# settylab/Mellon

Measured on AMD Instinct MI355X. Metric: cells/sec fit_predict, higher is better.
Workload: dtype f64

## Files before the change

mellon_amd/csrc/api_fit.hip:

```cpp
#include "api_internal.h"
#include "mln_options.h"
#include <mutex>
#include <unordered_map>

void fit_sample_rows(const mln_fit* f, int64_t s, int64_t* first, int64_t* rows) {
  if (s < 1) s = 1;
  *first = (s - f->row0 % s) % s;
  *rows = (f->n > *first) ? (f->n - *first + s - 1) / s : 0;
}

void fit_free(mln_fit* f) {
  if (!f) return;
  mln_ctx* ctx = f->ctx;
  (void)hipSetDevice(ctx->device);
  (void)hipStreamSynchronize(ctx->stream);
  if (f->L && f->L != f->Lp) (void)mln_dfree(f->L);
  if (f->Lp) (void)mln_dfree(f->Lp);
  triinv_free(&f->tri);
  void* ptrs[] = {f->V, f->Vdr, f->part_grad, f->part_hess, f->part_loss, f->d_z, f->d_out,
                  f->C, f->Cinv, f->d_u, f->d_gu, f->d_tmp, f->P, f->d_w, f->d_w_cached,
                  f->Q1, f->Q2, f->d_zw, f->d_zr, f->eigU, f->L32, f->sv_block, f->f_keep[0], f->f_keep[1], f->Kj, f->d_over,
                  f->dim_ell, f->dim_part, f->dim_z, f->dim_out};
  for (void* p : ptrs) if (p) (void)mln_dfree(p);
  for (double* p : f->saved_precond) if (p) (void)mln_dfree(p);
  if (f->h_state) (void)mln_hfree(f->h_state);
  fit_events_return(ctx, &f->evs);
  if (f->h_z) (void)mln_hfree(f->h_z);
  if (f->h_out) (void)mln_hfree(f->h_out);
  if (f->ev0) (void)hipEventDestroy(f->ev0);
  if (f->ev1) (void)hipEventDestroy(f->ev1);
  delete f;
}

extern "C" void mln_fit_destroy(mln_fit* fit) { fit_free(fit); }

int fit_alloc_workspace(mln_fit* f) {
  mln_ctx* ctx = f->ctx;
  int64_t steps = (f->n + 1) / 2;
  int n_wg = ctx->n_cu > 0 ? ctx->n_cu : 256;
  f->n_wg_cap = n_wg;
  if (steps < n_wg) n_wg = (int)(steps > 0 ? steps : 1);
  f->n_wg = n_wg;
  n_wg = f->n_wg_cap;
  const size_t pm = (size_t)f->ldl;
  f->ld2 = pad16(f->m + 2);
  MLN_HIP(ctx, mln_dmalloc((void**)&f->d_u, sizeof(double) * pm));
  MLN_HIP(ctx, mln_dmalloc((void**)&f->d_gu, sizeof(double) * pm));
  MLN_HIP(ctx, mln_dmalloc((void**)&f->d_tmp, sizeof(double) * (1 + pm)));
  MLN_HIP(ctx, mln_dmalloc((void**)&f->d_w, sizeof(double) * pm));
  MLN_HIP(ctx, mln_dmalloc((void**)&f->d_w_cached, sizeof(double) * pm));
  MLN_HIP(ctx, mln_dmalloc((void**)&f->d_zw, sizeof(double) * 2 * pm));
  MLN_HIP(ctx, mln_dmalloc((void**)&f->d_zr, sizeof(double) * 2 * (size_t)f->ld2));
  MLN_HIP(ctx, hipMemsetAsync(f->d_zr, 0, sizeof(double) * 2 * (size_t)f->ld2, ctx->stream));
  MLN_HIP(ctx, mln_dmalloc((void**)&f->d_over, 64));
  MLN_HIP(ctx, hipMemsetAsync(f->d_over, 0, 64, ctx->stream));
  MLN_HIP(ctx, mln_dmalloc((void**)&f->part_grad, sizeof(double) * pm * n_wg));
  MLN_HIP(ctx, mln_dmalloc((void**)&f->part_hess, sizeof(double) * pm * n_wg));
  MLN_HIP(ctx, mln_dmalloc((void**)&f->part_loss, sizeof(double) * n_wg));
  MLN_HIP(ctx, mln_dmalloc((void**)&f->d_z, sizeof(double) * pm));
  MLN_HIP(ctx, mln_dmalloc((void**)&f->d_out, sizeof(double) * (1 + 2 * pm)));
  MLN_HIP(ctx, mln_hmalloc((void**)&f->h_z, sizeof(double) * pm));
  MLN_HIP(ctx, mln_hmalloc((void**)&f->h_out, sizeof(double) * (1 + 2 * pm)));
  MLN_HIP(ctx, hipEventCreate(&f->ev0));
  MLN_HIP(ctx, hipEventCreate(&f->ev1));
  return MLN_OK;
}

namespace {
struct CopyLane { hipStream_t stream = nullptr; std::vector<hipEvent_t> events; };
std::mutex g_copy_mu;
std::unordered_map<mln_ctx*, CopyLane> g_copy_lanes;
}

static int copy_lane_get(mln_ctx* ctx, int n_events, hipStream_t* stream, std::vector<hipEvent_t>* events) {
  std::lock_guard<std::mutex> lk(g_copy_mu);
  CopyLane& lane = g_copy_lanes[ctx];
  if (!lane.stream) MLN_HIP(ctx, hipStreamCreateWithFlags(&lane.stream, hipStreamNonBlocking));
  while ((int)lane.events.size() < n_events) {
    hipEvent_t e = nullptr;
    MLN_HIP(ctx, hipEventCreateWithFlags(&e, hipEventDisableTiming));
    lane.events.push_back(e);
  }
  *stream = lane.stream;
  events->assign(lane.events.begin(), lane.events.begin() + n_events);
  return MLN_OK;
}

namespace {
std::unordered_map<mln_ctx*, std::vector<hipEvent_t>> g_event_pools;
}
void fit_events_borrow(mln_ctx* ctx, std::vector<hipEvent_t>* evs) {
  std::lock_guard<std::mutex> lk(g_copy_mu);
  auto& pool = g_event_pools[ctx];
  if (evs->empty()) evs->swap(pool);
}
void fit_events_return(mln_ctx* ctx, std::vector<hipEvent_t>* evs) {
  std::lock_guard<std::mutex> lk(g_copy_mu);
  auto& pool = g_event_pools[ctx];
// ... 122 lines not shown
  const double t_enter = now_s();
  const bool trace_all = std::getenv("MELLON_AMD_TRACE") != nullptr;
  MLN_TRY(mln_lower_cov(ctx, cov, d, &f->cov));
  f->d = d; f->n = n; f->full = (xu == nullptr);
  if (f->full) m = n;
  f->m = m;
  if (m < 1 || m > 65535) { mln_set_error(ctx, "number of landmarks out of range"); return MLN_ERR_SHAPE; }
  if (m > objective_max_m()) { mln_set_error(ctx, "m > 8192 landmarks is not supported by this build"); return MLN_ERR_UNSUPPORTED; }
  if (f->full && ctx->n_ranks > 1) { mln_set_error(ctx, "the full (non-sparse) GP cannot be cell-sharded"); return MLN_ERR_UNSUPPORTED; }
  f->ldp = pad16(m);
  f->ldl = pad16(m);
  DevIn dx, du;
  HostUpload up;
  bool pipelined = !f->full && n > 0 && x && !is_device_ptr(x) && (size_t)n * d * sizeof(double) >= ((size_t)32 << 20);
  if (pipelined) {
    dx.ctx = ctx;
    MLN_HIP(ctx, mln_dmalloc((void**)&dx.owned, (size_t)n * d * sizeof(double)));
    dx.dev = dx.owned;
    MLN_TRY(up.start(ctx, x, dx.owned, n, d));
    if (trace_all) fprintf(stderr, "[trace] fit_prepare: upload started at %.4f s (%d chunks)\n", now_s() - t_enter, up.n_chunks);
  } else {
    MLN_TRY(dx.init(ctx, x, (size_t)n * d));
  }
  if (!f->full) MLN_TRY(du.init(ctx, xu, (size_t)m * d));
  const double* centers = f->full ? dx.dev : du.dev;

  double t0 = now_s();
  const size_t lp_bytes = sizeof(double) * (size_t)m * f->ldp;
  MLN_HIP(ctx, mln_dmalloc((void**)&f->Lp, lp_bytes));
  MLN_HIP(ctx, hipMemsetAsync(f->Lp, 0, lp_bytes, ctx->stream));
  if (Lp_in) {
    DevIn dl;
    MLN_TRY(dl.init(ctx, Lp_in, (size_t)m * m));
    MLN_TRY(launch_copy_block(ctx, dl.dev, m, f->Lp, f->ldp, m, m));
    MLN_HIP(ctx, hipStreamSynchronize(ctx->stream));
  } else {
    MLN_TRY(launch_kernel_matrix(ctx, f->cov, centers, m, centers, m, d, f->Lp, f->ldp, jitter));
    const bool implicit = !f->full && (flags & MLN_FIT_IMPLICIT) != 0;
    if (implicit) {
      MLN_HIP(ctx, mln_dmalloc((void**)&f->Kj, lp_bytes));
      MLN_HIP(ctx, hipMemcpyAsync(f->Kj, f->Lp, lp_bytes, hipMemcpyDeviceToDevice, ctx->stream));
    }
    MLN_HIP(ctx, hipStreamSynchronize(ctx->stream));
    f->times[0] += now_s() - t0;
    t0 = now_s();
    if (implicit && (flags & MLN_FIT_DEFER_LP)) f->lp_pending = true;
    else MLN_TRY(dev_cholesky_lower(ctx, f->Lp, m, f->ldp));
  }
  f->jitter = jitter;
  if (!f->lp_pending) {
    MLN_TRY(triinv_build(ctx, f->Lp, m, f->ldp, true, true, &f->tri));
    MLN_HIP(ctx, hipStreamSynchronize(ctx->stream));
    f->times[1] += now_s() - t0;
  }

  if (f->full) {
    f->L = f->Lp;
  } else {
    t0 = now_s();
    const size_t l_bytes = sizeof(double) * (size_t)(n > 0 ? n : 1) * f->ldl;
    const bool trace = std::getenv("MELLON_AMD_TRACE") != nullptr;
    MLN_HIP(ctx, mln_dmalloc((void**)&f->L, l_bytes));
    if (trace) { (void)hipStreamSynchronize(ctx->stream); fprintf(stderr, "[trace] L alloc %.4f s\n", now_s() - t0); }
    int64_t mixed_min = (int64_t)1 << 27;
    bool mixed = false;
    if (const char* ev = std::getenv("MELLON_AMD_MIXED")) mixed = (flags & MLN_FIT_IMPLICIT) != 0 && std::atoi(ev) != 0;
    if (const char* ev = std::getenv("MELLON_AMD_MIXED_MIN_ELEMS")) mixed_min = std::atoll(ev);
    if (mixed && n * m >= mixed_min && n > 0 && m <= 8192)
      MLN_HIP(ctx, mln_dmalloc((void**)&f->L32, sizeof(float) * (size_t)n * f->ldl));
    f->l32_fixed = 0;
    bool bounded = true;
    for (int l = 0; l < f->cov.n_leaves; ++l)
      bounded = bounded && f->cov.leaves[l].kind >= MLN_K_MATERN32 && f->cov.leaves[l].kind <= MLN_K_RATQUAD;
    for (int t = 0; t < f->cov.n_toks; ++t)
      bounded = bounded && (f->cov.tok_op[t] == MLN_OP_LEAF || f->cov.tok_op[t] == MLN_OP_MUL);
    f->cov_bounded01 = bounded;
    if (f->L32) {
      f->l32_fixed = bounded ? 1 : 0;
      if (const char* ev = std::getenv("MELLON_AMD_SURROGATE")) {
        if (std::strcmp(ev, "float") == 0) f->l32_fixed = 0;
        else if (std::strcmp(ev, "fixed") == 0 && bounded) f->l32_fixed = 1;
      }
    }
    if (pipelined) {
      for (int c = 0; c < up.n_chunks; ++c) {
        int64_t r0 = 0, rows = 0;
        MLN_TRY(up.wait_chunk(c, &r0, &rows));
        MLN_TRY(launch_kernel_matrix(ctx, f->cov, dx.dev + r0 * d, rows, du.dev, m, d, f->L + r0 * f->ldl, f->ldl, 0.0,
                                     f->L32 ? f->L32 + r0 * f->ldl : nullptr, f->l32_fixed));
      }
      MLN_TRY(up.finish());
    } else {
      MLN_TRY(launch_kernel_matrix(ctx, f->cov, dx.dev, n, du.dev, m, d, f->L, f->ldl, 0.0, f->L32, f->l32_fixed));
    }
    MLN_TRY(fit_alloc_workspace(f));
    MLN_HIP(ctx, hipStreamSynchronize(ctx->stream));
    if (trace) fprintf(stderr, "[trace] L kernel matrix done at %.4f s\n", now_s() - t0);
    f->times[0] += now_s() - t0;
    if (flags & MLN_FIT_IMPLICIT) {
      f->kspace = true;
    } else {
      t0 = now_s();
      MLN_TRY(triinv_solve_right_T(ctx, f->tri, f->L, n, f->ldl));
      MLN_HIP(ctx, hipStreamSynchronize(ctx->stream));
      f->times[2] += now_s() - t0;
    }
  }
  if (!f->d_u) MLN_TRY(fit_alloc_workspace(f));
  if (trace_all) fprintf(stderr, "[trace] fit_prepare: body done at %.4f s\n", now_s() - t_enter);
  return MLN_OK;
}

extern "C" int mln_fit_prepare(mln_ctx* ctx, const mln_kernel_desc* cov, const double* x, int64_t n_local,
                               int32_t d, const double* xu, int64_t m, double jitter, const double* Lp_in,
                               int32_t flags, mln_fit** out) {
  if (!ctx || !out) return MLN_ERR_ARG;
  *out = nullptr;
  if (n_local < 0 || d < 1 || (n_local > 0 && !x)) { mln_set_error(ctx, "bad shape"); return MLN_ERR_SHAPE; }
  MLN_HIP(ctx, hipSetDevice(ctx->device));
  mln_fit* f = new mln_fit();
  const double t_call = now_s();
  int rc = fit_prepare_impl(ctx, cov, x, n_local, d, xu, m, jitter, Lp_in, flags, f);
  if (std::getenv("MELLON_AMD_TRACE")) fprintf(stderr, "[trace] mln_fit_prepare: %.4f s with the upload's teardown\n", now_s() - t_call);
  if (rc != MLN_OK) { fit_free(f); return rc; }
  *out = f;
  return MLN_OK;
}

extern "C" int mln_fit_from_L(mln_ctx* ctx, const double* L, int64_t n_local, int64_t m, const double* Lp,
                              mln_fit** out) {
  if (!ctx || !out || !L) return MLN_ERR_ARG;
  *out = nullptr;
  if (n_local < 1 || m < 1 || m > 65535) { mln_set_error(ctx, "bad shape"); return MLN_ERR_SHAPE; }
  if (m > objective_max_m()) { mln_set_error(ctx, "m > 8192 columns is not supported by this build"); return MLN_ERR_UNSUPPORTED; }
  MLN_HIP(ctx, hipSetDevice(ctx->device));
  mln_fit* f = new mln_fit();
  f->ctx = ctx; f->n = n_local; f->m = m; f->d = 0; f->full = false;
  f->ldl = pad16(m); f->ldp = pad16(m);
  auto body = [&]() -> int {
    DevIn dl;
    MLN_TRY(dl.init(ctx, L, (size_t)n_local * m));
    const size_t l_bytes = sizeof(double) * (size_t)n_local * f->ldl;
    MLN_HIP(ctx, mln_dmalloc((void**)&f->L, l_bytes));
    MLN_HIP(ctx, hipMemsetAsync(f->L, 0, l_bytes, ctx->stream));
    MLN_TRY(launch_copy_block(ctx, dl.dev, m, f->L, f->ldl, n_local, m));
    if (Lp) {
      DevIn dp;
      MLN_TRY(dp.init(ctx, Lp, (size_t)m * m));
      const size_t lp_bytes = sizeof(double) * (size_t)m * f->ldp;
      MLN_HIP(ctx, mln_dmalloc((void**)&f->Lp, lp_bytes));
      MLN_HIP(ctx, hipMemsetAsync(f->Lp, 0, lp_bytes, ctx->stream));
      MLN_TRY(launch_copy_block(ctx, dp.dev, m, f->Lp, f->ldp, m, m));
      MLN_TRY(triinv_build(ctx, f->Lp, m, f->ldp, true, true, &f->tri));
    }
    MLN_HIP(ctx, hipStreamSynchronize(ctx->stream));
    return fit_alloc_workspace(f);
  };
  int rc = body();
  if (rc != MLN_OK) { fit_free(f); return rc; }
  *out = f;
  return MLN_OK;
}

extern "C" int mln_fit_prepare_from_K(mln_ctx* ctx, const double* Kuu, int64_t n_local, int64_t m, double jitter,
                                      const double* Lp_in, int32_t flags, mln_fit** out) {
  if (!ctx || !out) return MLN_ERR_ARG;
  *out = nullptr;
  const bool full = (flags & MLN_FIT_FULL) != 0;
  if (n_local < 0 || m < 1 || m > 65535 || (full && n_local != m)) { mln_set_error(ctx, "bad shape"); return MLN_ERR_SHAPE; }
  if (!Kuu && !Lp_in) { mln_set_error(ctx, "mln_fit_prepare_from_K needs cov(xu, xu) or its factor"); return MLN_ERR_ARG; }
  if (full && ctx->n_ranks > 1) { mln_set_error(ctx, "the full (non-sparse) GP cannot be cell-sharded"); return MLN_ERR_UNSUPPORTED; }
  MLN_HIP(ctx, hipSetDevice(ctx->device));
  mln_fit* f = new mln_fit();
  f->ctx = ctx; f->n = n_local; f->m = m; f->d = 0; f->full = full;
  f->ldl = pad16(m); f->ldp = pad16(m);
  f->cov.n_leaves = 0; f->cov.n_toks = 0;
// ... 44 lines not shown
  MLN_HIP(ctx, hipStreamSynchronize(ctx->stream));
  f->k_rows_done += n_rows;
  f->times[0] += now_s() - t0;
  return MLN_OK;
}

extern "C" int mln_fit_finish_K(mln_fit* f) {
  if (!f) return MLN_ERR_ARG;
  mln_ctx* ctx = f->ctx;
  if (!f->from_K) { mln_set_error(ctx, "mln_fit_finish_K: not a handle built from kernel values"); return MLN_ERR_ARG; }
  if (f->k_finished || f->full) { f->k_finished = true; return MLN_OK; }
  if (f->k_rows_done < f->n) { mln_set_error(ctx, "mln_fit_finish_K: kernel rows are missing"); return MLN_ERR_SHAPE; }
  MLN_HIP(ctx, hipSetDevice(ctx->device));
  if (!f->kspace) {
    double t0 = now_s();
    MLN_TRY(triinv_solve_right_T(ctx, f->tri, f->L, f->n, f->ldl));
    MLN_HIP(ctx, hipStreamSynchronize(ctx->stream));
    f->times[2] += now_s() - t0;
  }
  f->k_finished = true;
  return fit_alloc_workspace(f);
}


extern "C" int mln_fit_gram_eigh(mln_fit* f, double* w, int32_t* n_sweeps) {
  if (!f || !w) return MLN_ERR_ARG;
  mln_ctx* ctx = f->ctx;
  MLN_HIP(ctx, hipSetDevice(ctx->device));
  const int64_t m = f->m, ld = f->ldl;
  double* G = nullptr;
  MLN_HIP(ctx, mln_dmalloc((void**)&G, sizeof(double) * (size_t)m * ld));
  int rc = f->kspace ? fit_gram(f, G, ld, 1) : gram_of(ctx, f->L, f->ldl, f->n, m, 1.0, G, ld);
  if (rc == MLN_OK && !f->eigU) {
    hipError_t e = mln_dmalloc((void**)&f->eigU, sizeof(double) * (size_t)m * ld);
    if (e != hipSuccess) rc = mln_hip_fail(ctx, e, "alloc eigenvectors", __FILE__, __LINE__);
  }
  std::vector<double> wh((size_t)m);
  int sweeps = 0;
  if (rc == MLN_OK) rc = dev_eigh(ctx, G, m, ld, wh.data(), f->eigU, ld, &sweeps);
  (void)hipStreamSynchronize(ctx->stream);
  (void)mln_dfree(G);
  if (rc != MLN_OK) return rc;
  if (n_sweeps) *n_sweeps = sweeps;
  std::memcpy(w, wh.data(), sizeof(double) * (size_t)m);
  return MLN_OK;
}

extern "C" int mln_fit_gram_rank(mln_fit* f, double tol, int64_t* rank_out, double* sigma_max_out) {
  if (!f || !rank_out || !(tol >= 0.0)) return MLN_ERR_ARG;
  mln_ctx* ctx = f->ctx;
  MLN_HIP(ctx, hipSetDevice(ctx->device));
  const int64_t m = f->m, ld = f->ldl;
  double* G = nullptr;
  MLN_HIP(ctx, mln_dmalloc((void**)&G, sizeof(double) * (size_t)m * ld));
  const int n_ranks = ctx->n_ranks > 1 ? ctx->n_ranks : 1;
  const int64_t n_est = f->n * n_ranks;
  int64_t stride = 1;
  if (f->kspace && n_est >= 24 * m) stride = std::max<int64_t>(1, n_est / (12 * m));
  auto gram = [&]() { return f->kspace ? fit_gram(f, G, ld, stride) : gram_of(ctx, f->L, f->ldl, f->n, m, 1.0, G, ld); };
  int rc = gram();
  double lmax = 0.0;
  const bool ldl_ok = !(mln_experiment("MELLON_AMD_RANK_LDL") && std::atoi(mln_experiment("MELLON_AMD_RANK_LDL")) == 0);
  bool done = false;
  if (rc == MLN_OK && ldl_ok) {
    rc = dev_sym_rank_above_ldl(ctx, G, m, ld, tol * tol, rank_out, &lmax, &done);
    if (rc == MLN_OK && !done) rc = gram();
  }
  if (rc == MLN_OK && !done) rc = dev_sym_rank_above(ctx, G, m, ld, tol * tol, rank_out, &lmax);
  f->rank_path = done ? 1 : 2;
  (void)hipStreamSynchronize(ctx->stream);
  (void)mln_dfree(G);
  if (rc == MLN_OK && sigma_max_out) *sigma_max_out = std::sqrt(std::max(lmax, 0.0));
  return rc;
}

extern "C" int mln_fit_project(mln_fit* f, int64_t p, mln_fit** out) {
  if (!f || !out) return MLN_ERR_ARG;
  *out = nullptr;
  mln_ctx* ctx = f->ctx;
  if (!f->eigU) { mln_set_error(ctx, "project: call mln_fit_gram_eigh first"); return MLN_ERR_ARG; }
  if (f->kspace) { mln_set_error(ctx, "project needs the explicit factor (prepare without MLN_FIT_IMPLICIT)"); return MLN_ERR_UNSUPPORTED; }
  if (p < 1 || p > f->m) { mln_set_error(ctx, "project: rank out of range"); return MLN_ERR_SHAPE; }
  MLN_HIP(ctx, hipSetDevice(ctx->device));
  mln_fit* g = new mln_fit();
  g->ctx = ctx; g->n = f->n; g->m = p; g->d = 0; g->full = false;
  g->ldl = pad16(p); g->ldp = pad16(p);
  auto body = [&]() -> int {
    const size_t l_bytes = sizeof(double) * (size_t)(g->n > 0 ? g->n : 1) * g->ldl;
    MLN_HIP(ctx, mln_dmalloc((void**)&g->L, l_bytes));
    MLN_HIP(ctx, hipMemsetAsync(g->L, 0, l_bytes, ctx->stream));
    if (g->n > 0) {
      GemmArgs a{};
      a.A = f->L; a.lda = f->ldl; a.ta = 0;
      a.B = f->eigU + (f->m - p) * f->ldl; a.ldb = f->ldl; a.tb = 1;
      a.C = g->L; a.ldc = g->ldl;
      a.M = g->n; a.N = p; a.K = f->m; a.alpha = 1.0; a.beta = 0.0; a.split_k = 1;
      MLN_TRY(launch_dgemm(ctx, a));
    }
    MLN_HIP(ctx, hipStreamSynchronize(ctx->stream));
    return fit_alloc_workspace(g);
  };
  int rc = body();
  if (rc != MLN_OK) { fit_free(g); return rc; }
  *out = g;
  return MLN_OK;
}

extern "C" int mln_fit_rank(mln_fit* fit, int64_t* m_out) {
  if (!fit || !m_out) return MLN_ERR_ARG;
  *m_out = fit->m;
  return MLN_OK;
}

extern "C" int mln_fit_get_Lp(mln_fit* f, double* out) {
  if (!f || !out) return MLN_ERR_ARG;
  mln_ctx* ctx = f->ctx;
  if (!f->Lp) { mln_set_error(ctx, "this fit handle holds no Lp"); return MLN_ERR_ARG; }
  MLN_HIP(ctx, hipSetDevice(ctx->device));
  MLN_TRY(fit_ensure_lp(f, false));
  DevOut o;
  MLN_TRY(o.init(ctx, out, (size_t)f->m * f->m));
  MLN_TRY(launch_copy_block(ctx, f->Lp, f->ldp, o.dev, f->m, f->m, f->m));
  return o.commit();
}

extern "C" int mln_fit_get_L(mln_fit* f, int64_t row0, int64_t n_rows, double* out) {
  if (!f || (n_rows > 0 && !out)) return MLN_ERR_ARG;
  mln_ctx* ctx = f->ctx;
  if (row0 < 0 || n_rows < 0 || row0 + n_rows > f->n) { mln_set_error(ctx, "row range out of bounds"); return MLN_ERR_SHAPE; }
  if (n_rows == 0) return MLN_OK;
  MLN_HIP(ctx, hipSetDevice(ctx->device));
  DevOut o;
  MLN_TRY(o.init(ctx, out, (size_t)n_rows * f->m));
  if (f->kspace) {
    MLN_TRY(fit_ensure_lp(f));
    double* tmp = nullptr;
    MLN_HIP(ctx, mln_dmalloc((void**)&tmp, sizeof(double) * (size_t)n_rows * f->ldl));
    int rc = launch_copy_block(ctx, f->L + row0 * f->ldl, f->ldl, tmp, f->ldl, n_rows, f->ldl);
    if (rc == MLN_OK) rc = triinv_solve_right_T(ctx, f->tri, tmp, n_rows, f->ldl);
    if (rc == MLN_OK) rc = launch_copy_block(ctx, tmp, f->ldl, o.dev, f->m, n_rows, f->m);
    if (rc == MLN_OK) rc = o.commit();
    (void)mln_dfree(tmp);
    return rc;
  }
  MLN_TRY(launch_copy_block(ctx, f->L + row0 * f->ldl, f->ldl, o.dev, f->m, n_rows, f->m));
  return o.commit();
}

extern "C" int mln_fit_set_likelihood(mln_fit* f, const double* V, const double* Vdr, double mu) {
  if (!f || (f->n > 0 && (!V || !Vdr))) return MLN_ERR_ARG;
  mln_ctx* ctx = f->ctx;
  MLN_HIP(ctx, hipSetDevice(ctx->device));
  const size_t bytes = sizeof(double) * (size_t)(f->n > 0 ? f->n : 1);
  if (!f->V) MLN_HIP(ctx, mln_dmalloc((void**)&f->V, bytes));
  if (!f->Vdr) MLN_HIP(ctx, mln_dmalloc((void**)&f->Vdr, bytes));
  if (f->n > 0) {
    MLN_HIP(ctx, hipMemcpyAsync(f->V, V, sizeof(double) * f->n, hipMemcpyDefault, ctx->stream));
    MLN_HIP(ctx, hipMemcpyAsync(f->Vdr, Vdr, sizeof(double) * f->n, hipMemcpyDefault, ctx->stream));
    MLN_HIP(ctx, hipStreamSynchronize(ctx->stream));
  }
  f->mu = mu;
  return MLN_OK;
}

ObjArgs obj_args(mln_fit* f) {
  ObjArgs a{};
  a.L = f->L; a.ldl = f->ldl; a.n = f->n; a.m = f->m;
  a.z = f->d_z; a.V = f->V; a.Vdr = f->Vdr; a.mu = f->mu;
  a.part_grad = f->part_grad; a.part_hess = nullptr; a.part_loss = f->part_loss;
  a.weights = nullptr; a.f_out = nullptr;
  a.n_wg = f->n_wg; a.m_pad = f->ldl;
  return a;
}
```

mellon_amd/csrc/api_internal.h:

```cpp
#pragma once
#include <chrono>
#include <cmath>
#include <cstdio>
#include <cstdlib>
#include <algorithm>
#include <atomic>
#include <cstring>
#include <mutex>
#include <string>
#include <thread>
#include <vector>

#include "linalg.h"
#include "mln_internal.h"
#include "objective.h"
#include "precond_rebuild.h"
#include "solver.h"

hipError_t mln_hmalloc(void** out, size_t bytes);
hipError_t mln_hfree(void* p);
void fit_events_borrow(mln_ctx* ctx, std::vector<hipEvent_t>* evs);
void fit_events_return(mln_ctx* ctx, std::vector<hipEvent_t>* evs);

void mln_dfree_defer(std::vector<void*>* sink);
bool is_device_ptr(const void* p);
double now_s();

struct DevIn {
  mln_ctx* ctx;
  const double* dev = nullptr;
  double* owned = nullptr;
  int init(mln_ctx* c, const double* p, size_t count) {
    ctx = c;
    if (count == 0 || !p) { dev = p; return MLN_OK; }
    if (is_device_ptr(p)) { dev = p; return MLN_OK; }
    MLN_HIP(ctx, mln_dmalloc((void**)&owned, count * sizeof(double)));
    MLN_HIP(ctx, hipMemcpyAsync(owned, p, count * sizeof(double), hipMemcpyHostToDevice, ctx->stream));
    dev = owned;
    return MLN_OK;
  }
  ~DevIn() {
    if (owned) { (void)hipStreamSynchronize(ctx->stream); (void)mln_dfree(owned); }
  }
};

struct DevOut {
  mln_ctx* ctx;
  double* dev = nullptr;
  double* owned = nullptr;
  double* host = nullptr;
  size_t count = 0;
  int init(mln_ctx* c, double* p, size_t n, bool copy_in = false) {
    ctx = c; count = n;
    if (n == 0) { dev = p; return MLN_OK; }
    if (is_device_ptr(p)) { dev = p; return MLN_OK; }
    host = p;
    MLN_HIP(ctx, mln_dmalloc((void**)&owned, n * sizeof(double)));
    if (copy_in) MLN_HIP(ctx, hipMemcpyAsync(owned, p, n * sizeof(double), hipMemcpyHostToDevice, ctx->stream));
    dev = owned;
    return MLN_OK;
  }
  int commit() {
    if (owned && count) {
      MLN_HIP(ctx, hipMemcpyAsync(host, owned, count * sizeof(double), hipMemcpyDeviceToHost, ctx->stream));
    }
    MLN_HIP(ctx, hipStreamSynchronize(ctx->stream));
    return MLN_OK;
  }
  ~DevOut() {
    if (owned) { (void)hipStreamSynchronize(ctx->stream); (void)mln_dfree(owned); }
  }
};

struct mln_fit {
  mln_ctx* ctx = nullptr;
  DevCov cov;
  int d = 0;
  int64_t n = 0, m = 0, ldl = 0, ldp = 0;
  bool full = false;
  double* L = nullptr;
  double* Lp = nullptr;
  TriInv tri;
  double *V = nullptr, *Vdr = nullptr;
  double mu = 0.0;
  int n_wg = 0;
  double *part_grad = nullptr, *part_hess = nullptr, *part_loss = nullptr;
  double *d_z = nullptr, *d_out = nullptr;
  double *h_z = nullptr, *h_out = nullptr;
  hipEvent_t ev0 = nullptr, ev1 = nullptr;
  double times[MLN_N_STAGE_TIMES] = {0};
  double *C = nullptr, *Cinv = nullptr;
  double *d_u = nullptr, *d_gu = nullptr, *d_tmp = nullptr;
  int n_wg_cap = 0;
  bool kspace = false;
  double* P = nullptr;
  double* Kj = nullptr;
  bool lp_pending = false, lp_failed = false, tri_pending = false;
  double jitter = 0.0;
  double* d_w = nullptr;
  std::vector<double> z_cached;
  double* d_w_cached = nullptr;
  double *Q1 = nullptr, *Q2 = nullptr, *d_zw = nullptr, *d_zr = nullptr;
  double* eigU = nullptr;
  float* L32 = nullptr;
  double emu_excluded = 0.0;
  bool cov_bounded01 = false;
  int l32_fixed = 0;
  int evals32 = 0;
  double times32 = 0.0;
  int64_t ld2 = 0;
  int* d_over = nullptr;
  int64_t row0 = 0;
  SolverBuffers sv{};
  void* sv_block = nullptr;
  SolverState* h_state = nullptr;
  int sv_maxcor = 0;
  std::vector<hipEvent_t> evs;
  double* f_keep[2] = {nullptr, nullptr};
  int f_final = -1;
  int64_t precond_stride = 0;
  bool from_K = false, k_finished = false;
  int64_t k_rows_done = 0;
  double* saved_precond[5] = {nullptr, nullptr, nullptr, nullptr, nullptr};
  int n_revert = 0, n_rebuild_skipped = 0, n_start_halvings = 0, rank_path = 0;
  double build_seconds = 0.0;
  double times_sub = 0.0, times_rebuild = 0.0, sub_pass_equiv = 0.0;
  int evals_sub = 0, n_rebuild = 0;
  double* dim_ell = nullptr;
  int dim_k = 0;
  double mu_dim = 0.0, mu_dens = 0.0;
  double *dim_part = nullptr, *dim_z = nullptr, *dim_out = nullptr;
};

struct DevScratch {
  mln_ctx* ctx;
  double* p = nullptr;
  explicit DevScratch(mln_ctx* c) : ctx(c) {}
  hipError_t alloc(size_t bytes) { return mln_dmalloc((void**)&p, bytes); }
  ~DevScratch() {
    if (p) { (void)hipStreamSynchronize(ctx->stream); (void)mln_dfree(p); }
  }
  DevScratch(const DevScratch&) = delete;
  DevScratch& operator=(const DevScratch&) = delete;
};


int dev_allreduce(mln_ctx* ctx, double* dev, int64_t count);
int dev_bcast0(mln_ctx* ctx, double* dev, int64_t count);
int reject_distance_leaf(mln_ctx* ctx, const DevCov& dc);
int64_t pad16(int64_t m);
void fit_sample_rows(const mln_fit* f, int64_t s, int64_t* first, int64_t* rows);
void fit_free(mln_fit* f);
int fit_alloc_workspace(mln_fit* f);
int fit_prepare_impl(mln_ctx* ctx, const mln_kernel_desc* cov, const double* x, int64_t n, int32_t d,
                            const double* xu, int64_t m, double jitter, const double* Lp_in, int32_t flags,
                            mln_fit* f);
ObjArgs obj_args(mln_fit* f);
void obj_account(mln_fit* f, bool f32 = false);
int fit_w_from_z(mln_fit* f, const double* z_dev, double* w_dev, const double* z_host = nullptr);
int fit_cache_pair_from_u(mln_fit* f, const double* u_dev);
int fit_enqueue_eval(mln_fit* f, const double* u_dev, double* gn_dev, bool use32, const int* gate,
                            hipEvent_t* ev, const std::vector<int64_t>* sub_strides = nullptr);
int fit_objective_u(mln_fit* f, const double* u, double* loss, double* grad_u, double* z_out,
                           bool use32 = false);
int fit_solver_alloc(mln_fit* f, int maxcor);
int gram_of(mln_ctx* ctx, const double* A, int64_t lda, int64_t rows, int64_t m, double alpha, double* G,
                   int64_t ldg, bool quantised = false);
int emulated_ranks(const mln_ctx* ctx);
int fit_ensure_kj(mln_fit* f);
int fit_ensure_lp(mln_fit* f, bool need_tri = true);
int fit_lp_finish(mln_fit* f, int rc_chol, double t0);
int fit_gram(mln_fit* f, double* G, int64_t ldg, int64_t row_stride, bool whiten = true);
int fit_gemvT(mln_fit* f, const double* t_dev, double* rhs_dev);
void fit_drop_precond_operators(mln_fit* f);
int fit_factor_precond(mln_fit* f);
int fit_build_precond(mln_fit* f, int64_t row_stride);
int fit_rebuild_precond(mln_fit* f, const double* f_dev, double rows_per_m, int* outcome, double cap = 1e300);
void fit_precond_saved_free(mln_fit* f);
int fit_precond_revert(mln_fit* f);
int fit_small_gemv(mln_fit* f, const double* M, int trans, const double* w, double* y);
int launch_scale_rows_cols(mln_ctx* ctx, double* A, int64_t ld, int64_t rows, int64_t cols, const double* row,
                                  const double* col);
int sparse_solve_impl(mln_ctx* ctx, const mln_kernel_desc* cov, const double* x, int64_t n_local,
                             int32_t d, const double* xu, int64_t m, const double* y, int64_t p, double mu,
                             const double* sigmas, int32_t kind, double jitter, double* W, double* Lp_out,
                             double* Cs_out);
unsigned grid_1d(int64_t count);
```

mellon_amd/csrc/api_precond.hip:

```cpp
#include "api_internal.h"
#include "mln_options.h"

namespace {
__global__ void k_pack_lower(const double* __restrict__ G, int64_t m, int64_t ld, double* __restrict__ out) {
  const int64_t i = blockIdx.y;
  const int64_t j = (int64_t)blockIdx.x * blockDim.x + threadIdx.x;
  if (j <= i) out[i * (i + 1) / 2 + j] = G[i * ld + j];
}
__global__ void k_unpack_symmetric(const double* __restrict__ in, int64_t m, int64_t ld, double* __restrict__ G) {
  const int64_t i = blockIdx.y;
  const int64_t j = (int64_t)blockIdx.x * blockDim.x + threadIdx.x;
  if (j < m) G[i * ld + j] = (j <= i) ? in[i * (i + 1) / 2 + j] : in[j * (j + 1) / 2 + i];
}
}

int allreduce_symmetric_lower(mln_ctx* ctx, double* G, int64_t m, int64_t ldg) {
  const int64_t cnt = m * (m + 1) / 2;
  double* packed = nullptr;
  MLN_HIP(ctx, mln_dmalloc((void**)&packed, sizeof(double) * (size_t)cnt));
  const dim3 grid((unsigned)((m + 255) / 256), (unsigned)m), block(256);
  hipLaunchKernelGGL(k_pack_lower, grid, block, 0, ctx->stream, G, m, ldg, packed);
  int rc = dev_allreduce(ctx, packed, cnt);
  if (rc == MLN_OK) {
    hipLaunchKernelGGL(k_unpack_symmetric, grid, block, 0, ctx->stream, packed, m, ldg, G);
// ... 13 lines not shown
  double* parts = nullptr;
  if (split > 1) MLN_HIP(ctx, mln_dmalloc((void**)&parts, sizeof(double) * stride * split));
  GemmArgs g{};
  g.A = A; g.lda = lda; g.B = A; g.ldb = lda;
  g.C = (split > 1) ? parts : G; g.ldc = ldg;
  g.M = m; g.N = m; g.K = rows; g.alpha = alpha; g.beta = 0.0; g.ta = 1; g.tb = 0; g.lower_only = 1;
  g.split_k = split; g.c_split_stride = (int64_t)stride;
  int rc = MLN_OK;
  if (split > 1) rc = (hipMemsetAsync(parts, 0, sizeof(double) * stride * split, ctx->stream) == hipSuccess) ? MLN_OK : MLN_ERR_HIP;
  else rc = (hipMemsetAsync(G, 0, sizeof(double) * stride, ctx->stream) == hipSuccess) ? MLN_OK : MLN_ERR_HIP;
  if (rc == MLN_OK && rows > 0)
    rc = quantised ? launch_gram_i8(ctx, A, lda, rows, m, alpha, g.C, ldg, (int64_t)stride, split) : launch_dgemm(ctx, g);
  if (rc == MLN_OK && split > 1) rc = launch_sum_partials(ctx, parts, split, (int64_t)stride, G, (int64_t)stride, 0.0);
  if (rc == MLN_OK && ctx->n_ranks > 1) rc = allreduce_symmetric_lower(ctx, G, m, ldg);
  else if (rc == MLN_OK) rc = launch_symmetrize_from_lower(ctx, G, m, ldg);
  (void)hipStreamSynchronize(ctx->stream);
  if (parts) (void)mln_dfree(parts);
  return rc;
}

extern "C" int mln_diag_gram_i8(mln_ctx* ctx, const double* A, int64_t rows, int64_t m, double* out, int32_t reps,
                                double* ms_out) {
  if (!ctx || !A || !out || rows < 1 || m < 1) return MLN_ERR_ARG;
  MLN_HIP(ctx, hipSetDevice(ctx->device));
  DevIn a;
  DevOut o;
  MLN_TRY(a.init(ctx, A, (size_t)rows * m));
  MLN_TRY(o.init(ctx, out, (size_t)m * m));
  const int split = gram_i8_splits(rows, m);
  const size_t stride = (size_t)m * m;
  double *parts = nullptr, *G = nullptr;
  MLN_HIP(ctx, mln_dmalloc((void**)&parts, sizeof(double) * stride * split));
  MLN_HIP(ctx, mln_dmalloc((void**)&G, sizeof(double) * stride));
  hipEvent_t e0, e1;
  MLN_HIP(ctx, hipEventCreate(&e0));
  MLN_HIP(ctx, hipEventCreate(&e1));
  int rc = MLN_OK;
  if (reps < 1) reps = 1;
  for (int r = 0; r <= reps && rc == MLN_OK; ++r) {
    if (r == 1) (void)hipEventRecord(e0, ctx->stream);
    rc = (hipMemsetAsync(parts, 0, sizeof(double) * stride * split, ctx->stream) == hipSuccess) ? MLN_OK : MLN_ERR_HIP;
    if (rc == MLN_OK) rc = launch_gram_i8(ctx, a.dev, m, rows, m, 1.0, parts, m, (int64_t)stride, split);
    if (rc == MLN_OK) rc = launch_sum_partials(ctx, parts, split, (int64_t)stride, G, (int64_t)stride, 0.0);
  }
  (void)hipEventRecord(e1, ctx->stream);
  (void)hipStreamSynchronize(ctx->stream);
  float ms = 0.f;
  (void)hipEventElapsedTime(&ms, e0, e1);
  if (ms_out) *ms_out = ms / reps;
  if (rc == MLN_OK) rc = launch_symmetrize_from_lower(ctx, G, m, m);
  if (rc == MLN_OK) rc = launch_copy_block(ctx, G, m, o.dev, m, m, m);
  if (rc == MLN_OK) rc = o.commit();
  (void)hipStreamSynchronize(ctx->stream);
  (void)mln_dfree(parts); (void)mln_dfree(G);
  (void)hipEventDestroy(e0); (void)hipEventDestroy(e1);
  return rc;
}

int emulated_ranks(const mln_ctx* ctx) {
  if (ctx->n_ranks > 1) return 0;
  if (const char* ev = std::getenv("MELLON_AMD_EMULATE_RANKS")) { const int n = std::atoi(ev); return n > 1 ? n : 0; }
  return 0;
}

int fit_ensure_kj(mln_fit* f) {
  if (f->Kj) return MLN_OK;
  mln_ctx* ctx = f->ctx;
  if (!f->Lp) { mln_set_error(ctx, "this fit handle holds no Lp"); return MLN_ERR_ARG; }
  const size_t bytes = sizeof(double) * (size_t)f->m * f->ldp;
  MLN_HIP(ctx, mln_dmalloc((void**)&f->Kj, bytes));
  MLN_HIP(ctx, hipMemsetAsync(f->Kj, 0, bytes, ctx->stream));
  GemmArgs g{};
  g.A = f->Lp; g.lda = f->ldp; g.B = f->Lp; g.ldb = f->ldp; g.C = f->Kj; g.ldc = f->ldp;
  g.M = f->m; g.N = f->m; g.K = f->m; g.alpha = 1.0; g.beta = 0.0; g.ta = 0; g.tb = 1; g.lower_only = 1;
  MLN_TRY(launch_dgemm(ctx, g));
  return launch_symmetrize_from_lower(ctx, f->Kj, f->m, f->ldp);
}

int fit_gram(mln_fit* f, double* G, int64_t ldg, int64_t row_stride, bool whiten) {
  mln_ctx* ctx = f->ctx;
  if (row_stride < 1) row_stride = 1;
  const int64_t first = (row_stride - f->row0 % row_stride) % row_stride;
  const int64_t rows = (f->n > first) ? (f->n - first + row_stride - 1) / row_stride : 0;
  const double* Ls = f->L + first * f->ldl;
  if (!f->kspace) return gram_of(ctx, Ls, f->ldl * row_stride, rows, f->m, (double)row_stride, G, ldg);
  bool quant = f->cov_bounded01 && f->m >= 256 && row_stride > 1;
  if (const char* ev = mln_experiment("MELLON_AMD_GRAM_I8")) quant = quant && std::atoi(ev) != 0;
  int rc = gram_of(ctx, Ls, f->ldl * row_stride, rows, f->m, (double)row_stride, G, ldg, quant);
  if (rc != MLN_OK || !whiten) return rc;
  MLN_TRY(fit_ensure_lp(f));
  double* T = nullptr;
  {
    hipError_t e = mln_dmalloc((void**)&T, sizeof(double) * (size_t)f->m * ldg);
    if (e == hipSuccess) e = hipMemsetAsync(T, 0, sizeof(double) * (size_t)f->m * ldg, ctx->stream);
    if (e != hipSuccess) rc = mln_hip_fail(ctx, e, "alloc Gram temp", __FILE__, __LINE__);
  }
  if (rc == MLN_OK) rc = triinv_solve_left(ctx, f->tri, G, f->m, ldg);
  if (rc == MLN_OK) rc = launch_transpose(ctx, G, ldg, T, ldg, f->m);
  if (rc == MLN_OK) rc = triinv_solve_left(ctx, f->tri, T, f->m, ldg);
  if (rc == MLN_OK) rc = (hipMemcpyAsync(G, T, sizeof(double) * (size_t)f->m * ldg, hipMemcpyDeviceToDevice,
                                         ctx->stream) == hipSuccess) ? MLN_OK : MLN_ERR_HIP;
  (void)hipStreamSynchronize(ctx->stream);
  if (T) (void)mln_dfree(T);
  return rc;
}

int fit_gemvT(mln_fit* f, const double* t_dev, double* rhs_dev) {
  mln_ctx* ctx = f->ctx;
  ObjArgs a = obj_args(f);
  a.weights = t_dev;
  a.part_loss = nullptr;
  MLN_TRY(launch_objective(ctx, a));
  MLN_TRY(launch_reduce_obj(ctx, a, f->d_out));
  MLN_TRY(dev_allreduce(ctx, f->d_out, 1 + f->m));
  if (f->kspace) { MLN_TRY(fit_ensure_lp(f)); MLN_TRY(triinv_solve_left(ctx, f->tri, f->d_out + 1, 1, 1)); }
  MLN_HIP(ctx, hipMemcpyAsync(rhs_dev, f->d_out + 1, sizeof(double) * f->m, hipMemcpyDeviceToDevice, ctx->stream));
  return MLN_OK;
}

void fit_drop_precond_operators(mln_fit* f) {
  (void)hipStreamSynchronize(f->ctx->stream);
  void* ptrs[] = {f->Cinv, f->P, f->Q1, f->Q2};
  for (void* p : ptrs) if (p) (void)mln_dfree(p);
  f->Cinv = nullptr; f->P = nullptr; f->Q1 = nullptr; f->Q2 = nullptr;
}

int fit_factor_precond(mln_fit* f) {
  mln_ctx* ctx = f->ctx;
  const int64_t m = f->m, ldg = f->ldl;
  const size_t bytes = sizeof(double) * (size_t)m * ldg;
  int rc = f->kspace ? MLN_OK : launch_add_diag(ctx, f->C, m, ldg, 1.0);
  if (rc == MLN_OK && f->kspace && f->lp_pending && !f->lp_failed && f->ldp == ldg) {
    const double t0 = now_s();
    int bad = 0;
    rc = dev_cholesky_lower2(ctx, f->C, f->Lp, m, ldg, &bad);
    const int rc_lp = (rc == MLN_ERR_NOT_PD && !(bad & 2)) ? MLN_OK : rc;
    if (rc == MLN_OK || rc == MLN_ERR_NOT_PD) {
      const std::string msg = ctx->err;
      const int rl = fit_lp_finish(f, rc_lp, t0);
      if (rl != MLN_OK) return rl;
      if (rc != MLN_OK) mln_set_error(ctx, msg);
    }
  } else if (rc == MLN_OK) {
    rc = dev_cholesky_lower(ctx, f->C, m, ldg);
  }
  TriInv t;
  if (rc == MLN_OK) rc = triinv_build(ctx, f->C, m, ldg, true, false, &t);
  double* inv = nullptr;
  auto zeroed = [&](double** p, const char* what) {
    hipError_t e = mln_dmalloc((void**)p, bytes);
    if (e == hipSuccess) e = hipMemsetAsync(*p, 0, bytes, ctx->stream);
    if (e != hipSuccess) rc = mln_hip_fail(ctx, e, what, __FILE__, __LINE__);
  };
  if (rc == MLN_OK) zeroed(&inv, "alloc factor inverse");
  if (rc == MLN_OK) rc = launch_add_diag(ctx, inv, m, ldg, 1.0);
  if (rc == MLN_OK) rc = triinv_solve_left(ctx, t, inv, m, ldg, true);
  if (rc == MLN_OK && f->kspace) {
    zeroed(&f->P, "alloc P");
    if (rc == MLN_OK) rc = launch_transpose(ctx, inv, ldg, f->P, ldg, m);
  } else if (rc == MLN_OK) {
    const int64_t ld = ldg;
    const size_t blk = (size_t)m * ld;
    hipError_t e = mln_dmalloc((void**)&f->Q1, sizeof(double) * blk);
    if (e == hipSuccess) e = mln_dmalloc((void**)&f->Q2, sizeof(double) * blk * 2);
    if (e == hipSuccess) e = hipMemsetAsync(f->Q1, 0, sizeof(double) * blk, ctx->stream);
    if (e == hipSuccess) e = hipMemsetAsync(f->Q2, 0, sizeof(double) * blk * 2, ctx->stream);
    if (e != hipSuccess) rc = mln_hip_fail(ctx, e, "alloc stacked operators", __FILE__, __LINE__);
    if (rc == MLN_OK) rc = launch_transpose(ctx, inv, ld, f->Q1, ld, m);
    if (rc == MLN_OK) rc = launch_copy_block(ctx, inv, ld, f->Q2, ld * 2, m, ld);
    if (rc == MLN_OK) rc = launch_copy_block(ctx, inv, ld, f->Q2 + ld, ld * 2, m, ld);
  }
  (void)hipStreamSynchronize(ctx->stream);
  triinv_free(&t);
  if (rc == MLN_OK) f->Cinv = inv; else if (inv) (void)mln_dfree(inv);
  return rc;
}

int fit_build_precond(mln_fit* f, int64_t row_stride) {
  if (f->Cinv) return MLN_OK;
  mln_ctx* ctx = f->ctx;
  const int64_t m = f->m, ldg = f->ldl;
  const size_t bytes = sizeof(double) * (size_t)m * ldg;
  double t0 = now_s();
  MLN_HIP(ctx, mln_dmalloc((void**)&f->C, bytes));
  int rc = fit_gram(f, f->C, ldg, row_stride, false);
  if (rc == MLN_OK && f->kspace) rc = fit_ensure_kj(f);
  if (rc == MLN_OK && f->kspace) rc = launch_axpby(ctx, m * ldg, 1.0, f->Kj, 1.0, f->C);
  MLN_HIP(ctx, hipStreamSynchronize(ctx->stream));
  f->times[3] += now_s() - t0;
  double t1 = now_s();
  if (rc == MLN_OK) rc = fit_factor_precond(f);
  f->times[4] += now_s() - t1;
  if (rc == MLN_OK) { f->precond_stride = row_stride < 1 ? 1 : row_stride; f->build_seconds = now_s() - t0; }
  return rc;
}

void fit_precond_saved_free(mln_fit* f) {
  bool any = false;
  for (double* p : f->saved_precond) any = any || p;
  if (!any) return;
  (void)hipStreamSynchronize(f->ctx->stream);
  for (double*& p : f->saved_precond) { if (p) (void)mln_dfree(p); p = nullptr; }
}

int fit_precond_revert(mln_fit* f) {
  if (!f->saved_precond[0] || !f->saved_precond[1]) return MLN_ERR_ARG;
  fit_drop_precond_operators(f);
  if (f->C) { (void)mln_dfree(f->C); f->C = nullptr; }
  f->C = f->saved_precond[0]; f->Cinv = f->saved_precond[1]; f->P = f->saved_precond[2];
  f->Q1 = f->saved_precond[3]; f->Q2 = f->saved_precond[4];
  for (double*& p : f->saved_precond) p = nullptr;
  return MLN_OK;
}

int fit_rebuild_precond(mln_fit* f, const double* f_dev, double rows_per_m, int* outcome, double cap) {
  mln_ctx* ctx = f->ctx;
  const int64_t m = f->m, ldg = f->ldl;
  *outcome = 0;
  RebuildSelection sel{};
  double target = rows_per_m * (double)m;
  if (const int n_emu = emulated_ranks(ctx)) target /= (double)n_emu;
  const bool tr_on = std::getenv("MELLON_AMD_TRACE") != nullptr;
  double tt[6] = {0, 0, 0, 0, 0, 0};
  auto lap = [&](int i, double& t0) { if (tr_on) { (void)hipStreamSynchronize(ctx->stream); const double t1 = now_s(); tt[i] += t1 - t0; t0 = t1; } };
  double tl = now_s();
  MLN_TRY(rebuild_select_rows(ctx, f_dev, f->V, f->n, f->row0, target, 0x6d656c6c6f6eull, &sel, cap));
  lap(0, tl);
  if (tr_on)
    fprintf(stderr, "[trace] rebuild: %lld of %lld local rows kept (target %.0f global), c = %.4g, 1/c = %.4g, w_max = %.4g, sum a = %.6g\n",
            (long long)sel.rows, (long long)f->n, target, sel.c, 1.0 / sel.c, sel.w_max, sel.sum_a);
  double range_cap = 1e7;
  if (const char* ev = mln_experiment("MELLON_AMD_REBUILD_RANGE")) range_cap = std::atof(ev);
  if (!(sel.w_max * sel.c <= range_cap) || !std::isfinite(sel.sum_a)) {
    rebuild_selection_free(ctx, &sel);
    *outcome = 1;
    return MLN_OK;
  }
  double* R = nullptr;
  int rc = MLN_OK;
  const int64_t rr = sel.rows > 0 ? sel.rows : 1;
  if (mln_dmalloc((void**)&R, sizeof(double) * (size_t)rr * f->ldl) != hipSuccess) rc = MLN_ERR_HIP;
  if (rc == MLN_OK) rc = launch_gather_scale_rows(ctx, f->L, f->ldl, sel.idx, sel.scale, sel.rows, R);
  double* old_set[5] = {f->C, f->Cinv, f->P, f->Q1, f->Q2};
  f->C = nullptr; f->Cinv = nullptr; f->P = nullptr; f->Q1 = nullptr; f->Q2 = nullptr;
  if (rc == MLN_OK && mln_dmalloc((void**)&f->C, sizeof(double) * (size_t)m * ldg) != hipSuccess) rc = MLN_ERR_HIP;
  lap(1, tl);
  if (rc == MLN_OK) {
    bool quant = f->kspace && f->cov_bounded01 && m >= 256;
    if (const char* ev = mln_experiment("MELLON_AMD_GRAM_I8")) quant = quant && std::atoi(ev) != 0;
    rc = gram_of(ctx, R, f->ldl, sel.rows, m, sel.w_max, f->C, ldg, quant);
  }
  (void)hipStreamSynchronize(ctx->stream);
  if (R) (void)mln_dfree(R);
  rebuild_selection_free(ctx, &sel);
  lap(2, tl);
  if (rc == MLN_OK && f->kspace) rc = fit_ensure_kj(f);
  if (rc == MLN_OK && f->kspace) rc = launch_axpby(ctx, m * ldg, 1.0, f->Kj, 1.0, f->C);
  lap(3, tl);
  if (rc == MLN_OK) rc = fit_factor_precond(f);
  lap(4, tl);
  if (tr_on) fprintf(stderr, "[trace] rebuild ms: select %.2f, gather %.2f, gram %.2f, + Kj %.2f, factor+inverses+stacks %.2f (rc %d)\n",
                     1e3 * tt[0], 1e3 * tt[1], 1e3 * tt[2], 1e3 * tt[3], 1e3 * tt[4], rc);
  if (rc == MLN_ERR_NOT_PD) {
    fit_drop_precond_operators(f);
    if (f->C) { (void)hipStreamSynchronize(ctx->stream); (void)mln_dfree(f->C); }
    f->C = old_set[0]; f->Cinv = old_set[1]; f->P = old_set[2]; f->Q1 = old_set[3]; f->Q2 = old_set[4];
    *outcome = 2;
    return MLN_OK;
  }
  if (rc != MLN_OK) {
    fit_drop_precond_operators(f);
    if (f->C) { (void)hipStreamSynchronize(ctx->stream); (void)mln_dfree(f->C); }
    f->C = old_set[0]; f->Cinv = old_set[1]; f->P = old_set[2]; f->Q1 = old_set[3]; f->Q2 = old_set[4];
    return rc;
  }
  fit_precond_saved_free(f);
  for (int i = 0; i < 5; ++i) f->saved_precond[i] = old_set[i];
  return MLN_OK;
}

int fit_small_gemv(mln_fit* f, const double* M, int trans, const double* w, double* y) {
  mln_ctx* ctx = f->ctx;
  ObjArgs a{};
  a.L = M; a.ldl = f->ldl; a.n = f->m; a.m = f->m; a.mu = 0.0;
  a.part_grad = f->part_grad; a.part_hess = nullptr; a.part_loss = nullptr;
  a.m_pad = f->ldl;
  int64_t steps = (f->m + 1) / 2;
  a.n_wg = (int)((steps < f->n_wg_cap) ? (steps > 0 ? steps : 1) : f->n_wg_cap);
  if (trans) {
    a.weights = w;
    MLN_TRY(launch_objective(ctx, a));
    MLN_TRY(launch_reduce_obj(ctx, a, f->d_tmp));
    MLN_HIP(ctx, hipMemcpyAsync(y, f->d_tmp + 1, sizeof(double) * f->m, hipMemcpyDeviceToDevice, ctx->stream));
  } else {
    a.z = w;
    a.f_out = y;
    MLN_TRY(launch_objective(ctx, a));
  }
  return MLN_OK;
}

extern "C" int mln_fit_set_row_offset(mln_fit* f, int64_t global_row0) {
  if (!f || global_row0 < 0) return MLN_ERR_ARG;
  f->row0 = global_row0;
  return MLN_OK;
}

extern "C" int mln_precond_build(mln_fit* f, int64_t row_stride) {
  if (!f) return MLN_ERR_ARG;
  MLN_HIP(f->ctx, hipSetDevice(f->ctx->device));
  if (row_stride < 1) row_stride = 1;
  if (f->Cinv && f->precond_stride != row_stride) {
    fit_drop_precond_operators(f);
    if (f->C) { (void)mln_dfree(f->C); f->C = nullptr; }
    f->precond_stride = 0;
  }
  return fit_build_precond(f, row_stride);
}

extern "C" int mln_ridge_init(mln_fit* f, const double* target, double* z0) {
  if (!f || !z0 || (f->n > 0 && !target)) return MLN_ERR_ARG;
  mln_ctx* ctx = f->ctx;
  MLN_HIP(ctx, hipSetDevice(ctx->device));
  MLN_TRY(fit_build_precond(f, 1));
  double t0 = now_s();
  DevIn dt;
  MLN_TRY(dt.init(ctx, target, (size_t)f->n));
  int64_t rs = (f->precond_stride >= 11 && f->m <= objective_max_m_one_pass()) ? f->precond_stride : 1;
  if (const char* ev = mln_experiment("MELLON_AMD_SUBSAMPLE")) { if (std::atoi(ev) == 0) rs = 1; }
  ObjArgs a = obj_args(f);
  a.weights = dt.dev;
  a.part_loss = nullptr;
  if (rs > 1) {
    int64_t first = 0, rows = 0;
    fit_sample_rows(f, rs, &first, &rows);
    a.n = rows; a.row_first = first; a.row_stride = rs; a.out_scale = (double)rs;
  }
  if (f->kspace) {
    a.L32 = f->L32;
    a.l32_fixed = f->l32_fixed;
    MLN_TRY(launch_objective(ctx, a));
    MLN_TRY(launch_reduce_obj(ctx, a, f->d_out));
    MLN_TRY(dev_allreduce(ctx, f->d_out, 1 + f->m));
    MLN_TRY(fit_small_gemv(f, f->Cinv, 0, f->d_out + 1, f->d_gu));
    MLN_TRY(fit_small_gemv(f, f->P, 0, f->d_gu, f->d_w));
    MLN_TRY(fit_ensure_lp(f, false));
    MLN_TRY(fit_small_gemv(f, f->Lp, 1, f->d_w, f->d_z));
  } else {
    MLN_TRY(launch_objective(ctx, a));
    MLN_TRY(launch_reduce_obj(ctx, a, f->d_out));
    MLN_TRY(dev_allreduce(ctx, f->d_out, 1 + f->m));
    MLN_TRY(fit_small_gemv(f, f->Cinv, 0, f->d_out + 1, f->d_gu));
  }
  if (!f->kspace) MLN_TRY(fit_small_gemv(f, f->Cinv, 1, f->d_gu, f->d_z));
  MLN_TRY(fit_cache_pair_from_u(f, f->d_gu));
  MLN_HIP(ctx, hipMemcpyAsync(z0, f->d_z, sizeof(double) * f->m, hipMemcpyDefault, ctx->stream));
  MLN_HIP(ctx, hipStreamSynchronize(ctx->stream));
  f->times[4] += now_s() - t0;
  return MLN_OK;
}

extern "C" int mln_precond_apply(mln_fit* f, int32_t mode, const double* in, double* out) {
  if (!f || !in || !out) return MLN_ERR_ARG;
  mln_ctx* ctx = f->ctx;
  MLN_HIP(ctx, hipSetDevice(ctx->device));
  MLN_TRY(fit_build_precond(f, 1));
  MLN_HIP(ctx, hipMemcpyAsync(f->d_u, in, sizeof(double) * f->m, hipMemcpyDefault, ctx->stream));
  if (f->kspace && mode >= 0 && mode <= 2) {
    MLN_TRY(fit_ensure_lp(f));
    if (mode == 0) {
      MLN_TRY(fit_w_from_z(f, f->d_u, f->d_w, is_device_ptr(in) ? nullptr : in));
      MLN_TRY(fit_small_gemv(f, f->C, 1, f->d_w, f->d_gu));
    } else if (mode == 1) {
      MLN_TRY(fit_small_gemv(f, f->P, 0, f->d_u, f->d_w));
      MLN_TRY(fit_small_gemv(f, f->Lp, 1, f->d_w, f->d_gu));
    } else {
      MLN_TRY(fit_small_gemv(f, f->Lp, 0, f->d_u, f->d_w));
      MLN_TRY(fit_small_gemv(f, f->Cinv, 0, f->d_w, f->d_gu));
    }
  }
  else if (mode == 0) MLN_TRY(fit_small_gemv(f, f->C, 1, f->d_u, f->d_gu));
  else if (mode == 1) MLN_TRY(fit_small_gemv(f, f->Cinv, 1, f->d_u, f->d_gu));
  else if (mode == 2) MLN_TRY(fit_small_gemv(f, f->Cinv, 0, f->d_u, f->d_gu));
  else { mln_set_error(ctx, "mln_precond_apply: unknown mode"); return MLN_ERR_ARG; }
  MLN_HIP(ctx, hipMemcpyAsync(out, f->d_gu, sizeof(double) * f->m, hipMemcpyDefault, ctx->stream));
  MLN_HIP(ctx, hipStreamSynchronize(ctx->stream));
  return MLN_OK;
}
```

mellon_amd/csrc/api_solve.hip:

```cpp
#include "api_internal.h"
#include "mln_options.h"


void obj_account(mln_fit* f, bool f32) {
  float ms = 0.f;
  const bool ok = hipEventElapsedTime(&ms, f->ev0, f->ev1) == hipSuccess;
  if (f32) {
    if (ok) f->times32 += 1e-3 * ms;
    f->evals32 += 1;
    return;
  }
  if (ok) f->times[5] += 1e-3 * ms;
  f->times[6] += 1.0;
  f->times[7] = (double)f->n * (double)f->ldl * 8.0;
}

int fit_w_from_z(mln_fit* f, const double* z_dev, double* w_dev, const double* z_host) {
  mln_ctx* ctx = f->ctx;
  if (z_host && f->z_cached.size() == (size_t)f->m &&
      std::memcmp(z_host, f->z_cached.data(), sizeof(double) * f->m) == 0) {
    MLN_HIP(ctx, hipMemcpyAsync(w_dev, f->d_w_cached, sizeof(double) * f->m, hipMemcpyDeviceToDevice, ctx->stream));
    return MLN_OK;
  }
  MLN_TRY(fit_ensure_lp(f));
  MLN_HIP(ctx, hipMemcpyAsync(w_dev, z_dev, sizeof(double) * f->m, hipMemcpyDeviceToDevice, ctx->stream));
  return triinv_solve_left_T(ctx, f->tri, w_dev, 1, 1);
}

int fit_cache_pair_from_u(mln_fit* f, const double* u_dev) {
  mln_ctx* ctx = f->ctx;
  f->z_cached.assign((size_t)f->m, 0.0);
  MLN_HIP(ctx, hipMemcpyAsync(f->z_cached.data(), f->d_z, sizeof(double) * f->m, hipMemcpyDeviceToHost, ctx->stream));
  if (f->kspace) MLN_TRY(fit_small_gemv(f, f->P, 0, u_dev, f->d_w_cached));
  MLN_HIP(ctx, hipStreamSynchronize(ctx->stream));
  return MLN_OK;
}

extern "C" int mln_objective(mln_fit* f, const double* z, double* loss, double* grad, double* hess_diag) {
  if (!f || !z || !loss || !grad) return MLN_ERR_ARG;
  mln_ctx* ctx = f->ctx;
  if (!f->V) { mln_set_error(ctx, "mln_fit_set_likelihood has not been called"); return MLN_ERR_ARG; }
  if (hess_diag && f->kspace) {
    mln_set_error(ctx, "the Hessian diagonal needs the explicit factor L: prepare the fit without MLN_FIT_IMPLICIT");
    return MLN_ERR_UNSUPPORTED;
  }
  MLN_HIP(ctx, hipSetDevice(ctx->device));
  MLN_TRY(fit_ensure_lp(f));
  const int64_t m = f->m;
  MLN_HIP(ctx, hipMemcpyAsync(f->d_z, z, sizeof(double) * m, hipMemcpyDefault, ctx->stream));
  MLN_HIP(ctx, hipMemcpyAsync(f->h_z, f->d_z, sizeof(double) * m, hipMemcpyDeviceToHost, ctx->stream));
  ObjArgs a = obj_args(f);
  if (f->kspace) {
    MLN_TRY(fit_w_from_z(f, f->d_z, f->d_w));
    a.z = f->d_w;
  }
  if (hess_diag) a.part_hess = f->part_hess;
  const int64_t nout = 1 + m + (hess_diag ? m : 0);
  MLN_HIP(ctx, hipEventRecord(f->ev0, ctx->stream));
  MLN_TRY(launch_objective(ctx, a));
  MLN_HIP(ctx, hipEventRecord(f->ev1, ctx->stream));
  MLN_TRY(launch_reduce_obj(ctx, a, f->d_out));
  MLN_TRY(dev_allreduce(ctx, f->d_out, nout));
  if (f->kspace) MLN_TRY(triinv_solve_left(ctx, f->tri, f->d_out + 1, 1, 1));
  MLN_HIP(ctx, hipMemcpyAsync(f->h_out, f->d_out, sizeof(double) * nout, hipMemcpyDeviceToHost, ctx->stream));
  MLN_HIP(ctx, hipStreamSynchronize(ctx->stream));
  obj_account(f);
  double zz = 0.0;
  for (int64_t j = 0; j < m; ++j) zz += f->h_z[j] * f->h_z[j];
  *loss = f->h_out[0] + 0.5 * zz + 0.5 * (double)m * std::log(2.0 * M_PI);
  std::vector<double> tmp;
  double* gh = grad;
  if (is_device_ptr(grad)) { tmp.resize(m); gh = tmp.data(); }
  for (int64_t j = 0; j < m; ++j) gh[j] = f->h_out[1 + j] + f->h_z[j];
  if (gh != grad) MLN_HIP(ctx, hipMemcpy(grad, gh, sizeof(double) * m, hipMemcpyHostToDevice));
  if (hess_diag) {
    std::vector<double> th;
    double* hh = hess_diag;
    if (is_device_ptr(hess_diag)) { th.resize(m); hh = th.data(); }
    for (int64_t j = 0; j < m; ++j) hh[j] = f->h_out[1 + m + j] + 1.0;
    if (hh != hess_diag) MLN_HIP(ctx, hipMemcpy(hess_diag, hh, sizeof(double) * m, hipMemcpyHostToDevice));
  }
  return MLN_OK;
}

extern "C" int mln_transform(mln_fit* f, const double* z, double mu, double* f_out) {
  if (!f || !z || (f->n > 0 && !f_out)) return MLN_ERR_ARG;
  mln_ctx* ctx = f->ctx;
  MLN_HIP(ctx, hipSetDevice(ctx->device));
  if (f->n == 0) return MLN_OK;
  MLN_HIP(ctx, hipMemcpyAsync(f->d_z, z, sizeof(double) * f->m, hipMemcpyDefault, ctx->stream));
  if (f->f_final >= 0 && mu == f->mu && !is_device_ptr(z) && f->z_cached.size() == (size_t)f->m &&
      std::memcmp(z, f->z_cached.data(), sizeof(double) * f->m) == 0) {
    MLN_HIP(ctx, hipMemcpyAsync(f_out, f->f_keep[f->f_final], sizeof(double) * (size_t)f->n, hipMemcpyDefault, ctx->stream));
    MLN_HIP(ctx, hipStreamSynchronize(ctx->stream));
    return MLN_OK;
  }
  DevOut o;
  MLN_TRY(o.init(ctx, f_out, (size_t)f->n));
  ObjArgs a = obj_args(f);
  if (f->kspace) {
    MLN_TRY(fit_w_from_z(f, f->d_z, f->d_w, is_device_ptr(z) ? nullptr : z));
    a.z = f->d_w;
  }
  a.f_out = o.dev;
  a.mu = mu;
  MLN_TRY(launch_objective(ctx, a));
  return o.commit();
}

int fit_enqueue_eval(mln_fit* f, const double* u_dev, double* gn_dev, bool use32, const int* gate,
                            hipEvent_t* ev, const std::vector<int64_t>* sub_strides) {
  mln_ctx* ctx = f->ctx;
  const int64_t m = f->m, ld = f->ldl, ld2 = f->ld2;
  if (f->kspace) {
    GemvTri g1{f->P, ld, m, u_dev, f->d_w, nullptr, 1, m, m, 0, 0, gate};
    MLN_TRY(launch_gemv_tri(ctx, g1));
    GemvTri gk{f->Kj, f->ldp, m, f->d_w, f->d_zr, nullptr, 2, m, m, 0, 0, gate};
    MLN_TRY(launch_gemv_tri(ctx, gk));
  } else {
    GemvTri g1{f->Q1, ld, m, u_dev, f->d_zr, nullptr, 1, m, m, 0, 0, gate};
    MLN_TRY(launch_gemv_tri(ctx, g1));
  }
  ObjArgs a = obj_args(f);
  a.z = f->kspace ? f->d_w : f->d_zr;
  a.gate = gate;
  if (gate && f->f_keep[0] && objective_can_keep_f(f->n, f->n_wg)) { a.f_keep[0] = f->f_keep[0]; a.f_keep[1] = f->f_keep[1]; a.f_slot = &f->sv.st->f_slot; }
  if (gate) { a.cap = &f->sv.st->cap; a.over_flag = f->d_over; }
  if (ev) MLN_HIP(ctx, hipEventRecord(ev[0], ctx->stream));
  if (f->L32 && (gate || use32)) {
    ObjArgs a32 = a;
    a32.L32 = f->L32;
    a32.l32_fixed = f->l32_fixed;
    a32.gate_want = MLN_GATE_F32;
    if (gate) a32.cap = &f->sv.st->cap;
    MLN_TRY(launch_objective(ctx, a32));
  }
  if (ev) MLN_HIP(ctx, hipEventRecord(ev[1], ctx->stream));
  if (gate || !use32 || !f->L32) {
    a.gate_want = MLN_GATE_F64;
    MLN_TRY(launch_objective(ctx, a));
  }
  if (gate && sub_strides) {
    for (size_t lv = 0; lv < sub_strides->size(); ++lv) {
      const int64_t sub_stride = (*sub_strides)[lv];
      ObjArgs as = a;
      int64_t first = 0, rows = 0;
      fit_sample_rows(f, sub_stride, &first, &rows);
      as.n = rows; as.row_first = first; as.row_stride = sub_stride; as.out_scale = (double)sub_stride;
      as.f_keep[0] = as.f_keep[1] = nullptr; as.f_slot = nullptr;
      as.gate_want = MLN_GATE_SUB;
      as.gate2 = &f->sv.st->sub_level; as.gate2_want = (int)lv;
      MLN_TRY(launch_objective(ctx, as));
    }
  }
  if (ev) MLN_HIP(ctx, hipEventRecord(ev[2], ctx->stream));
  MLN_TRY(launch_reduce_obj2(ctx, a, f->d_zr + ld2 + m, f->d_zr + ld2));
  MLN_TRY(dev_allreduce(ctx, f->d_zr + ld2, m + 2));
  if (f->kspace) {
    GemvTri g2{f->Cinv, ld, m, f->d_zr, gn_dev, nullptr, 0, m, m, 0, 0, gate};
    g2.xadd = f->d_zr + ld2;
    MLN_TRY(launch_gemv_tri(ctx, g2));
  } else {
    GemvTri g2{f->Q2, 2 * ld, m, f->d_zr, gn_dev, nullptr, 0, m, m, ld, ld2, gate};
    MLN_TRY(launch_gemv_tri(ctx, g2));
  }
  return MLN_OK;
}

int fit_objective_u(mln_fit* f, const double* u, double* loss, double* grad_u, double* z_out,
                           bool use32) {
  mln_ctx* ctx = f->ctx;
  const int64_t m = f->m;
  MLN_HIP(ctx, hipMemcpyAsync(f->d_u, u, sizeof(double) * m, hipMemcpyDefault, ctx->stream));
  hipEvent_t ev[3] = {f->ev0, use32 ? f->ev1 : f->ev0, f->ev1};
  MLN_TRY(fit_enqueue_eval(f, f->d_u, f->d_gu, use32, nullptr, ev));
  MLN_HIP(ctx, hipMemcpyAsync(f->h_out, f->d_zr + f->ld2 + m, sizeof(double), hipMemcpyDeviceToHost, ctx->stream));
  MLN_HIP(ctx, hipMemcpyAsync(f->h_out + 1, f->d_gu, sizeof(double) * m, hipMemcpyDeviceToHost, ctx->stream));
  MLN_HIP(ctx, hipMemcpyAsync(f->h_z, f->kspace ? f->d_w : f->d_zr, sizeof(double) * m, hipMemcpyDeviceToHost, ctx->stream));
  if (f->kspace) MLN_HIP(ctx, hipMemcpyAsync(f->h_out + 1 + m, f->d_zr, sizeof(double) * m, hipMemcpyDeviceToHost, ctx->stream));
  MLN_HIP(ctx, hipStreamSynchronize(ctx->stream));
  obj_account(f, use32);
  double zz = 0.0;
  for (int64_t j = 0; j < m; ++j) zz += f->h_z[j] * (f->kspace ? f->h_out[1 + m + j] : f->h_z[j]);
  *loss = f->h_out[0] + 0.5 * zz + 0.5 * (double)m * std::log(2.0 * M_PI);
  std::memcpy(grad_u, f->h_out + 1, sizeof(double) * m);
  if (z_out && f->kspace) {
    MLN_TRY(fit_ensure_lp(f, false));
    MLN_TRY(fit_small_gemv(f, f->Lp, 1, f->d_w, f->d_z));
    MLN_HIP(ctx, hipMemcpyAsync(z_out, f->d_z, sizeof(double) * m, hipMemcpyDeviceToHost, ctx->stream));
    MLN_HIP(ctx, hipStreamSynchronize(ctx->stream));
  } else if (z_out) {
    std::memcpy(z_out, f->h_z, sizeof(double) * m);
  }
  return MLN_OK;
}

extern "C" int mln_objective_precond(mln_fit* f, const double* u, double* loss, double* grad_u, double* z_out) {
  if (!f || !u || !loss || !grad_u) return MLN_ERR_ARG;
  mln_ctx* ctx = f->ctx;
  if (!f->V) { mln_set_error(ctx, "mln_fit_set_likelihood has not been called"); return MLN_ERR_ARG; }
  MLN_HIP(ctx, hipSetDevice(ctx->device));
  MLN_TRY(fit_build_precond(f, 1));
  return fit_objective_u(f, u, loss, grad_u, z_out);
}

int fit_solver_alloc(mln_fit* f, int maxcor) {
  mln_ctx* ctx = f->ctx;
  if (f->sv_block && f->sv_maxcor >= maxcor) return MLN_OK;
  if (f->sv_block) { MLN_HIP(ctx, hipStreamSynchronize(ctx->stream)); MLN_HIP(ctx, mln_dfree(f->sv_block)); f->sv_block = nullptr; }
  const size_t ld = (size_t)f->ldl;
  const size_t n_dbl = 6 * ld + 2 * (size_t)maxcor * ld + 2 * 64 + 4 * 512 + (sizeof(SolverState) + 63) / 64 * 8;
  MLN_HIP(ctx, mln_dmalloc(&f->sv_block, sizeof(double) * n_dbl));
  MLN_HIP(ctx, hipMemsetAsync(f->sv_block, 0, sizeof(double) * n_dbl, ctx->stream));
  double* p = (double*)f->sv_block;
  SolverBuffers& b = f->sv;
  b.u = p; p += ld; b.g = p; p += ld; b.un = p; p += ld; b.gn = p; p += ld; b.d = p; p += ld;
  b.S = p; p += (size_t)maxcor * ld; b.Y = p; p += (size_t)maxcor * ld;
  b.rho = p; p += 64; b.yy = p; p += 64;
  b.c = p; p += ld;
  b.trace = p; p += 4 * 512;
  b.st = (SolverState*)p;
  b.ld = (int64_t)ld;
  b.z = f->kspace ? f->d_w : f->d_zr;
  b.z2 = f->kspace ? f->d_zr : nullptr;
  b.lik = f->d_zr + f->ld2 + f->m;
  b.over = f->d_zr + f->ld2 + f->m + 1;
  f->sv_maxcor = maxcor;
  if (!f->h_state) MLN_HIP(ctx, mln_hmalloc((void**)&f->h_state, sizeof(SolverState)));
  return MLN_OK;
}

extern "C" int mln_map_solve(mln_fit* f, const double* z0, const mln_solver_opts* opts_in, double* z_out,
                             double* loss_out, int32_t* n_eval_out, int32_t* n_iter_out, int32_t* status_out) {
  if (!f || !z0 || !z_out) return MLN_ERR_ARG;
// ... 38 lines not shown
  init.use_corr = (phase32 && f->l32_fixed) ? 1 : 0;
  if (const char* ev = mln_experiment("MELLON_AMD_CORRECTED")) init.use_corr = init.use_corr && std::atoi(ev) != 0;
  init.prior_const = 0.5 * (double)m * std::log(2.0 * M_PI);
  init.t0 = 1.0;
  init.boost = 0.15;
  if (const char* ev = mln_experiment("MELLON_AMD_LS_BOOST")) init.boost = std::atof(ev);
  init.cap = 9.0;
  init.cap_step = 4.0;
  if (const char* ev = mln_experiment("MELLON_AMD_EXP_CAP"))
    init.cap = (std::strcmp(ev, "off") == 0 || std::atof(ev) <= 0.0) ? __builtin_inf() : std::atof(ev);
  if (phase32 && !mln_experiment("MELLON_AMD_EXP_CAP")) init.cap = __builtin_inf();
  init.cap0 = init.cap;
  init.boost_fall = 0.15;
  std::vector<int64_t> sub_strides;
  if (f->precond_stride >= 11) sub_strides.push_back(std::max<int64_t>(2, 3 * f->precond_stride / 16));
  if (const char* ev = mln_experiment("MELLON_AMD_SUBSAMPLE")) { if (std::atoi(ev) == 0) sub_strides.clear(); }
  const std::vector<int64_t>* subs = sub_strides.empty() ? nullptr : &sub_strides;
  init.gate_full = init.gate;
  init.sub_tol = 1e-3;
  init.sub_max_evals = 1 << 30;
  init.n_sub_levels = (int)sub_strides.size();
  init.sub_level = 0;
  if (subs) init.gate = MLN_GATE_SUB;
  const double pass_s = (double)f->n * (double)f->ldl * 8.0 / 6.5e12 + 1.4e-4;
  const double md = (double)f->m;
  const double gram_rows = (double)f->n / (double)(f->precond_stride > 0 ? f->precond_stride : 1);
  const double build_model_s = 2.2e-4 * std::ceil(md / 128.0) + gram_rows * md * md * 2.0 / 1.0e15;
  double want_rebuild = (f->build_seconds > 0.0 && 13.0 * pass_s > build_model_s) ? 1.0 : 0.0;
  if (const char* ev = mln_experiment("MELLON_AMD_REBUILD")) want_rebuild = std::atoi(ev) != 0 ? 1.0 : 0.0;
  if (phase32 && !(f->l32_fixed)) want_rebuild = 0.0;
  const bool keeps_f = f->f_keep[0] && f->f_keep[1] && objective_can_keep_f(f->n, f->n_wg);
  {
    double vote[2] = {ctx->rank == 0 ? want_rebuild : 0.0, keeps_f ? 0.0 : 1.0};
    MLN_HIP(ctx, hipMemcpyAsync(f->d_tmp, vote, sizeof(vote), hipMemcpyHostToDevice, ctx->stream));
    MLN_TRY(dev_allreduce(ctx, f->d_tmp, 2));
    MLN_HIP(ctx, hipMemcpyAsync(vote, f->d_tmp, sizeof(vote), hipMemcpyDeviceToHost, ctx->stream));
    MLN_HIP(ctx, hipStreamSynchronize(ctx->stream));
    want_rebuild = (vote[0] != 0.0 && vote[1] == 0.0) ? 1.0 : 0.0;
  }
  int max_rebuilds = 1000;
  if (const char* ev = mln_experiment("MELLON_AMD_MAX_REBUILDS")) max_rebuilds = std::max(1, std::atoi(ev));
  init.rebuild_armed = want_rebuild != 0.0 ? (phase32 ? 1 : max_rebuilds) : 0;
  init.it_resume = -1;
  init.over_many = std::max(8.0, 1e-4 * (double)f->n * (double)(ctx->n_ranks > 1 ? ctx->n_ranks : 1));
  init.over_cnt_acc = 0.0;
  init.switch_t0 = 0.35;
  init.gap_tol = 0.2 * o.ftol;
  init.dec_prev = 0.0; init.dec_prev2 = 0.0;
  init.rebuild_tol = 1e-3;
  init.start_cap = 1e30;
  init.n_shrink = 0;
  init.revert_after = 0; init.it_at_resume = -1; init.pause_reason = 0;
  int revert_after = 60;
  if (const char* ev = mln_experiment("MELLON_AMD_REVERT_AFTER")) revert_after = std::atoi(ev);
  double rebuild_rows_per_m = 6.0;
  MLN_TRY(launch_solver_init(ctx, f->sv, init, f->d_gu));
  const int* gate = &f->sv.st->gate;
  static const bool timing = !(std::getenv("MELLON_AMD_TIMING") && std::atoi(std::getenv("MELLON_AMD_TIMING")) == 0);
  int n_enq = 0, rebuilds_this_solve = 0, failed_rebuilds = 0;
  auto events_for = [&](int i) -> hipEvent_t* {
    if (!timing || i >= 512) return nullptr;
    while ((int)f->evs.size() < 3 * (i + 1)) {
      hipEvent_t e;
      if (hipEventCreate(&e) != hipSuccess) return nullptr;
      f->evs.push_back(e);
    }
    return &f->evs[3 * i];
  };
  MLN_TRY(fit_enqueue_eval(f, f->sv.un, f->sv.gn, false, gate, events_for(n_enq), subs));
  ++n_enq;
  std::vector<std::pair<int, int>> slot_shift;
  const std::vector<int64_t>* subs_live = subs;
  int batch = 8;
  const int64_t hard_cap = (int64_t)o.maxiter * o.maxls + 16;
  for (;;) {
    for (int b = 0; b < batch; ++b) {
      MLN_TRY(launch_solver_step(ctx, f->sv, (int)m));
      MLN_TRY(fit_enqueue_eval(f, f->sv.un, f->sv.gn, false, gate, events_for(n_enq), subs_live));
      ++n_enq;
    }
    MLN_TRY(dev_bcast0(ctx, (double*)f->sv.st, (int64_t)(sizeof(SolverState) / sizeof(double))));
    MLN_HIP(ctx, hipMemcpyAsync(f->h_state, f->sv.st, sizeof(SolverState), hipMemcpyDeviceToHost, ctx->stream));
    MLN_HIP(ctx, hipStreamSynchronize(ctx->stream));
    if (f->h_state->gate == MLN_GATE_DONE) break;
    if (subs_live && f->h_state->n_eval_sub > 0 && f->h_state->gate != MLN_GATE_SUB) subs_live = nullptr;
    if (f->h_state->gate == MLN_GATE_PAUSE) {
      const double tr0 = now_s(), ex_r0 = f->emu_excluded;
      const SolverState ps = *f->h_state;
      const bool revert = ps.pause_reason == 2 && f->saved_precond[0] != nullptr;
      if (!revert && (ps.pause_reason == 2 || !ps.f_valid)) {
        MLN_TRY(launch_solver_resume(ctx, f->sv, ps.gate_after_pause, 0));
      } else {
        double *zt = nullptr, *gz = nullptr, *cz = nullptr;
        MLN_HIP(ctx, mln_dmalloc((void**)&zt, sizeof(double) * 3 * (size_t)f->ldl));
        gz = zt + f->ldl; cz = gz + f->ldl;
        MLN_HIP(ctx, hipMemsetAsync(zt, 0, sizeof(double) * 3 * (size_t)f->ldl, ctx->stream));
        int rc = f->kspace ? fit_small_gemv(f, f->P, 0, f->sv.u, zt) : fit_small_gemv(f, f->Cinv, 1, f->sv.u, zt);
        if (rc == MLN_OK) rc = fit_small_gemv(f, f->C, 0, f->sv.g, gz);
        if (rc == MLN_OK && ps.corr) rc = fit_small_gemv(f, f->C, 0, f->sv.c, cz);
        int outcome = 0;
        if (rc == MLN_OK) rc = revert ? fit_precond_revert(f) : fit_rebuild_precond(f, f->f_keep[ps.f_slot], rebuild_rows_per_m * (rebuilds_this_solve > 0 ? 2.0 : 1.0), &outcome, ps.cap);
        if (rc == MLN_OK && outcome == 0) {
          rc = fit_small_gemv(f, f->C, 1, zt, f->sv.u);
          if (rc == MLN_OK) rc = f->kspace ? fit_small_gemv(f, f->P, 1, gz, f->sv.g) : fit_small_gemv(f, f->Cinv, 0, gz, f->sv.g);
          if (rc == MLN_OK && ps.corr) rc = f->kspace ? fit_small_gemv(f, f->P, 1, cz, f->sv.c) : fit_small_gemv(f, f->Cinv, 0, cz, f->sv.c);
        }
        (void)hipStreamSynchronize(ctx->stream);
        (void)mln_dfree(zt);
        MLN_TRY(rc);
        if (outcome == 0) {
          if (revert && ps.corr && (ps.gate_after_pause & 3) == MLN_GATE_F32)
            MLN_TRY(launch_solver_resume_plain32(ctx, f->sv, MLN_GATE_F32, (int)m, 1));
          else
            MLN_TRY(launch_solver_resume(ctx, f->sv, ps.gate_after_pause, 1, (revert || ps.rebuild_armed > 0) ? 0 : revert_after));
          if (revert) f->n_revert += 1; else { f->n_rebuild += 1; rebuilds_this_solve += 1; }
        } else {
          failed_rebuilds += 1;
          if (ps.corr && (ps.gate_after_pause & 3) == MLN_GATE_F32) MLN_TRY(launch_solver_resume_plain32(ctx, f->sv, MLN_GATE_F32, (int)m));
          else MLN_TRY(launch_solver_resume(ctx, f->sv, ps.gate_after_pause, 0, 0, failed_rebuilds >= 2 ? 0 : -1));
          f->n_rebuild_skipped += 1;
        }
        if (trace_lvl) fprintf(stderr, "[trace] map_solve pause at evaluation %d: %s\n", ps.n_eval,
                               revert ? "second preconditioner failed its trial: first one restored"
                                      : (outcome == 0 ? "preconditioner rebuilt" : (outcome == 1 ? "rebuild declined (weight range)" : "rebuild lost positive definiteness: kept the first")));
      }
      MLN_HIP(ctx, hipStreamSynchronize(ctx->stream));
      f->times_rebuild += now_s() - tr0 - (f->emu_excluded - ex_r0);
      slot_shift.push_back({ps.n_eval, n_enq - ps.n_eval});
      continue;
    }
    if (n_enq > hard_cap) { mln_set_error(ctx, "map_solve: the device solver did not terminate"); return MLN_ERR_NOCONV; }
    if (batch < 16 && f->h_state->gate == MLN_GATE_F64) batch = std::min(batch, 6);
  }
  const SolverState st = *f->h_state;
  fit_precond_saved_free(f);
  f->n_start_halvings = st.n_shrink;
  std::vector<double> tr;
  const int n_done = st.n_eval < 512 ? st.n_eval : 512;
  if (n_done > 0) {
    tr.resize((size_t)4 * n_done);
    MLN_HIP(ctx, hipMemcpy(tr.data(), f->sv.trace, sizeof(double) * 4 * n_done, hipMemcpyDeviceToHost));
    for (int i = 0; i < n_done && timing; ++i) {
      const int gcode = (int)tr[4 * i + 3] & 15, lvl = (int)tr[4 * i + 3] >> 4;
      const bool was32 = (gcode & 3) == MLN_GATE_F32, was_sub = gcode == MLN_GATE_SUB;
      int slot = i;
      for (const auto& sh : slot_shift) if (i >= sh.first) slot = i + sh.second;
      if (3 * (slot + 1) > (int)f->evs.size()) continue;
      float ms = 0.f;
      if (hipEventElapsedTime(&ms, f->evs[3 * slot + (was32 ? 0 : 1)], f->evs[3 * slot + (was32 ? 1 : 2)]) != hipSuccess) continue;
      if (was_sub) {
        f->times_sub += 1e-3 * ms; f->evals_sub += 1;
        f->sub_pass_equiv += 1.0 / (double)((lvl >= 0 && lvl < (int)sub_strides.size()) ? sub_strides[lvl] : 1);
      }
      else if (was32) { f->times32 += 1e-3 * ms; f->evals32 += 1; }
      else { f->times[5] += 1e-3 * ms; f->times[6] += 1.0; f->times[7] = (double)f->n * (double)f->ldl * 8.0; }
    }
    if (trace_lvl >= 2)
      for (int i = 0; i < n_done; ++i)
        fprintf(stderr, "[eval %d] %s mode=%d t=%.3g f=%.15g\n", i, ((int)tr[4 * i + 3] & 15) == MLN_GATE_F32 ? "f32" : (((int)tr[4 * i + 3] & 15) == MLN_GATE_F32C ? "f32c" : (((int)tr[4 * i + 3] & 15) == MLN_GATE_SUB ? (((int)tr[4 * i + 3] >> 4) ? "sub1" : "sub0") : "f64")),
                (int)tr[4 * i + 2], tr[4 * i + 1], tr[4 * i]);
  }
  {
    if (f->kspace) {
      GemvTri g1{f->P, f->ldl, m, f->sv.u, f->d_w_cached, nullptr, 1, m, m, 0, 0, nullptr};
      MLN_TRY(launch_gemv_tri(ctx, g1));
      MLN_TRY(fit_ensure_lp(f, false));
// ... 86 lines not shown
```

mellon_amd/csrc/cov_kernels.hip:

```cpp
#include <cstdlib>
#include <vector>

#include "mln_internal.h"
#include "rowmin_f16.h"
#include "predict_rows_prod.h"
#include "cov_program.h"
#include "cov_rows.h"
#include "cov_rows_q.h"
#include "mln_options.h"

namespace {

constexpr int TM = 64, TN = covrows::TN, DK = 16, PADT = 4;
constexpr int NNS = covrows::NNS;

__device__ __forceinline__ double leaf_value(const DevLeaf& lf, double xx, double yy, double xy) {
  const double inv_ls = lf.alpha_inv_ls[1];
  if (lf.kind == MLN_K_LINEAR) return xy * inv_ls;
  double sq = xx - 2.0 * xy + yy + 1e-12;
  double dist = sqrt(fmax(sq, 0.0));
  switch (lf.kind) {
    case MLN_K_DISTANCE: return dist * inv_ls;
    case MLN_K_MATERN32: {
      double r = 1.7320508075688772 * dist * inv_ls;
// ... 841 lines not shown
      const double l = s1, r = s0;
      s0 = (op == MLN_OP_ADD) ? (l + r) : (op == MLN_OP_MUL) ? (l * r) : pow(l, r);
      s1 = s2;
      --sp;
    }
  }
  out[i] = s0;
}

__global__ void k_row_sumsq(const double* __restrict__ T, int64_t ld, int64_t rows, int64_t cols,
                            const double* __restrict__ base, double sign, double* __restrict__ out) {
  const int64_t i = blockIdx.x;
  if (i >= rows) return;
  __shared__ double red[256];
  double s = 0.0;
  for (int64_t j = threadIdx.x; j < cols; j += 256) { const double v = T[i * ld + j]; s = fma(v, v, s); }
  red[threadIdx.x] = s;
  __syncthreads();
  for (int off = 128; off > 0; off >>= 1) {
    if (threadIdx.x < off) red[threadIdx.x] += red[threadIdx.x + off];
    __syncthreads();
  }
  if (threadIdx.x == 0) out[i] = (base ? base[i] : 0.0) + sign * red[0];
}

int sqnorms(mln_ctx* ctx, const DevCov& cov, const double* x, int64_t n, int d, double* xx) {
  if (n == 0) return MLN_OK;
  hipLaunchKernelGGL(k_row_sqnorms, dim3((unsigned)((n + 31) / 32)), dim3(256), 0, ctx->stream, cov, x, n, d, xx);
  MLN_HIP(ctx, hipGetLastError());
  return MLN_OK;
}

}

constexpr int64_t ROWS_PAD = 3 * 64;
static int pad_rows(mln_ctx* ctx, const double* src, int64_t rows, int64_t cols, double* dst) {
  MLN_HIP(ctx, hipMemcpyAsync(dst, src, sizeof(double) * (size_t)(rows * cols), hipMemcpyDeviceToDevice, ctx->stream));
  MLN_HIP(ctx, hipMemsetAsync(dst + rows * cols, 0, sizeof(double) * (size_t)(ROWS_PAD * cols), ctx->stream));
  return MLN_OK;
}

int launch_kernel_matrix(mln_ctx* ctx, const DevCov& cov, const double* x, int64_t n, const double* y,
                         int64_t m, int d, double* out, int64_t ldo, double add_diag, float* out32, int q32) {
  if (n == 0 || m == 0) return MLN_OK;
  double* norms = nullptr;
  const int64_t mp = m + ROWS_PAD;
  MLN_TRY(mln_scratch(ctx, sizeof(double) * ((size_t)cov.n_leaves * (size_t)(n + mp) + (size_t)(mp * d)), (void**)&norms));
  double* xx = norms;
  double* yy = norms + (int64_t)cov.n_leaves * n;
  double* ypad = yy + (int64_t)cov.n_leaves * mp;
  MLN_TRY(sqnorms(ctx, cov, x, n, d, xx));
  MLN_TRY(sqnorms(ctx, cov, y, m, d, yy));
  const int64_t tiles_n = (ldo + TN - 1) / TN, tiles_m = (n + TM - 1) / TM;
  const int64_t nblk = tiles_n * tiles_m;
  if (nblk > 0x7fffffffLL) { mln_set_error(ctx, "kernel matrix too large for one launch"); return MLN_ERR_UNSUPPORTED; }
  const bool single = (cov.n_toks == 1);
  bool contiguous = single && cov.leaves[0].ndims == d;
  if (contiguous)
    for (int k = 0; k < d; ++k) contiguous = contiguous && cov.dims[cov.leaves[0].dims_off + k] == k;
  static const bool no_rows_env = mln_experiment("MELLON_AMD_KM_NO_ROWS") != nullptr;
  const bool no_rows = no_rows_env || ldo > m + 64;
  if (contiguous && !no_rows && d <= 64 && n >= 4096 && m >= 256 && cov.leaves[0].kind != MLN_K_LINEAR &&
      cov.leaves[0].kind != MLN_K_DISTANCE && cov.leaves[0].kind != MLN_K_RATQUAD && (!out32 || q32)) {
    MLN_TRY(pad_rows(ctx, y, m, d, ypad));
    MLN_HIP(ctx, hipMemsetAsync(yy + m, 0, sizeof(double) * (size_t)ROWS_PAD, ctx->stream));
    MLN_TRY(launch_kernel_matrix_rows_q(ctx, cov, x, n, ypad, m, d, xx, yy, out, ldo, add_diag, out32, q32));
  } else if (!no_rows && n >= 4096 && m >= 256 && (!out32 || q32) && predict_rows_prod_eligible(cov, d)) {
    MLN_TRY(pad_rows(ctx, y, m, d, ypad));
    MLN_HIP(ctx, hipMemsetAsync(yy + m, 0, sizeof(double) * (size_t)ROWS_PAD, ctx->stream));
    MLN_TRY(launch_kernel_matrix_rows_prod(ctx, cov, x, n, ypad, m, d, xx, yy, out, ldo, add_diag, out32, q32));
  } else if (contiguous && n * m >= 4096)
    hipLaunchKernelGGL(k_kernel_matrix_mfma, dim3((unsigned)nblk), dim3(256), 0, ctx->stream, cov, x, n, y, m, d,
                       xx, yy, out, ldo, add_diag, tiles_n, out32, q32);
  else if (single)
    hipLaunchKernelGGL(k_kernel_matrix<true>, dim3((unsigned)nblk), dim3(256), 0, ctx->stream, cov, x, n, y, m, d,
                       xx, yy, out, ldo, add_diag, tiles_n, out32, q32);
  else
    hipLaunchKernelGGL(k_kernel_matrix<false>, dim3((unsigned)nblk), dim3(256), 0, ctx->stream, cov, x, n, y, m, d,
                       xx, yy, out, ldo, add_diag, tiles_n, out32, q32);
  MLN_HIP(ctx, hipGetLastError());
  return MLN_OK;
}

int launch_predict_mean1(mln_ctx* ctx, const DevCov& cov, const double* x, int64_t n, const double* y,
                         int64_t m, int d, const double* w, double mu, double* out) {
  if (n == 0) return MLN_OK;
  double* norms = nullptr;
  const int64_t mp = m + ROWS_PAD;
  MLN_TRY(mln_scratch(ctx, sizeof(double) * ((size_t)cov.n_leaves * (size_t)(n + mp) + (size_t)(mp * (d + 1))), (void**)&norms));
  double* xx = norms;
  double* yy = norms + (int64_t)cov.n_leaves * n;
  double* ypad = yy + (int64_t)cov.n_leaves * mp;
  double* wpad = ypad + mp * d;
  MLN_TRY(sqnorms(ctx, cov, x, n, d, xx));
  MLN_TRY(sqnorms(ctx, cov, y, m, d, yy));
  const int64_t nblk = (n + TM - 1) / TM;
  const bool single = (cov.n_toks == 1);
  bool contiguous = single && cov.leaves[0].ndims == d;
  if (contiguous)
    for (int k = 0; k < d; ++k) contiguous = contiguous && cov.dims[cov.leaves[0].dims_off + k] == k;
  if (contiguous && d <= 64 && n >= 4096 && m >= 256 && cov.leaves[0].kind != MLN_K_LINEAR &&
      cov.leaves[0].kind != MLN_K_DISTANCE) {
    MLN_TRY(pad_rows(ctx, y, m, d, ypad));
    MLN_TRY(pad_rows(ctx, w, m, 1, wpad));
    MLN_HIP(ctx, hipMemsetAsync(yy + m, 0, sizeof(double) * (size_t)ROWS_PAD, ctx->stream));
    MLN_TRY(launch_predict_mean_rows(ctx, cov, x, n, ypad, m, d, xx, yy, wpad, mu, out));
  } else if (n >= 4096 && m >= 256 && predict_rows_prod_eligible(cov, d)) {
    MLN_TRY(pad_rows(ctx, y, m, d, ypad));
    MLN_TRY(pad_rows(ctx, w, m, 1, wpad));
    MLN_HIP(ctx, hipMemsetAsync(yy + m, 0, sizeof(double) * (size_t)ROWS_PAD, ctx->stream));
    MLN_TRY(launch_predict_mean_rows_prod(ctx, cov, x, n, ypad, m, d, xx, yy, wpad, mu, out));
  } else if (contiguous && n * m >= 4096)
    hipLaunchKernelGGL(k_predict_mean_mfma, dim3((unsigned)nblk), dim3(256), 0, ctx->stream, cov, x, n, y, m, d,
                       xx, yy, w, mu, out);
  else if (single)
    hipLaunchKernelGGL(k_predict_mean1<true>, dim3((unsigned)nblk), dim3(256), 0, ctx->stream, cov, x, n, y, m, d,
                       xx, yy, w, mu, out);
  else
    hipLaunchKernelGGL(k_predict_mean1<false>, dim3((unsigned)nblk), dim3(256), 0, ctx->stream, cov, x, n, y, m, d,
                       xx, yy, w, mu, out);
  MLN_HIP(ctx, hipGetLastError());
  return MLN_OK;
}

int launch_nn_distances_exact(mln_ctx* ctx, const double* x, int64_t n, const double* y, int64_t m, int d,
                              int64_t self_offset, const int64_t* excl, double* out) {
  if (n == 0) return MLN_OK;
  double* norms = nullptr;
  MLN_HIP(ctx, mln_dmalloc((void**)&norms, sizeof(double) * (size_t)(n + m)));
  double* xx = norms;
  double* yy = norms + n;
  hipLaunchKernelGGL(k_row_sqnorms_all, dim3((unsigned)((n + 255) / 256)), dim3(256), 0, ctx->stream, x, n, d, xx);
  hipLaunchKernelGGL(k_row_sqnorms_all, dim3((unsigned)((m + 255) / 256)), dim3(256), 0, ctx->stream, y, m, d, yy);
  if (d <= 64 && n * m >= 4096)
    hipLaunchKernelGGL(k_nn_distances_mfma, dim3((unsigned)((n + 127) / 128)), dim3(512), 0, ctx->stream, x, n, y, m, d,
                       xx, yy, self_offset, excl, out);
  else
    hipLaunchKernelGGL(k_nn_distances, dim3((unsigned)((n + TM - 1) / TM)), dim3(256), 0, ctx->stream, x, n, y, m, d,
                       xx, yy, self_offset, excl, out);
  hipError_t e = hipGetLastError();
  (void)hipStreamSynchronize(ctx->stream);
  (void)mln_dfree(norms);
  if (e != hipSuccess) return mln_hip_fail(ctx, e, "nn_distances", __FILE__, __LINE__);
  return MLN_OK;
}

int launch_nn_distances(mln_ctx* ctx, const double* x, int64_t n, const double* y, int64_t m, int d,
                        int64_t self_offset, double* out) {
  if (n == 0) return MLN_OK;
  const char* e_on = std::getenv("MELLON_AMD_NN_PREFILTER");
  const char* e_min = std::getenv("MELLON_AMD_NN_PREFILTER_MIN");
  const bool prefilter = !(e_on && std::atoi(e_on) == 0);
  const int64_t min_pairs = e_min ? std::atoll(e_min) : ((int64_t)1 << 26);
  if (prefilter && d <= 64 && m >= 2 && n * m >= min_pairs && m < 2147483647LL)
    return nn_distances_prefiltered(ctx, x, n, y, m, d, self_offset, out, nullptr);
  return launch_nn_distances_exact(ctx, x, n, y, m, d, self_offset, nullptr, out);
}

int launch_cov_diag(mln_ctx* ctx, const DevCov& cov, const double* x, int64_t n, int d, double* out) {
  if (n == 0) return MLN_OK;
  hipLaunchKernelGGL(k_cov_diag, dim3((unsigned)((n + 255) / 256)), dim3(256), 0, ctx->stream, cov, x, n, d, out);
  MLN_HIP(ctx, hipGetLastError());
  return MLN_OK;
}

int launch_row_sumsq(mln_ctx* ctx, const double* T, int64_t ld, int64_t rows, int64_t cols, const double* base,
// ... 166 lines not shown
```

mellon_amd/csrc/cov_rows.h:

```cpp
#pragma once
#include "mln_core.h"

typedef double v4d_t __attribute__((ext_vector_type(4)));

namespace covrows {
constexpr int TN = 64;
constexpr int NNS = 65;
}

int launch_kernel_matrix_rows(mln_ctx* ctx, const DevCov& cov, const double* x, int64_t n, const double* y, int64_t m,
                              int d, const double* xx, const double* yy, double* out, int64_t ldo, double add_diag,
                              float* out32);
int launch_predict_mean_rows(mln_ctx* ctx, const DevCov& cov, const double* x, int64_t n, const double* y, int64_t m,
                             int d, const double* xx, const double* yy, const double* w, double mu, double* out);
```

mellon_amd/csrc/cov_rows.hip:

```cpp
#include "cov_rows.h"
#include "cov_rows_q.h"

#define MLN_ROWS_DECL(NAME)                                                                                     \
  int NAME(mln_ctx* ctx, const DevCov& cov, const double* x, int64_t n, const double* y, int64_t m, int d,      \
           const double* xx, const double* yy, double* out, int64_t ldo, double add_diag, float* out32, int q32);
MLN_ROWS_DECL(launch_kernel_matrix_rows_matern32)
MLN_ROWS_DECL(launch_kernel_matrix_rows_matern52)
MLN_ROWS_DECL(launch_kernel_matrix_rows_expquad)
MLN_ROWS_DECL(launch_kernel_matrix_rows_exponential)
#undef MLN_ROWS_DECL

int launch_kernel_matrix_rows(mln_ctx* ctx, const DevCov& cov, const double* x, int64_t n, const double* y, int64_t m,
                              int d, const double* xx, const double* yy, double* out, int64_t ldo, double add_diag,
                              float* out32) {
  return launch_kernel_matrix_rows_q(ctx, cov, x, n, y, m, d, xx, yy, out, ldo, add_diag, out32, 0);
}

int launch_kernel_matrix_rows_q(mln_ctx* ctx, const DevCov& cov, const double* x, int64_t n, const double* y, int64_t m,
                                int d, const double* xx, const double* yy, double* out, int64_t ldo, double add_diag,
                                float* out32, int q32) {
  switch (cov.leaves[0].kind) {
    case MLN_K_MATERN32: return launch_kernel_matrix_rows_matern32(ctx, cov, x, n, y, m, d, xx, yy, out, ldo, add_diag, out32, q32);
    case MLN_K_MATERN52: return launch_kernel_matrix_rows_matern52(ctx, cov, x, n, y, m, d, xx, yy, out, ldo, add_diag, out32, q32);
    case MLN_K_EXPQUAD: return launch_kernel_matrix_rows_expquad(ctx, cov, x, n, y, m, d, xx, yy, out, ldo, add_diag, out32, q32);
    case MLN_K_EXPONENTIAL: return launch_kernel_matrix_rows_exponential(ctx, cov, x, n, y, m, d, xx, yy, out, ldo, add_diag, out32, q32);
    default:
      mln_set_error(ctx, "persistent-row kernel matrix: unsupported leaf kind");
      return MLN_ERR_UNSUPPORTED;
  }
}
```

mellon_amd/csrc/cov_rows_impl.h:

```cpp
#include <type_traits>

#pragma once
#include "cov_rows.h"
#include "cov_epilogue.h"

namespace {
using covrows::NNS;
using covrows::TN;

__device__ __forceinline__ void lds_barrier() {
  asm volatile("s_waitcnt lgkmcnt(0)\n\ts_barrier" ::: "memory");
}

__device__ __forceinline__ float surrogate_bits(double v, int) {
  return __uint_as_float((unsigned)__double2loint(fmin(v, 0x1.fffffffep-1) + 0x1p20));
}

template <int KIND>
__device__ __forceinline__ double leaf_value_k(double m2, double xs, double ys, double xy) {
  return covepi::leaf_value_s<KIND>(fmax(fma(m2, xy, xs) + ys, 1e-300));
}

template <int KIND, bool HAS32, int KSTEPS>
__global__ __launch_bounds__(512) void k_kernel_matrix_rows(DevCov cov, const double* __restrict__ x, int64_t n,
                                                            const double* __restrict__ y, int64_t m, int d,
                                                            const double* __restrict__ xx,
                                                            const double* __restrict__ yy,
                                                            double* __restrict__ out, int64_t ldo, double add_diag,
                                                            float* __restrict__ out32, int q32) {
  constexpr int YB = TN * NNS + 512;
  __shared__ double ys[2][YB];
  __shared__ double yn[3][512];
  constexpr int NST = (TN * 4 * KSTEPS + 511) / 512;
  constexpr int EPI_VALU = (HAS32 ? 32 : 29) * 16 + 8;
  const double c2 = covepi::sq_scale<KIND>(cov.leaves[0]), m2 = -2.0 * c2;
  const int tid = threadIdx.x;
  const int lane = tid & 63, wave = tid >> 6, li = lane & 15, lk = lane >> 4;
  const int64_t row0 = (int64_t)blockIdx.x * 128 + wave * 16;
  double a[16];
  {
    const int64_t ar = (row0 + li < n) ? row0 + li : n - 1;
#pragma unroll
    for (int ks = 0; ks < 16; ++ks) {
      const int k = 4 * ks + lk;
      a[ks] = (k < d) ? x[ar * d + k] : 0.0;
    }
  }
  double xr[4];
#pragma unroll
  for (int r = 0; r < 4; ++r) {
    const int64_t row = row0 + lk + 4 * r;
    xr[r] = (row < n) ? c2 * (xx[row] + 1e-12) : 0.0;
  }
  double* const out_wg = out + (int64_t)blockIdx.x * 128 * ldo;
  float* const out32_wg = HAS32 ? out32 + (int64_t)blockIdx.x * 128 * ldo : nullptr;
  unsigned lrowb[4], lrowb32[4];
#pragma unroll
  for (int r = 0; r < 4; ++r) {
    lrowb[r] = ((unsigned)(wave * 16 + lk + 4 * r) * (unsigned)ldo + (unsigned)li) * 8u;
    lrowb32[r] = lrowb[r] >> 1;
  }
  for (int e = tid; e < 2 * YB; e += 512) (&ys[0][0])[e] = 0.0;
  __syncthreads();
  const int cnt = TN * d;
  unsigned goffb[NST];
  double* dst[NST];
#pragma unroll
  for (int i = 0; i < NST; ++i) {
    const int e = tid + 512 * i;
    const int r = e / d, k = e - r * d;
    goffb[i] = (e < cnt) ? (unsigned)e * 8u : 0u;
    dst[i] = (e < cnt) ? &ys[0][r * NNS + k] : &ys[0][TN * NNS + tid];
  }
  const unsigned nb = (unsigned)(tid & (TN - 1)) * 8u;
  double sreg[NST], snorm = 0.0;
  auto stage_load = [&](int64_t tile) {
    const char* yt = (const char*)(y + tile * TN * d);
#pragma unroll
    for (int i = 0; i < NST; ++i) sreg[i] = *(const double*)(yt + goffb[i]);
    snorm = *(const double*)((const char*)(yy + tile * TN) + nb);
  };
  auto stage_store = [&](int par, int nbuf) {
#pragma unroll
    for (int i = 0; i < NST; ++i) dst[i][par * YB] = sreg[i];
    yn[nbuf][tid] = c2 * snorm;
  };
  auto mma = [&](int buf, v4d_t (&acc)[4]) {
    const double* yb = &ys[buf][li * NNS + lk];
#pragma unroll
    for (int t = 0; t < 4; ++t) acc[t] = v4d_t{0.0, 0.0, 0.0, 0.0};
#pragma unroll
    for (int ks = 0; ks < KSTEPS; ++ks)
#pragma unroll
      for (int t = 0; t < 4; ++t)
        acc[t] = __builtin_amdgcn_mfma_f64_16x16x4f64(a[ks], yb[16 * t * NNS + 4 * ks], acc[t], 0, 0, 0);
  };
  const int64_t ntiles = (ldo + TN - 1) / TN;
  const bool interior_rows = (int64_t)blockIdx.x * 128 + 128 <= n;
  stage_load(0); stage_store(0, 0);
  if (ntiles > 1) { stage_load(1); stage_store(1, 1); }
  __syncthreads();
  v4d_t accA[4], accB[4];
  mma(0, accA);
  lds_barrier();
  auto step = [&](int64_t t, v4d_t (&cur)[4], v4d_t (&nxt)[4], int par, int ncur, auto fast_tag) {
    constexpr bool FAST = decltype(fast_tag)::value;
    const int64_t t2 = FAST ? (t + 2) : ((t + 2 < ntiles) ? (t + 2) : (ntiles - 1));
    stage_load(t2);
    mma(par ^ 1, nxt);
    const int64_t col0 = t * TN;
    if (FAST) {
      char* const ob = (char*)(out_wg + col0);
      char* const ob32 = HAS32 ? (char*)(out32_wg + col0) : nullptr;
#pragma unroll
      for (int tt = 0; tt < 4; ++tt) {
        const double yc = yn[ncur][16 * tt + li];
#pragma unroll
        for (int r = 0; r < 4; ++r) {
          const double v = leaf_value_k<KIND>(m2, xr[r], yc, cur[tt][r]);
          *(double*)(ob + 128 * tt + lrowb[r]) = v;
          if (HAS32) *(float*)(ob32 + 64 * tt + lrowb32[r]) = surrogate_bits(v, q32);
        }
      }
#pragma unroll
      for (int i = 0; i < 4 * KSTEPS; ++i) {
        __builtin_amdgcn_sched_group_barrier(0x008, 1, 0);
        __builtin_amdgcn_sched_group_barrier(0x002, EPI_VALU / (4 * KSTEPS), 0);
      }
    } else {
#pragma unroll
      for (int tt = 0; tt < 4; ++tt) {
        const int64_t c = col0 + 16 * tt + li;
        const double yc = yn[ncur][16 * tt + li];
#pragma unroll
        for (int r = 0; r < 4; ++r) {
          const int64_t row = row0 + lk + 4 * r;
          if (row < n && c < ldo) {
            const double v = (c < m) ? leaf_value_k<KIND>(m2, xr[r], yc, cur[tt][r]) + ((row == c) ? add_diag : 0.0) : 0.0;
            out[row * ldo + c] = v;
            if (HAS32) out32[row * ldo + c] = surrogate_bits(v, q32);
          }
        }
      }
    }
    stage_store(par, (ncur == 0) ? 2 : ncur - 1);
    lds_barrier();
  };
  const int64_t n_fast = (interior_rows && add_diag == 0.0) ? (m / TN) : 0;
  int64_t t = 0;
  int nc = 0;
  for (; t + 2 <= n_fast; t += 2) {
    step(t, accA, accB, 0, nc, std::true_type{});
    nc = (nc == 2) ? 0 : nc + 1;
    step(t + 1, accB, accA, 1, nc, std::true_type{});
    nc = (nc == 2) ? 0 : nc + 1;
  }
  for (; t < ntiles; ++t) {
    step(t, accA, accB, (int)(t & 1), nc, std::false_type{});
    nc = (nc == 2) ? 0 : nc + 1;
#pragma unroll
    for (int tt = 0; tt < 4; ++tt) accA[tt] = accB[tt];
  }
}

}


template <int KIND>
static int launch_rows_kind(mln_ctx* ctx, const DevCov& cov, const double* x, int64_t n, const double* y, int64_t m, int d,
                            const double* xx, const double* yy, double* out, int64_t ldo, double add_diag, float* out32,
                            int q32) {
  const dim3 grid((unsigned)((n + 127) / 128)), block(512);
#define MLN_KM_ROWS2(KS)                                                                                              \
  if (out32) hipLaunchKernelGGL((k_kernel_matrix_rows<KIND, true, KS>), grid, block, 0, ctx->stream, cov, x, n, y, m, d, \
                                xx, yy, out, ldo, add_diag, out32, q32);                                             \
  else hipLaunchKernelGGL((k_kernel_matrix_rows<KIND, false, KS>), grid, block, 0, ctx->stream, cov, x, n, y, m, d, xx,  \
                          yy, out, ldo, add_diag, out32, q32);
  if (d <= 32) { MLN_KM_ROWS2(8) }
  else if (d <= 52) { MLN_KM_ROWS2(13) }
  else { MLN_KM_ROWS2(16) }
#undef MLN_KM_ROWS2
  MLN_HIP(ctx, hipGetLastError());
  return MLN_OK;
}

#define MLN_DEFINE_ROWS_KIND(NAME, KIND)                                                                                 \
  int NAME(mln_ctx* ctx, const DevCov& cov, const double* x, int64_t n, const double* y, int64_t m, int d,               \
           const double* xx, const double* yy, double* out, int64_t ldo, double add_diag, float* out32, int q32) {       \
    return launch_rows_kind<KIND>(ctx, cov, x, n, y, m, d, xx, yy, out, ldo, add_diag, out32, q32);                      \
  }
```

mellon_amd/csrc/cov_rows_q.h:

```cpp
#pragma once
#include "mln_core.h"
int launch_kernel_matrix_rows_q(mln_ctx* ctx, const DevCov& cov, const double* x, int64_t n, const double* y, int64_t m,
                                int d, const double* xx, const double* yy, double* out, int64_t ldo, double add_diag,
                                float* out32, int q32);
```

mellon_amd/csrc/dimensionality.hip:

```cpp
#include "api_internal.h"

namespace {

constexpr int KNN_WG = 256;
constexpr int KNN_QB = 64;
constexpr int KNN_CB = 64;
constexpr int KNN_DC = 16;
constexpr int KNN_KMAX = 64;

struct KnnArgs {
  const double* x; int64_t n;
  const double* y; int64_t m;
  int d, k;
  int exclude; int64_t self_offset;
  double* dist; int64_t* idx;
};

__global__ __launch_bounds__(KNN_WG) void k_knn(KnnArgs a) {
  __shared__ double qs[KNN_DC][KNN_QB];
  __shared__ double cs[KNN_DC][KNN_CB];
  __shared__ double topd[KNN_QB][KNN_KMAX];
  __shared__ int topi[KNN_QB][KNN_KMAX];
  __shared__ double cand_d[KNN_QB][KNN_CB];
  __shared__ int cand_i[KNN_QB][KNN_CB];
// ... 472 lines not shown
  MLN_TRY(o.init(ctx, dist, (size_t)n * k));
  int64_t* di = nullptr;
  DevScratch si(ctx);
  if (idx) {
    if (is_device_ptr(idx)) di = idx;
    else { MLN_HIP(ctx, si.alloc(sizeof(int64_t) * (size_t)n * k)); di = reinterpret_cast<int64_t*>(si.p); }
  }
  KnnArgs a{dx.dev, n, dy.dev, m, d, k, exclude ? 1 : 0, self_offset, o.dev, di};
  hipLaunchKernelGGL(k_knn, dim3((unsigned)((n + KNN_QB - 1) / KNN_QB)), dim3(KNN_WG), 0, ctx->stream, a);
  MLN_HIP(ctx, hipGetLastError());
  if (idx && di != idx)
    MLN_HIP(ctx, hipMemcpyAsync(idx, di, sizeof(int64_t) * (size_t)n * k, hipMemcpyDeviceToHost, ctx->stream));
  return o.commit();
}

extern "C" int mln_local_dimensionality(mln_ctx* ctx, const double* x, int64_t n, int32_t d, const int64_t* nbr,
                                        int64_t q, int32_t k, double* out) {
  if (!ctx) return MLN_ERR_ARG;
  if (n < 1 || q < 0 || d < 1) { mln_set_error(ctx, "local_dimensionality: bad shape"); return MLN_ERR_SHAPE; }
  if (k < 2 || k > LD_KMAX) { mln_set_error(ctx, "local_dimensionality: k must lie in [2, 64]"); return MLN_ERR_SHAPE; }
  if (q == 0) return MLN_OK;
  if (!x || !nbr || !out) return MLN_ERR_ARG;
  MLN_HIP(ctx, hipSetDevice(ctx->device));
  DevIn dx;
  DevOut o;
  MLN_TRY(dx.init(ctx, x, (size_t)n * d));
  MLN_TRY(o.init(ctx, out, (size_t)q));
  const int64_t* dn = nbr;
  DevScratch sn(ctx);
  if (!is_device_ptr(nbr)) {
    MLN_HIP(ctx, sn.alloc(sizeof(int64_t) * (size_t)q * k));
    MLN_HIP(ctx, hipMemcpyAsync(sn.p, nbr, sizeof(int64_t) * (size_t)q * k, hipMemcpyHostToDevice, ctx->stream));
    dn = reinterpret_cast<const int64_t*>(sn.p);
  }
  hipLaunchKernelGGL(k_local_dim, dim3((unsigned)q), dim3(LD_WG), 0, ctx->stream, dx.dev, n, (int)d, dn, (int)k, o.dev);
  MLN_HIP(ctx, hipGetLastError());
  return o.commit();
}

static int dim_one_pass_ok(mln_fit* f) {
  if (f->ldl > DIM_MAX_LD) {
    mln_set_error(f->ctx, "dimensionality objective: one pass covers at most " + std::to_string(DIM_MAX_LD) +
                              " columns of L (this fit has " + std::to_string(f->m) + ")");
    return MLN_ERR_UNSUPPORTED;
  }
  return MLN_OK;
}

extern "C" int mln_fit_set_dim_likelihood(mln_fit* f, const double* ell, int32_t k, double mu_dim, double mu_dens) {
  if (!f || (f->n > 0 && !ell)) return MLN_ERR_ARG;
  mln_ctx* ctx = f->ctx;
  if (k < 1 || k > 64) { mln_set_error(ctx, "set_dim_likelihood: k must lie in [1, 64]"); return MLN_ERR_SHAPE; }
  MLN_TRY(dim_one_pass_ok(f));
  MLN_HIP(ctx, hipSetDevice(ctx->device));
  const size_t ld = (size_t)f->ldl;
  if (f->dim_ell && f->dim_k != k) { (void)hipStreamSynchronize(ctx->stream); (void)mln_dfree(f->dim_ell); f->dim_ell = nullptr; }
  if (!f->dim_ell) MLN_HIP(ctx, mln_dmalloc((void**)&f->dim_ell, sizeof(double) * (size_t)(f->n > 0 ? f->n : 1) * k));
  if (!f->dim_part) MLN_HIP(ctx, mln_dmalloc((void**)&f->dim_part, sizeof(double) * 4 * ld * (size_t)f->n_wg_cap));
  if (!f->dim_z) {
    MLN_HIP(ctx, mln_dmalloc((void**)&f->dim_z, sizeof(double) * 4 * ld));
    MLN_HIP(ctx, hipMemsetAsync(f->dim_z, 0, sizeof(double) * 4 * ld, ctx->stream));
  }
  if (!f->dim_out) MLN_HIP(ctx, mln_dmalloc((void**)&f->dim_out, sizeof(double) * (2 + 4 * ld)));
  if (f->n > 0)
    MLN_HIP(ctx, hipMemcpyAsync(f->dim_ell, ell, sizeof(double) * (size_t)f->n * k, hipMemcpyDefault, ctx->stream));
  MLN_HIP(ctx, hipStreamSynchronize(ctx->stream));
  f->dim_k = k;
  f->mu_dim = mu_dim;
  f->mu_dens = mu_dens;
  return MLN_OK;
}

extern "C" int mln_dim_objective(mln_fit* f, const double* z, double* loss, double* grad, double* hess_diag) {
  if (!f || !z || !loss || !grad) return MLN_ERR_ARG;
  mln_ctx* ctx = f->ctx;
  if (!f->dim_ell) { mln_set_error(ctx, "mln_fit_set_dim_likelihood has not been called"); return MLN_ERR_ARG; }
  if (hess_diag && f->kspace) {
    mln_set_error(ctx, "the Hessian diagonal needs the explicit factor L: prepare the fit without MLN_FIT_IMPLICIT");
    return MLN_ERR_UNSUPPORTED;
  }
  MLN_TRY(dim_one_pass_ok(f));
  MLN_HIP(ctx, hipSetDevice(ctx->device));
  MLN_TRY(fit_ensure_lp(f));
  const int64_t m = f->m, ld = f->ldl;
  std::vector<double> zh((size_t)(2 * m));
  MLN_HIP(ctx, hipMemcpyAsync(zh.data(), z, sizeof(double) * 2 * m, hipMemcpyDefault, ctx->stream));
  MLN_HIP(ctx, hipMemcpyAsync(f->dim_z, z, sizeof(double) * m, hipMemcpyDefault, ctx->stream));
  MLN_HIP(ctx, hipMemcpyAsync(f->dim_z + ld, z + m, sizeof(double) * m, hipMemcpyDefault, ctx->stream));
  DimArgs a{};
  a.L = f->L; a.ldl = ld; a.n = f->n; a.m = m;
  a.z = f->dim_z;
  if (f->kspace) {
    double* w = f->dim_z + 2 * ld;
    MLN_HIP(ctx, hipMemcpyAsync(w, f->dim_z, sizeof(double) * 2 * ld, hipMemcpyDeviceToDevice, ctx->stream));
    MLN_TRY(triinv_solve_left_T(ctx, f->tri, w, 1, 1));
    MLN_TRY(triinv_solve_left_T(ctx, f->tri, w + ld, 1, 1));
    a.z = w;
  }
  a.ell = f->dim_ell; a.k = f->dim_k; a.mu_dim = f->mu_dim; a.mu_dens = f->mu_dens;
  a.part = f->dim_part; a.part_loss = f->part_loss; a.n_wg = f->n_wg;
  const bool hess = hess_diag != nullptr;
  if (f->n > 0) {
    MLN_TRY(launch_dim_objective(ctx, a, false));
    if (hess) MLN_TRY(launch_dim_objective(ctx, a, true));
  }
  ObjArgs r{};
  r.n = f->n; r.m = 2 * ld; r.m_pad = 4 * ld; r.n_wg = f->n > 0 ? f->n_wg : 0;
  r.part_grad = f->dim_part; r.part_hess = hess ? f->dim_part + 2 * ld : nullptr; r.part_loss = f->part_loss;
  const int64_t nout = 1 + 2 * ld + (hess ? 2 * ld : 0);
  MLN_TRY(launch_reduce_obj(ctx, r, f->dim_out));
  MLN_TRY(dev_allreduce(ctx, f->dim_out, nout));
  if (f->kspace) {
    MLN_TRY(triinv_solve_left(ctx, f->tri, f->dim_out + 1, 1, 1));
    MLN_TRY(triinv_solve_left(ctx, f->tri, f->dim_out + 1 + ld, 1, 1));
  }
  std::vector<double> out((size_t)nout);
  MLN_HIP(ctx, hipMemcpyAsync(out.data(), f->dim_out, sizeof(double) * nout, hipMemcpyDeviceToHost, ctx->stream));
  MLN_HIP(ctx, hipStreamSynchronize(ctx->stream));
  double zz = 0.0;
  for (int64_t j = 0; j < 2 * m; ++j) zz += zh[j] * zh[j];
  const double lv = out[0] + 0.5 * zz + std::log(2.0 * M_PI);
  *loss = std::isfinite(lv) ? lv : HUGE_VAL;
  std::vector<double> tmp;
  double* gh = grad;
  if (is_device_ptr(grad)) { tmp.resize(2 * m); gh = tmp.data(); }
  for (int64_t j = 0; j < m; ++j) {
    gh[j] = out[1 + j] + zh[j];
    gh[m + j] = out[1 + ld + j] + zh[m + j];
  }
  if (gh != grad) MLN_HIP(ctx, hipMemcpy(grad, gh, sizeof(double) * 2 * m, hipMemcpyHostToDevice));
  if (hess) {
    std::vector<double> th;
    double* hh = hess_diag;
    if (is_device_ptr(hess_diag)) { th.resize(2 * m); hh = th.data(); }
    for (int64_t j = 0; j < m; ++j) {
      hh[j] = out[1 + 2 * ld + j] + 1.0;
      hh[m + j] = out[1 + 3 * ld + j] + 1.0;
    }
    if (hh != hess_diag) MLN_HIP(ctx, hipMemcpy(hess_diag, hh, sizeof(double) * 2 * m, hipMemcpyHostToDevice));
  }
  return MLN_OK;
}
```

mellon_amd/csrc/mln_internal.h:

```cpp
#pragma once
#include "mln_core.h"

int comm_allreduce(mln_ctx* ctx, double* dev, int64_t count);
int comm_bcast0(mln_ctx* ctx, double* dev, int64_t count);
int comm_allgather(mln_ctx* ctx, const double* send, double* recv, int64_t count);
void comm_release(mln_ctx* ctx);

int launch_kernel_matrix(mln_ctx* ctx, const DevCov& cov, const double* x, int64_t n, const double* y,
                         int64_t m, int d, double* out, int64_t ldo, double add_diag, float* out32 = nullptr,
                         int q32 = 0);
__device__ __forceinline__ float mln_surrogate_bits(double v, int q32) {
  const unsigned fx = (unsigned)fmin(fma(v, 4294967296.0, 0.5), 4294967295.0);
  return q32 ? __uint_as_float(fx) : (float)v;
}
int launch_predict_mean1(mln_ctx* ctx, const DevCov& cov, const double* x, int64_t n, const double* y,
                         int64_t m, int d, const double* w, double mu, double* out);

int launch_cov_diag(mln_ctx* ctx, const DevCov& cov, const double* x, int64_t n, int d, double* out);
int launch_row_sumsq(mln_ctx* ctx, const double* T, int64_t ld, int64_t rows, int64_t cols, const double* base,
                     double sign, double* out);
int launch_nn_distances(mln_ctx* ctx, const double* x, int64_t n, const double* y, int64_t m, int d,
                        int64_t self_offset, double* out);

struct GemmArgs {
  const double* A; int64_t lda;
  const double* B; int64_t ldb;
  double* C; int64_t ldc;
  int64_t M, N, K;
  double alpha, beta;
  int ta, tb;
  int lower_only;
  int split_k; int64_t c_split_stride;
  int kmode;
  int batch; int64_t bsa, bsb, bsc;
};
int launch_dgemm(mln_ctx* ctx, const GemmArgs& g);
int launch_sum_partials(mln_ctx* ctx, const double* parts, int n_parts, int64_t stride, double* out,
                        int64_t count, double beta);

int dev_cholesky_lower(mln_ctx* ctx, double* A, int64_t m, int64_t lda);
int dev_cholesky_lower2(mln_ctx* ctx, double* A, double* A2, int64_t m, int64_t lda, int* bad);
int launch_add_diag(mln_ctx* ctx, double* A, int64_t m, int64_t lda, double v);
int launch_symmetrize_from_lower(mln_ctx* ctx, double* A, int64_t m, int64_t lda);
int dev_sym_rank_above(mln_ctx* ctx, double* A, int64_t m, int64_t ld, double tol2, int64_t* rank, double* lambda_max);
int dev_sym_rank_above_ldl(mln_ctx* ctx, double* A, int64_t m, int64_t ld, double tol2, int64_t* rank, double* lambda_max, bool* ok);
int gram_i8_splits(int64_t rows, int64_t m);
int launch_gram_i8(mln_ctx* ctx, const double* K, int64_t ldk, int64_t rows, int64_t m, double alpha, double* parts,
                   int64_t ldg, int64_t part_stride, int n_splits);
int launch_axpby(mln_ctx* ctx, int64_t n, double a, const double* x, double b, double* y);

int launch_kernel_grad(mln_ctx* ctx, const DevCov& cov, const double* x, int64_t n, const double* y, int64_t m,
                       int d, int exact_denominator, double* out);
int launch_predict_gradient_gemm(mln_ctx* ctx, const DevCov& cov, const double* x, int64_t n, const double* c,
                                 int64_t m, int d, const double* w, double* out);
int launch_predict_gradient_gemm_multi(mln_ctx* ctx, const DevCov& cov, const double* x, int64_t n, const double* c,
                                       int64_t m, int d, const double* w, double* out);
int launch_predict_hessian(mln_ctx* ctx, const DevCov& cov, const double* x, int64_t n, const double* c, int64_t m,
                           int d, const double* w, double* out);
int launch_predict_gradient(mln_ctx* ctx, const DevCov& cov, const double* x, int64_t n, const double* c, int64_t m,
                            int d, const double* w, double* out);

int dev_eigh(mln_ctx* ctx, const double* A, int64_t m, int64_t lda, double* w_host, double* Vrows, int64_t ldv,
             int* n_sweeps_out);
```

mellon_amd/csrc/objective.h:

```cpp
#pragma once
#include "mln_core.h"

struct ObjArgs {
  const double* L; int64_t ldl; int64_t n; int64_t m;
  const double* z; const double* V; const double* Vdr; double mu;
  double* part_grad;
  double* part_hess;
  double* part_loss;
  const double* weights;
  double* f_out;
  int n_wg; int64_t m_pad;
  const float* L32;
  int l32_fixed;
  double* f_keep[2];
  const int* f_slot;
  const double* cap;
  int* over_flag;
  const int* gate;
  int gate_want;
  int64_t row_stride;
  int64_t row_first;
  double out_scale;
  const int* gate2;
  int gate2_want;
  int64_t seg_cols;
  int64_t seg_left;
  int f_accum;
};
enum { MLN_GATE_F64 = 0, MLN_GATE_F32 = 1, MLN_GATE_DONE = 2, MLN_GATE_SUB = 3, MLN_GATE_F32C = 5, MLN_GATE_PAUSE = 6 };
int objective_max_m();
int objective_max_m_one_pass();
bool objective_can_keep_f(int64_t n, int n_wg);
int launch_to_f32(mln_ctx* ctx, const double* src, float* dst, int64_t count);
int launch_objective(mln_ctx* ctx, const ObjArgs& a);
int launch_reduce_obj(mln_ctx* ctx, const ObjArgs& a, double* out_loss_grad );
int launch_reduce_obj2(mln_ctx* ctx, const ObjArgs& a, double* out_loss, double* out_grad);
int launch_gemv_rows(mln_ctx* ctx, const double* M, int64_t ld, int64_t rows, int64_t cols, const double* x,
                     double* y);
int launch_gemv_rows_tri(mln_ctx* ctx, const double* M, int64_t ld, int64_t rows, const double* x, double* y,
                         int upper, int64_t blk, int64_t ncol, int64_t seg);
struct GemvTri {
  const double* M; int64_t ld; int64_t rows;
  const double* x; double* y; double* y2;
  int upper;
  int64_t blk, ncol, mseg, xseg;
  const int* gate;
  const double* xadd;
};
int launch_gemv_tri(mln_ctx* ctx, const GemvTri& g);
```

mellon_amd/csrc/objective.hip:

```cpp
#include <cstdlib>

#include "mln_internal.h"
#include "objective.h"
#include "mln_options.h"

namespace {

constexpr int WG = 512;
constexpr int MLN_FSTAGE = 6144;
enum { MODE_OBJ = 0, MODE_OBJ_HESS = 1, MODE_GEMVT = 2, MODE_FONLY = 3 };

typedef double d2 __attribute__((ext_vector_type(2)));

__device__ __forceinline__ void lds_store_f64(double* base, int idx, double v) {
  const unsigned addr = (unsigned)(uintptr_t)(__attribute__((address_space(3))) double*)base + 8u * (unsigned)idx;
  asm volatile("ds_write_b64 %0, %1" : : "v"(addr), "v"(v));
}

struct RowMap { int64_t r0, rs; __device__ __forceinline__ int64_t operator()(int64_t i) const { return r0 + i * rs; } };
__device__ __forceinline__ RowMap row_map(const ObjArgs& a) { return RowMap{a.row_first, a.row_stride > 0 ? a.row_stride : 1}; }

template <int CPT, int R>
__device__ __forceinline__ void load_rows(const d2* __restrict__ L2, int64_t ld2, int64_t row, int64_t row_end,
                                          unsigned tid, d2 (&v)[R][CPT], const RowMap rm, unsigned lim) {
#pragma unroll
  for (int r = 0; r < R; ++r) {
    const bool rok = (row + r) < row_end;
    const d2* rowp = L2 + rm(rok ? (row + r) : row) * ld2;
#pragma unroll
    for (int c = 0; c < CPT; ++c) {
      unsigned off = (unsigned)c * WG + tid;
      off = (off < lim) ? off : lim - 1u;
      v[r][c] = __builtin_nontemporal_load(rowp + off);
    }
  }
}


template <int R>
__device__ __forceinline__ void load_lik(const ObjArgs& a, int64_t row, double (&pv)[2][R]) {
  const RowMap rm = row_map(a);
#pragma unroll
  for (int r = 0; r < R; ++r) {
    const int64_t i = rm((row + r < a.n) ? (row + r) : (a.n - 1));
    pv[0][r] = a.V[i];
    pv[1][r] = a.Vdr[i];
  }
}

template <int R>
__device__ __forceinline__ void load_lik_vec(const ObjArgs& a, int64_t row, int tid, double (&pv)[2][R]) {
  const RowMap rm = row_map(a);
  const int lane = tid & 63;
  const int64_t want = row + (lane < R ? lane : R - 1);
  const int64_t i = rm((want < a.n) ? want : (a.n - 1));
  pv[0][0] = a.V[i];
  pv[1][0] = a.Vdr[i];
}

__device__ __forceinline__ double read_lane_f64(double v, int lane) {
  const int lo = __builtin_amdgcn_readlane(__double2loint(v), lane);
  const int hi = __builtin_amdgcn_readlane(__double2hiint(v), lane);
  return __hiloint2double(hi, lo);
}

template <int R>
__device__ __forceinline__ double transposed_wave_sum(double (&v)[R], int lane) {
  constexpr int K = (R == 16) ? 4 : (R == 8) ? 3 : (R == 4) ? 2 : (R == 2) ? 1 : 0;
  static_assert((1 << K) == R, "R must be a power of two <= 16");
#pragma unroll
  for (int st = 0; st < K; ++st) {
    const int half = R >> (st + 1), mask = 32 >> st;
    const bool upper = (lane & mask) != 0;
#pragma unroll
    for (int i = 0; i < half; ++i) {
      const double send = upper ? v[i] : v[i + half];
      const double keep = upper ? v[i + half] : v[i];
      v[i] = keep + __shfl_xor(send, mask, 64);
    }
  }
  double s = v[0];
#pragma unroll
  for (int mask = 32 >> K; mask > 0; mask >>= 1) s += __shfl_xor(s, mask, 64);
  return s;
}

template <int CPT, int R, int MODE, bool KEEP, bool VEC = false>
// ... 28 lines not shown
#pragma unroll
    for (int w = 0; w < 8; ++w) sr += red[par][w][rl];
    const bool rok = lane < R && (row + rl) < row_end;
    const double f = sr + a.mu;
    const double Vi = pv[0][0];
    const double tt = f + Vi;
    const bool over = tt > capv;
    const double ex = rok ? exp(over ? capv : tt) : 0.0;
    const double dc = over ? (tt - capv) : 0.0;
    const double e = ex * fma(dc, fma(0.5, dc, 1.0), 1.0);
    const double cf = rok ? (over ? fma(ex, dc, ex - 1.0) : ex - 1.0) : 0.0;
    if (wave == 0 && rok) loss -= (f + pv[1][0]) - e;
    any_over += (wave == 0 && rok && over) ? 1 : 0;
    if (KEEP) lds_store_f64(fstage, (wave == 0 && rok) ? (int)(row + rl - fbase) : (MLN_FSTAGE + tid), f);
#pragma unroll
    for (int r = 0; r < R; ++r) {
      coef[r] = read_lane_f64(cf, r);
      aexp[r] = (MODE == MODE_OBJ_HESS) ? read_lane_f64(ex, r) : 0.0;
    }
  } else {
    double dot[R];
#pragma unroll
    for (int r = 0; r < R; ++r) {
      double s = 0.0;
#pragma unroll
      for (int c = 0; c < CPT; ++c) {
        s = fma(v[r][c].x, z[c].x, s);
        s = fma(v[r][c].y, z[c].y, s);
      }
#pragma unroll
      for (int off = 32; off > 0; off >>= 1) s += __shfl_xor(s, off, 64);
      dot[r] = s;
    }
    const int wave = tid >> 6;
    if ((tid & 63) == 0) {
#pragma unroll
      for (int r = 0; r < R; ++r) red[par][wave][r] = dot[r];
    }
    __syncthreads();
#pragma unroll
    for (int r = 0; r < R; ++r) {
      double s = 0.0;
#pragma unroll
      for (int w = 0; w < 8; ++w) s += red[par][w][r];
      const bool rok = (row + r) < row_end;
      const double f = s + a.mu;
      if (MODE == MODE_FONLY) {
        if (rok && tid == 0) a.f_out[row + r] = a.f_accum ? (s + a.f_out[row + r]) : f;
        coef[r] = 0.0;
        aexp[r] = 0.0;
      } else {
        const double Vi = KEEP ? pv[0][r] : (rok ? a.V[rm(row + r)] : 0.0);
        const double tt = f + Vi;
        const bool over = tt > capv;
        const double ex = rok ? exp(over ? capv : tt) : 0.0;
        const double dc = over ? (tt - capv) : 0.0;
        const double e = ex * fma(dc, fma(0.5, dc, 1.0), 1.0);
        aexp[r] = ex;
        coef[r] = rok ? (over ? fma(ex, dc, ex - 1.0) : ex - 1.0) : 0.0;
        if (KEEP) { if (tid == 0 && rok) loss -= (f + pv[1][r]) - e; }
        else if (tid == 0 && rok) loss -= (f + a.Vdr[rm(row + r)]) - e;
        any_over += (tid == 0 && rok && over) ? 1 : 0;
        if (KEEP) lds_store_f64(fstage, (tid == 0 && rok) ? (int)(row + r - fbase) : (MLN_FSTAGE + tid), f);
      }
    }
  }
  if (MODE != MODE_FONLY) {
#pragma unroll
    for (int r = 0; r < R; ++r) {
#pragma unroll
      for (int c = 0; c < CPT; ++c) {
        g[c].x = fma(coef[r], v[r][c].x, g[c].x);
        g[c].y = fma(coef[r], v[r][c].y, g[c].y);
        if (MODE == MODE_OBJ_HESS) {
          h[c].x = fma(aexp[r] * v[r][c].x, v[r][c].x, h[c].x);
          h[c].y = fma(aexp[r] * v[r][c].y, v[r][c].y, h[c].y);
        }
      }
    }
  }
}

template <int CPT, int R, int MODE, bool KEEP = false, bool VEC = false>
__global__ __launch_bounds__(WG) void k_objective(ObjArgs a) {
  if (a.gate && (*a.gate & 3) != a.gate_want) return;
  if (a.gate2 && *a.gate2 != a.gate2_want) return;
  __shared__ double red[2][8][R];
  const int tid = threadIdx.x;
  const int64_t ld2 = a.ldl / 2;
  const d2* __restrict__ L2 = reinterpret_cast<const d2*>(a.L);
  const int64_t nsteps = (a.n + R - 1) / R;
  const int64_t per = (nsteps + a.n_wg - 1) / a.n_wg;
  const int64_t s_beg = (int64_t)blockIdx.x * per;
  int64_t s_end = s_beg + per;
  if (s_end > nsteps) s_end = nsteps;

  d2 z[CPT], g[CPT], h[CPT];
#pragma unroll
  for (int c = 0; c < CPT; ++c) {
    const int64_t col = 2 * ((int64_t)c * WG + tid);
    z[c] = (d2){0.0, 0.0};
    if (MODE != MODE_GEMVT) {
      if (col < a.m) z[c].x = a.z[col];
      if (col + 1 < a.m) z[c].y = a.z[col + 1];
    }
    g[c] = (d2){0.0, 0.0};
    h[c] = (d2){0.0, 0.0};
  }
  double loss = 0.0;
  int any_over = 0;
  const double capv = a.cap ? *a.cap : __builtin_inf();
  __shared__ double fstage[KEEP ? (MLN_FSTAGE + WG) : 1];
  const int64_t fbase = s_beg * R;
  d2 va[R][CPT], vb[R][CPT];
  const int64_t s_last = s_end - 1;
  double pa[2][R], pb[2][R];
  const RowMap rm = row_map(a);
  const unsigned lim = a.seg_cols > 0 ? (unsigned)(a.seg_left / 2) : (unsigned)ld2;
  auto lik = [&](int64_t r0, double (&pv)[2][R]) { if (VEC) load_lik_vec<R>(a, r0, tid, pv); else load_lik<R>(a, r0, pv); };
  constexpr bool PRE = KEEP || (VEC && (MODE == MODE_OBJ || MODE == MODE_OBJ_HESS));
  if (s_beg < s_end) { load_rows<CPT, R>(L2, ld2, s_beg * R, a.n, tid, va, rm, lim); if (PRE) lik(s_beg * R, pa); }
  for (int64_t s = s_beg; s < s_end; s += 2) {
    const int64_t s1 = (s + 1 < s_end) ? s + 1 : s_last, s2 = (s + 2 < s_end) ? s + 2 : s_last;
    load_rows<CPT, R>(L2, ld2, s1 * R, a.n, tid, vb, rm, lim);
    if (PRE) lik(s1 * R, pb);
    process_rows<CPT, R, MODE, KEEP, VEC>(a, s * R, a.n, tid, 0, va, z, g, h, loss, red, fstage, fbase, pa, capv, any_over);
    load_rows<CPT, R>(L2, ld2, s2 * R, a.n, tid, va, rm, lim);
    if (PRE) lik(s2 * R, pa);
    if (s + 1 < s_end) process_rows<CPT, R, MODE, KEEP, VEC>(a, (s + 1) * R, a.n, tid, 1, vb, z, g, h, loss, red, fstage, fbase, pb, capv, any_over);
  }
  if (any_over && a.over_flag) atomicAdd(a.over_flag, any_over);
  if (KEEP) {
    __syncthreads();
    double* fo = a.f_keep[1 - *a.f_slot];
    const int64_t r_beg = s_beg * R, r_end = (s_end * R < a.n) ? s_end * R : a.n;
    for (int64_t i = r_beg + tid; i < r_end; i += WG) fo[i] = fstage[i - r_beg];
  }
  if (MODE != MODE_FONLY) {
    double* pg = a.part_grad + (int64_t)blockIdx.x * a.m_pad;
    const int64_t store_lim = a.seg_cols > 0 ? ((a.seg_cols + 1) & ~(int64_t)1) : a.m_pad;
    const double osc = a.out_scale != 0.0 ? a.out_scale : 1.0;
#pragma unroll
    for (int c = 0; c < CPT; ++c) {
      const int64_t col = 2 * ((int64_t)c * WG + tid);
      if (col < store_lim) *reinterpret_cast<d2*>(pg + col) = (d2){g[c].x * osc, g[c].y * osc};
    }
    if (MODE == MODE_OBJ_HESS) {
      double* ph = a.part_hess + (int64_t)blockIdx.x * a.m_pad;
#pragma unroll
      for (int c = 0; c < CPT; ++c) {
        const int64_t col = 2 * ((int64_t)c * WG + tid);
        if (col < a.m_pad) *reinterpret_cast<d2*>(ph + col) = h[c];
      }
    }
    if (VEC) {
#pragma unroll
      for (int off = 32; off > 0; off >>= 1) loss += __shfl_xor(loss, off, 64);
    }
    if (tid == 0 && a.part_loss) a.part_loss[blockIdx.x] = loss * osc;
  }
}

typedef float f4 __attribute__((ext_vector_type(4)));

template <int CQ, int R, int NW>
__device__ __forceinline__ void load_rows32(const f4* __restrict__ L4, int64_t ld4, int64_t row, int64_t row_end,
                                            unsigned tid, f4 (&v)[R][CQ], const RowMap rm) {
#pragma unroll
  for (int r = 0; r < R; ++r) {
    const bool rok = (row + r) < row_end;
    const f4* rowp = L4 + rm(rok ? (row + r) : row) * ld4;
#pragma unroll
    for (int c = 0; c < CQ; ++c) {
      unsigned off = (unsigned)c * (64 * NW) + tid;
      off = (off < (unsigned)ld4) ? off : (unsigned)ld4 - 1u;
      v[r][c] = __builtin_nontemporal_load(rowp + off);
    }
  }
}

template <bool FIXED>
__device__ __forceinline__ double elem32(float v) {
  return FIXED ? (double)__float_as_uint(v) : (double)v;
}

template <int CQ, int R, bool GEMVT, bool KEEP, int NW, bool FIXED, bool VEC = false>
__device__ __forceinline__ void process_rows32(const ObjArgs& a, int64_t row, int64_t row_end, int tid, int par,
                                               const f4 (&v)[R][CQ], const double (&z)[CQ][4], double (&g)[CQ][4],
                                               double& loss, double (*red)[NW][R], double* fstage, int64_t fbase,
                                               const double (&pv)[2][R], double capv, double ecap, int& any_over) {
  double coef[R], dot[R];
  const RowMap rm = row_map(a);
  if (GEMVT) {
#pragma unroll
    for (int r = 0; r < R; ++r) coef[r] = (row + r < row_end) ? a.weights[rm(row + r)] : 0.0;
#pragma unroll
    for (int r = 0; r < R; ++r) {
#pragma unroll
      for (int c = 0; c < CQ; ++c) {
        g[c][0] = fma(coef[r], elem32<FIXED>(v[r][c].x), g[c][0]);
        g[c][1] = fma(coef[r], elem32<FIXED>(v[r][c].y), g[c][1]);
        g[c][2] = fma(coef[r], elem32<FIXED>(v[r][c].z), g[c][2]);
        g[c][3] = fma(coef[r], elem32<FIXED>(v[r][c].w), g[c][3]);
      }
    }
    return;
  }
  if constexpr (VEC) {
#pragma unroll
    for (int r = 0; r < R; ++r) {
      double s = 0.0;
#pragma unroll
      for (int c = 0; c < CQ; ++c) {
        s = fma(elem32<FIXED>(v[r][c].x), z[c][0], s);
        s = fma(elem32<FIXED>(v[r][c].y), z[c][1], s);
        s = fma(elem32<FIXED>(v[r][c].z), z[c][2], s);
        s = fma(elem32<FIXED>(v[r][c].w), z[c][3], s);
      }
      dot[r] = s;
    }
    const int wave = tid >> 6, lane = tid & 63;
    constexpr int GRP = 64 / R;
    const double tot = transposed_wave_sum<R>(dot, lane);
    if ((lane & (GRP - 1)) == 0) red[par][wave][lane / GRP] = tot;
    __syncthreads();
    const int rl = lane < R ? lane : R - 1;
    double sr = 0.0;
#pragma unroll
    for (int w = 0; w < NW; ++w) sr += red[par][w][rl];
    const bool rok = lane < R && (row + rl) < row_end;
    const double f = sr + a.mu;
    const double Vi = pv[0][0];
    const double tt = f + Vi;
    const bool over = tt > capv;
    const double ex = exp(over ? capv : tt);
    const double dc = over ? (tt - capv) : 0.0;
    const double e = rok ? ex * fma(dc, fma(0.5, dc, 1.0), 1.0) : 0.0;
    const double cf = rok ? (over ? fma(ex, dc, ex - 1.0) : ex - 1.0) : 0.0;
    if (wave == 0 && rok) loss -= (f + pv[1][0]) - e;
    any_over += (wave == 0 && rok && over) ? 1 : 0;
    if (KEEP) lds_store_f64(fstage, (wave == 0 && rok) ? (int)(row + rl - fbase) : (MLN_FSTAGE + tid), f);
#pragma unroll
// ... 357 lines not shown
      s.weights = gemvt ? a.weights : coef;
      s.part_grad = a.part_grad + c0; s.part_hess = nullptr; s.part_loss = nullptr; s.f_out = nullptr; s.f_slot = nullptr;
      s.seg_cols = s.m; s.seg_left = a.ldl - c0;
      rc = launch_objective(ctx, s);
    }
  }
  if (ftmp) { (void)hipStreamSynchronize(ctx->stream); (void)mln_dfree(ftmp); }
  return rc;
}

int objective_max_m_one_pass() { return (int)MLN_SEG; }
bool objective_can_keep_f(int64_t n, int n_wg) { return n_wg > 0 && (n + n_wg - 1) / n_wg + 16 <= MLN_FSTAGE; }

int launch_objective(mln_ctx* ctx, const ObjArgs& a) {
  if (a.ldl % 2 != 0) { mln_set_error(ctx, "objective: leading dimension of L must be even"); return MLN_ERR_ARG; }
  if (a.seg_cols == 0 && a.m > MLN_SEG) return launch_objective_wide(ctx, a);
  int mode = MODE_OBJ;
  if (a.weights) mode = MODE_GEMVT;
  else if (a.f_out) mode = MODE_FONLY;
  else if (a.part_hess) mode = MODE_OBJ_HESS;
  if (a.L32 && (mode == MODE_OBJ || mode == MODE_GEMVT) && a.ldl % 4 == 0) {
    const int cq = (int)((a.ldl / 4 + WG - 1) / WG);
    const bool vec32 = mode == MODE_OBJ;
    switch (cq) {
      case 1: return vec32 ? launch_f32<1, 8, true>(ctx, a) : launch_f32<1, 8>(ctx, a);
      case 2: return vec32 ? launch_f32<2, 4, true>(ctx, a) : launch_f32<2, 4>(ctx, a);
      case 3:
        return vec32 ? launch_f32<3, 2, true>(ctx, a) : launch_f32<3, 3>(ctx, a);
      default: return launch_f32<4, 2>(ctx, a);
    }
  }
  const int64_t pairs = a.seg_cols > 0 ? (a.seg_cols + 1) / 2 : a.ldl / 2;
  const int cpt = (int)((pairs + WG - 1) / WG);
  const bool vec = mode == MODE_OBJ || mode == MODE_OBJ_HESS;
  switch (cpt) {
    case 1: return vec ? launch_mode<1, 8, true>(ctx, a, mode) : launch_mode<1, 8>(ctx, a, mode);
    case 2: return vec ? launch_mode<2, 8, true>(ctx, a, mode) : launch_mode<2, 5>(ctx, a, mode);
    case 3: return vec ? launch_mode<3, 4, true>(ctx, a, mode) : launch_mode<3, 3>(ctx, a, mode);
    case 4: return launch_mode<4, 2>(ctx, a, mode);
    case 5: return launch_mode<5, 2>(ctx, a, mode);
    case 6: return launch_mode<6, 2>(ctx, a, mode);
    case 7:
    case 8: return launch_mode<8, 1>(ctx, a, mode);
    default:
      mln_set_error(ctx, "objective: m > 8192 landmarks is not supported by this build");
      return MLN_ERR_UNSUPPORTED;
  }
}

int launch_gemv_rows(mln_ctx* ctx, const double* M, int64_t ld, int64_t rows, int64_t cols, const double* x,
                     double* y) {
  if (rows <= 0) return MLN_OK;
  if ((ld & 1) || ((uintptr_t)M & 15) || ((uintptr_t)x & 15)) { mln_set_error(ctx, "gemv_rows: unaligned operands"); return MLN_ERR_ARG; }
  hipLaunchKernelGGL(k_gemv_rows, dim3((unsigned)((rows + 3) / 4)), dim3(256), 0, ctx->stream, M, ld, rows, cols, x, y);
  MLN_HIP(ctx, hipGetLastError());
  return MLN_OK;
}

int launch_gemv_tri(mln_ctx* ctx, const GemvTri& g) {
  if (g.rows <= 0) return MLN_OK;
  if ((g.ld & 1) || (g.mseg & 1) || (g.xseg & 1) || ((uintptr_t)g.M & 15) || ((uintptr_t)g.x & 15)) {
    mln_set_error(ctx, "gemv_rows_tri: unaligned operands");
    return MLN_ERR_ARG;
  }
  hipLaunchKernelGGL(k_gemv_rows_tri, dim3((unsigned)((g.rows + 3) / 4)), dim3(256), 0, ctx->stream, g);
  MLN_HIP(ctx, hipGetLastError());
  return MLN_OK;
}

int launch_gemv_rows_tri(mln_ctx* ctx, const double* M, int64_t ld, int64_t rows, const double* x, double* y,
                         int upper, int64_t blk, int64_t ncol, int64_t seg) {
  GemvTri g{M, ld, rows, x, y, nullptr, upper, blk, ncol, seg, seg, nullptr};
  return launch_gemv_tri(ctx, g);
}

int launch_reduce_obj2(mln_ctx* ctx, const ObjArgs& a, double* out_loss, double* out_grad) {
  hipLaunchKernelGGL(k_reduce_obj, dim3((unsigned)((a.m + 15) / 16)), dim3(256), 0, ctx->stream, a, out_loss, out_grad,
                     a.part_hess ? 1 : 0);
  MLN_HIP(ctx, hipGetLastError());
  return MLN_OK;
}

int launch_reduce_obj(mln_ctx* ctx, const ObjArgs& a, double* out) { return launch_reduce_obj2(ctx, a, out, out + 1); }
```

mellon_amd/csrc/objective_batch.hip:

```cpp
#include "api_internal.h"

namespace {

typedef double v4d __attribute__((ext_vector_type(4)));
typedef double d2 __attribute__((ext_vector_type(2)));

constexpr int BT = 256;
constexpr int BK = 16;
constexpr int A_LD = BK + 4;
constexpr int B_LD = BT + 16;
constexpr int S_CHUNK = 64;

template <int NT> struct SkinnyLd { static constexpr int v = (NT % 2) ? 16 * NT : 16 * NT + 16; };

template <int NT>
__global__ __launch_bounds__(256, 2) void k_batch_forward(const double* __restrict__ B, int64_t ldb, int64_t n, int64_t kdim,
                                                         const double* __restrict__ W, const double* __restrict__ V,
                                                         const double* __restrict__ Vdr, double mu, double* __restrict__ A1,
                                                         double* __restrict__ part_loss) {
  constexpr int SP = 16 * NT, WLD = SkinnyLd<NT>::v;
  __shared__ __attribute__((aligned(16))) double As[BT][A_LD];
  __shared__ double Ws[BK][WLD];
  __shared__ double lred[4][SP];
  const int t = threadIdx.x, lane = t & 63, wave = t >> 6, lk = lane >> 4, li = lane & 15;
// ... 128 lines not shown
    for (int kk = 0; kk < BK; kk += 4) {
      double a[4], b[NT];
#pragma unroll
      for (int i = 0; i < 4; ++i) a[i] = Bs[kk + lk][wave * 64 + i * 16 + li];
#pragma unroll
      for (int j = 0; j < NT; ++j) b[j] = Cs[kk + lk][j * 16 + li];
#pragma unroll
      for (int i = 0; i < 4; ++i)
#pragma unroll
        for (int j = 0; j < NT; ++j) acc[i][j] = __builtin_amdgcn_mfma_f64_16x16x4f64(a[i], b[j], acc[i][j], 0, 0, 0);
    }
  }
  double* out = part + (int64_t)blockIdx.y * ldb * SP;
#pragma unroll
  for (int i = 0; i < 4; ++i)
#pragma unroll
    for (int r = 0; r < 4; ++r) {
      const int64_t c = c0 + wave * 64 + i * 16 + lk + 4 * r;
      if (c < ldb) {
#pragma unroll
        for (int j = 0; j < NT; ++j) out[c * SP + j * 16 + li] = acc[i][j][r];
      }
    }
}

__global__ __launch_bounds__(256) void k_batch_sum(const double* __restrict__ parts, int n_parts, int64_t stride,
                                                   double* __restrict__ out, int64_t count) {
  const int64_t i = (int64_t)blockIdx.x * 256 + threadIdx.x;
  if (i >= count) return;
  double s = 0.0;
  for (int p = 0; p < n_parts; ++p) s += parts[(int64_t)p * stride + i];
  out[i] = s;
}

__global__ __launch_bounds__(256) void k_batch_loss_sum(const double* __restrict__ part_loss, int64_t n_tiles, int SP,
                                                        double* __restrict__ out) {
  __shared__ double red[256];
  const int s = blockIdx.x, t = threadIdx.x;
  double l = 0.0;
  for (int64_t w = t; w < n_tiles; w += 256) l += part_loss[w * SP + s];
  red[t] = l;
  __syncthreads();
  for (int off = 128; off > 0; off >>= 1) {
    if (t < off) red[t] += red[t + off];
    __syncthreads();
  }
  if (t == 0) out[s] = red[0];
}

__global__ __launch_bounds__(256) void k_batch_z_to_w(const double* __restrict__ Z, int S, int64_t m, int SP, int64_t rows,
                                                      double* __restrict__ W) {
  const int64_t i = (int64_t)blockIdx.x * 256 + threadIdx.x;
  if (i >= rows * SP) return;
  const int64_t j = i / SP;
  const int s = (int)(i % SP);
  W[i] = (j < m && s < S) ? Z[(int64_t)s * m + j] : 0.0;
}

__global__ __launch_bounds__(256) void k_batch_finish(const double* __restrict__ Z, int64_t m, int SP,
                                                      const double* __restrict__ lik, const double* __restrict__ G,
                                                      double* __restrict__ loss, double* __restrict__ grad) {
  __shared__ double red[256];
  const int s = blockIdx.x, t = threadIdx.x;
  const double* z = Z + (int64_t)s * m;
  double zz = 0.0;
  for (int64_t j = t; j < m; j += 256) {
    const double v = z[j];
    zz = fma(v, v, zz);
    grad[(int64_t)s * m + j] = G[j * SP + s] + v;
  }
  red[t] = zz;
  __syncthreads();
  for (int off = 128; off > 0; off >>= 1) {
    if (t < off) red[t] += red[t + off];
    __syncthreads();
  }
  if (t == 0) loss[s] = lik[s] + 0.5 * red[0] + 0.5 * (double)m * 1.8378770664093453;
}

template <int NT>
int launch_batch(mln_fit* f, const double* W, double* A1, double* part_loss, int64_t n_tiles, double* part, int n_ranges,
                 int64_t rows_per_range) {
  mln_ctx* ctx = f->ctx;
  hipLaunchKernelGGL((k_batch_forward<NT>), dim3((unsigned)n_tiles), dim3(256), 0, ctx->stream, f->L, f->ldl, f->n, f->ldl, W,
                     f->V, f->Vdr, f->mu, A1, part_loss);
  MLN_HIP(ctx, hipGetLastError());
  const unsigned col_blocks = (unsigned)((f->ldl + BT - 1) / BT);
  hipLaunchKernelGGL((k_batch_backward<NT>), dim3(col_blocks, (unsigned)n_ranges), dim3(256), 0, ctx->stream, f->L, f->ldl,
                     f->n, rows_per_range, A1, part);
  MLN_HIP(ctx, hipGetLastError());
  return MLN_OK;
}

}

extern "C" int mln_objective_batch(mln_fit* f, const double* Z, int32_t S, double* loss, double* grad) {
  if (!f || !Z || !loss || !grad || S < 1) return MLN_ERR_ARG;
  mln_ctx* ctx = f->ctx;
  if (!f->V) { mln_set_error(ctx, "mln_fit_set_likelihood has not been called"); return MLN_ERR_ARG; }
  MLN_HIP(ctx, hipSetDevice(ctx->device));
  MLN_TRY(fit_ensure_lp(f));
  const int64_t m = f->m, ldl = f->ldl, n = f->n;
  const int sp_max = 16 * (int)((std::min<int64_t>(S, S_CHUNK) + 15) / 16);
  const int64_t col_blocks = (ldl + BT - 1) / BT;
  const int64_t n_cu = ctx->n_cu > 0 ? ctx->n_cu : 256;
  int64_t n_ranges = std::max<int64_t>(1, (4 * n_cu) / col_blocks);
  n_ranges = std::min<int64_t>(n_ranges, std::max<int64_t>(1, (n + 255) / 256));
  const int64_t rows_per_range = std::max<int64_t>(16, (((n + n_ranges - 1) / n_ranges) + 15) / 16 * 16);
  const int64_t n_tiles = (n + BT - 1) / BT;
  const size_t c_z = (size_t)sp_max * m, c_w = (size_t)ldl * sp_max, c_lg = (size_t)sp_max * (1 + ldl),
               c_a1 = (size_t)std::max<int64_t>(n, 1) * sp_max, c_pl = (size_t)std::max<int64_t>(n_tiles, 1) * sp_max,
               c_part = (size_t)n_ranges * ldl * sp_max, c_out = (size_t)sp_max * (1 + m);
  auto even = [](size_t c) { return (c + 1) & ~(size_t)1; };
  DevScratch sc(ctx);
  MLN_HIP(ctx, sc.alloc(sizeof(double) * (even(c_z) + even(c_w) + even(c_lg) + even(c_a1) + even(c_pl) + even(c_part) + even(c_out))));
  double* d_Z = sc.p;
  double* d_W = d_Z + even(c_z);
  double* d_lg = d_W + even(c_w);
  double* d_A1 = d_lg + even(c_lg);
  double* d_pl = d_A1 + even(c_a1);
  double* d_part = d_pl + even(c_pl);
  double* d_out = d_part + even(c_part);

  for (int32_t s0 = 0; s0 < S; s0 += S_CHUNK) {
    const int Sc = std::min<int32_t>(S_CHUNK, S - s0);
    const int NT = (Sc + 15) / 16, SP = 16 * NT;
    double* d_lik = d_lg;
    double* d_G = d_lg + SP;
    MLN_HIP(ctx, hipMemcpyAsync(d_Z, Z + (int64_t)s0 * m, sizeof(double) * (size_t)Sc * m, hipMemcpyDefault, ctx->stream));
    hipLaunchKernelGGL(k_batch_z_to_w, dim3((unsigned)((ldl * SP + 255) / 256)), dim3(256), 0, ctx->stream, d_Z, Sc, m, SP, ldl, d_W);
    MLN_HIP(ctx, hipGetLastError());
    if (f->kspace) MLN_TRY(triinv_solve_left_T(ctx, f->tri, d_W, SP, SP));
    if (n > 0) {
      int rc = MLN_OK;
      switch (NT) {
        case 1: rc = launch_batch<1>(f, d_W, d_A1, d_pl, n_tiles, d_part, (int)n_ranges, rows_per_range); break;
        case 2: rc = launch_batch<2>(f, d_W, d_A1, d_pl, n_tiles, d_part, (int)n_ranges, rows_per_range); break;
        case 3: rc = launch_batch<3>(f, d_W, d_A1, d_pl, n_tiles, d_part, (int)n_ranges, rows_per_range); break;
        default: rc = launch_batch<4>(f, d_W, d_A1, d_pl, n_tiles, d_part, (int)n_ranges, rows_per_range); break;
      }
      MLN_TRY(rc);
      hipLaunchKernelGGL(k_batch_loss_sum, dim3((unsigned)SP), dim3(256), 0, ctx->stream, d_pl, n_tiles, SP, d_lik);
      MLN_HIP(ctx, hipGetLastError());
      hipLaunchKernelGGL(k_batch_sum, dim3((unsigned)((ldl * SP + 255) / 256)), dim3(256), 0, ctx->stream, d_part, (int)n_ranges, ldl * SP, d_G,
                         ldl * SP);
      MLN_HIP(ctx, hipGetLastError());
    } else {
      MLN_HIP(ctx, hipMemsetAsync(d_lg, 0, sizeof(double) * (size_t)SP * (1 + ldl), ctx->stream));
    }
    MLN_TRY(dev_allreduce(ctx, d_lg, (int64_t)SP * (1 + ldl)));
    if (f->kspace) MLN_TRY(triinv_solve_left(ctx, f->tri, d_G, SP, SP));
    double* o_loss = d_out;
    double* o_grad = d_out + SP;
    hipLaunchKernelGGL(k_batch_finish, dim3((unsigned)Sc), dim3(256), 0, ctx->stream, d_Z, m, SP, d_lik, d_G, o_loss, o_grad);
    MLN_HIP(ctx, hipGetLastError());
    MLN_HIP(ctx, hipMemcpyAsync(loss + s0, o_loss, sizeof(double) * (size_t)Sc, hipMemcpyDefault, ctx->stream));
    MLN_HIP(ctx, hipMemcpyAsync(grad + (int64_t)s0 * m, o_grad, sizeof(double) * (size_t)Sc * m, hipMemcpyDefault, ctx->stream));
    MLN_HIP(ctx, hipStreamSynchronize(ctx->stream));
  }
  return MLN_OK;
}
```

Measured before the change: 7.347 million.

## Defer kernel-matrix row generation and overlap it with subsampled objective evaluations

In implicit-factor fits, only the row classes needed by the subsampled objective and by the Gram stride are generated up front. The remaining row blocks are deferred and either produced inside a role-split kernel that runs the sub-objective alongside row generation, or flushed by a finish call before any consumer that needs the full factor. This is meant to take most of the kernel-matrix build off the critical path of fit_prepare. It adds gating state, many finish hooks and a fused kernel. If any consumer is missed it risks reading uncomputed rows.

```diff
diff --git a/mellon_amd/csrc/api_fit.hip b/mellon_amd/csrc/api_fit.hip
--- a/mellon_amd/csrc/api_fit.hip
+++ b/mellon_amd/csrc/api_fit.hip
@@ -9,11 +9,92 @@
   *rows = (f->n > *first) ? (f->n - *first + s - 1) / s : 0;
 }
 
+int fit_enqueue_pending_rows(mln_fit* f, int64_t from, int64_t count, const int* gate) {
+  if (count <= 0) return MLN_OK;
+  KmRowMap map = f->dr_map;
+  map.blocks = f->dr_blocks + from;
+  map.count = count;
+  map.skip_flag = f->dr_flag;
+  map.gate = gate;
+  map.gate_want = MLN_GATE_F64;
+  return launch_kernel_matrix_blocks(f->ctx, f->cov, f->dr_x, f->n, f->dr_ypad, f->m, f->d, f->dr_xx, f->dr_yy, f->L, f->ldl, map);
+}
+
+int fit_finish_rows(mln_fit* f) {
+  if (!fit_rows_pending(f)) return MLN_OK;
+  mln_ctx* ctx = f->ctx;
+  MLN_HIP(ctx, hipSetDevice(ctx->device));
+  const double t0 = now_s();
+  MLN_TRY(fit_enqueue_pending_rows(f, f->dr_done, f->dr_count - f->dr_done, nullptr));
+  f->dr_done = f->dr_count;
+  MLN_HIP(ctx, hipStreamSynchronize(ctx->stream));
+  f->times[0] += now_s() - t0;
+  MLN_HIP(ctx, mln_dfree(f->dr_block));
+  f->dr_block = nullptr; f->dr_x = f->dr_xx = f->dr_yy = f->dr_ypad = nullptr; f->dr_blocks = nullptr; f->dr_flag = nullptr;
+  return MLN_OK;
+}
+
+int fit_finish_rows_unless_sampled(mln_fit* f, int64_t stride, int64_t first) {
+  if (!fit_rows_pending(f)) return MLN_OK;
+  if (first == 0 && stride >= 1 && (stride % f->dr_map.rs == 0 || stride % f->dr_gram_stride == 0)) return MLN_OK;
+  return fit_finish_rows(f);
+}
+
+static int fit_generate_rows_deferred(mln_fit* f, const double* x_dev, const double* xu_dev, int32_t flags, bool* deferred,
+                                      std::vector<int>* list) {
+  mln_ctx* ctx = f->ctx;
+  const int64_t n = f->n, m = f->m, ld = f->ldl;
+  const int d = f->d;
+  *deferred = false;
+  if (!(flags & MLN_FIT_IMPLICIT) || f->L32 || ctx->n_ranks > 1 || emulated_ranks(ctx) || m > 8192) return MLN_OK;
+  if (const char* ev = mln_experiment("MELLON_AMD_DEFER_ROWS")) { if (std::atoi(ev) == 0) return MLN_OK; }
+  if (const char* ev = mln_experiment("MELLON_AMD_SUBSAMPLE")) { if (std::atoi(ev) == 0) return MLN_OK; }
+  if (!kernel_matrix_rows_eligible(f->cov, n, m, d, ld) || !objective_sub_gen_ok(ld, f->cov.leaves[0].kind, d)) return MLN_OK;
+  const int64_t gs = (n > 12 * m) ? n / (6 * m) : 1;
+  if (gs < 11) return MLN_OK;
+  const int64_t ss = std::max<int64_t>(2, 3 * gs / 16);
+  if ((double)gs * (double)ld * 1024.0 >= 4294967296.0) return MLN_OK;
+  const KmRowMap sub = km_row_map_class(n, ss, 0), gram = km_row_map_class(n, gs, 0);
+  if ((double)ss * (double)sub.bpc >= 2147483647.0) return MLN_OK;
+  list->clear();
+  for (int64_t cls = 1; cls < ss; ++cls) {
+    const KmRowMap c = km_row_map_class(n, ss, cls);
+    for (int64_t b = 0; b < c.count; ++b) list->push_back((int)(c.ord0 + b));
+  }
+  if (list->empty()) return MLN_OK;
+  const int64_t pad = kernel_matrix_rows_pad();
+  const size_t n_dbl = (size_t)n * d + (size_t)n + (size_t)(m + pad) + (size_t)(m + pad) * d;
+  const size_t n_int = list->size() + 16;
+  MLN_HIP(ctx, mln_dmalloc(&f->dr_block, sizeof(double) * n_dbl + sizeof(int) * n_int));
+  double* p = (double*)f->dr_block;
+  double* xc = p; p += (size_t)n * d;
+  double* xx = p; p += n;
+  double* yy = p; p += m + pad;
+  double* ypad = p; p += (size_t)(m + pad) * d;
+  f->dr_flag = (int*)p;
+  f->dr_blocks = f->dr_flag + 16;
+  MLN_HIP(ctx, hipMemcpyAsync(xc, x_dev, sizeof(double) * (size_t)n * d, hipMemcpyDeviceToDevice, ctx->stream));
+  MLN_HIP(ctx, hipMemsetAsync(f->dr_flag, 0, sizeof(int) * 16, ctx->stream));
+  MLN_HIP(ctx, hipMemcpyAsync(f->dr_blocks, list->data(), sizeof(int) * list->size(), hipMemcpyHostToDevice, ctx->stream));
+  MLN_TRY(kernel_matrix_rows_operands(ctx, f->cov, xc, n, xu_dev, m, d, xx, yy, ypad));
+  f->dr_x = xc; f->dr_xx = xx; f->dr_yy = yy; f->dr_ypad = ypad;
+  MLN_TRY(launch_kernel_matrix_blocks(ctx, f->cov, xc, n, ypad, m, d, xx, yy, f->L, ld, sub));
+  MLN_TRY(launch_kernel_matrix_blocks(ctx, f->cov, xc, n, ypad, m, d, xx, yy, f->L, ld, gram));
+  f->dr_map = sub;
+  f->dr_gram_stride = gs;
+  f->dr_count = (int64_t)list->size();
+  f->dr_done = 0;
+  *deferred = true;
+  return MLN_OK;
+}
+
 void fit_free(mln_fit* f) {
   if (!f) return;
   mln_ctx* ctx = f->ctx;
   (void)hipSetDevice(ctx->device);
+  (void)fit_finish_rows(f);
   (void)hipStreamSynchronize(ctx->stream);
+  if (f->dr_block) (void)mln_dfree(f->dr_block);
   if (f->L && f->L != f->Lp) (void)mln_dfree(f->L);
   if (f->Lp) (void)mln_dfree(f->Lp);
   triinv_free(&f->tri);
@@ -302,6 +383,7 @@
         else if (std::strcmp(ev, "fixed") == 0 && bounded) f->l32_fixed = 1;
       }
     }
+    std::vector<int> pending_list;
     if (pipelined) {
       for (int c = 0; c < up.n_chunks; ++c) {
         int64_t r0 = 0, rows = 0;
@@ -311,7 +393,9 @@
       }
       MLN_TRY(up.finish());
     } else {
-      MLN_TRY(launch_kernel_matrix(ctx, f->cov, dx.dev, n, du.dev, m, d, f->L, f->ldl, 0.0, f->L32, f->l32_fixed));
+      bool deferred = false;
+      MLN_TRY(fit_generate_rows_deferred(f, dx.dev, du.dev, flags, &deferred, &pending_list));
+      if (!deferred) MLN_TRY(launch_kernel_matrix(ctx, f->cov, dx.dev, n, du.dev, m, d, f->L, f->ldl, 0.0, f->L32, f->l32_fixed));
     }
     MLN_TRY(fit_alloc_workspace(f));
     MLN_HIP(ctx, hipStreamSynchronize(ctx->stream));
@@ -522,6 +606,7 @@
   if (f->kspace) { mln_set_error(ctx, "project needs the explicit factor (prepare without MLN_FIT_IMPLICIT)"); return MLN_ERR_UNSUPPORTED; }
   if (p < 1 || p > f->m) { mln_set_error(ctx, "project: rank out of range"); return MLN_ERR_SHAPE; }
   MLN_HIP(ctx, hipSetDevice(ctx->device));
+  MLN_TRY(fit_finish_rows(f));
   mln_fit* g = new mln_fit();
   g->ctx = ctx; g->n = f->n; g->m = p; g->d = 0; g->full = false;
   g->ldl = pad16(p); g->ldp = pad16(p);
@@ -570,6 +655,7 @@
   if (row0 < 0 || n_rows < 0 || row0 + n_rows > f->n) { mln_set_error(ctx, "row range out of bounds"); return MLN_ERR_SHAPE; }
   if (n_rows == 0) return MLN_OK;
   MLN_HIP(ctx, hipSetDevice(ctx->device));
+  MLN_TRY(fit_finish_rows(f));
   DevOut o;
   MLN_TRY(o.init(ctx, out, (size_t)n_rows * f->m));
   if (f->kspace) {
diff --git a/mellon_amd/csrc/api_internal.h b/mellon_amd/csrc/api_internal.h
--- a/mellon_amd/csrc/api_internal.h
+++ b/mellon_amd/csrc/api_internal.h
@@ -13,6 +13,7 @@
 
 #include "linalg.h"
 #include "mln_internal.h"
+#include "cov_rows.h"
 #include "objective.h"
 #include "precond_rebuild.h"
 #include "solver.h"
@@ -126,6 +127,12 @@
   double build_seconds = 0.0;
   double times_sub = 0.0, times_rebuild = 0.0, sub_pass_equiv = 0.0;
   int evals_sub = 0, n_rebuild = 0;
+  void* dr_block = nullptr;
+  const double *dr_x = nullptr, *dr_xx = nullptr, *dr_yy = nullptr, *dr_ypad = nullptr;
+  int* dr_blocks = nullptr;
+  int* dr_flag = nullptr;
+  int64_t dr_count = 0, dr_done = 0, dr_gram_stride = 0;
+  KmRowMap dr_map{};
   double* dim_ell = nullptr;
   int dim_k = 0;
   double mu_dim = 0.0, mu_dens = 0.0;
@@ -152,6 +159,10 @@
 void fit_sample_rows(const mln_fit* f, int64_t s, int64_t* first, int64_t* rows);
 void fit_free(mln_fit* f);
 int fit_alloc_workspace(mln_fit* f);
+inline bool fit_rows_pending(const mln_fit* f) { return f->dr_done < f->dr_count; }
+int fit_finish_rows(mln_fit* f);
+int fit_finish_rows_unless_sampled(mln_fit* f, int64_t stride, int64_t first);
+int fit_enqueue_pending_rows(mln_fit* f, int64_t from, int64_t count, const int* gate);
 int fit_prepare_impl(mln_ctx* ctx, const mln_kernel_desc* cov, const double* x, int64_t n, int32_t d,
                             const double* xu, int64_t m, double jitter, const double* Lp_in, int32_t flags,
                             mln_fit* f);
diff --git a/mellon_amd/csrc/api_precond.hip b/mellon_amd/csrc/api_precond.hip
--- a/mellon_amd/csrc/api_precond.hip
+++ b/mellon_amd/csrc/api_precond.hip
@@ -119,6 +119,7 @@
   if (row_stride < 1) row_stride = 1;
   const int64_t first = (row_stride - f->row0 % row_stride) % row_stride;
   const int64_t rows = (f->n > first) ? (f->n - first + row_stride - 1) / row_stride : 0;
+  MLN_TRY(fit_finish_rows_unless_sampled(f, row_stride, first));
   const double* Ls = f->L + first * f->ldl;
   if (!f->kspace) return gram_of(ctx, Ls, f->ldl * row_stride, rows, f->m, (double)row_stride, G, ldg);
   bool quant = f->cov_bounded01 && f->m >= 256 && row_stride > 1;
@@ -144,6 +145,7 @@
 
 int fit_gemvT(mln_fit* f, const double* t_dev, double* rhs_dev) {
   mln_ctx* ctx = f->ctx;
+  MLN_TRY(fit_finish_rows(f));
   ObjArgs a = obj_args(f);
   a.weights = t_dev;
   a.part_loss = nullptr;
@@ -254,6 +256,7 @@
   mln_ctx* ctx = f->ctx;
   const int64_t m = f->m, ldg = f->ldl;
   *outcome = 0;
+  MLN_TRY(fit_finish_rows(f));
   RebuildSelection sel{};
   double target = rows_per_m * (double)m;
   if (const int n_emu = emulated_ranks(ctx)) target /= (double)n_emu;
@@ -373,6 +376,7 @@
     fit_sample_rows(f, rs, &first, &rows);
     a.n = rows; a.row_first = first; a.row_stride = rs; a.out_scale = (double)rs;
   }
+  MLN_TRY(fit_finish_rows_unless_sampled(f, rs, a.row_first));
   if (f->kspace) {
     a.L32 = f->L32;
     a.l32_fixed = f->l32_fixed;
diff --git a/mellon_amd/csrc/api_solve.hip b/mellon_amd/csrc/api_solve.hip
--- a/mellon_amd/csrc/api_solve.hip
+++ b/mellon_amd/csrc/api_solve.hip
@@ -1,6 +1,9 @@
 #include "api_internal.h"
 #include "mln_options.h"
 
+
+static constexpr int DEFER_G_OBJ = 128;
+static constexpr int DEFER_SLICE = 448;
 
 void obj_account(mln_fit* f, bool f32) {
   float ms = 0.f;
@@ -46,6 +49,7 @@
   }
   MLN_HIP(ctx, hipSetDevice(ctx->device));
   MLN_TRY(fit_ensure_lp(f));
+  MLN_TRY(fit_finish_rows(f));
   const int64_t m = f->m;
   MLN_HIP(ctx, hipMemcpyAsync(f->d_z, z, sizeof(double) * m, hipMemcpyDefault, ctx->stream));
   MLN_HIP(ctx, hipMemcpyAsync(f->h_z, f->d_z, sizeof(double) * m, hipMemcpyDeviceToHost, ctx->stream));
@@ -88,6 +92,7 @@
   mln_ctx* ctx = f->ctx;
   MLN_HIP(ctx, hipSetDevice(ctx->device));
   if (f->n == 0) return MLN_OK;
+  MLN_TRY(fit_finish_rows(f));
   MLN_HIP(ctx, hipMemcpyAsync(f->d_z, z, sizeof(double) * f->m, hipMemcpyDefault, ctx->stream));
   if (f->f_final >= 0 && mu == f->mu && !is_device_ptr(z) && f->z_cached.size() == (size_t)f->m &&
       std::memcmp(z, f->z_cached.data(), sizeof(double) * f->m) == 0) {
@@ -112,6 +117,13 @@
                             hipEvent_t* ev, const std::vector<int64_t>* sub_strides) {
   mln_ctx* ctx = f->ctx;
   const int64_t m = f->m, ld = f->ldl, ld2 = f->ld2;
+  bool fuse = false;
+  if (fit_rows_pending(f)) {
+    int64_t first = 0, rows = 0;
+    if (gate && sub_strides && sub_strides->size() == 1) fit_sample_rows(f, (*sub_strides)[0], &first, &rows);
+    fuse = gate && sub_strides && sub_strides->size() == 1 && first == 0 && (*sub_strides)[0] % f->dr_map.rs == 0 && !f->L32;
+    if (!fuse) MLN_TRY(fit_finish_rows(f));
+  }
   if (f->kspace) {
     GemvTri g1{f->P, ld, m, u_dev, f->d_w, nullptr, 1, m, m, 0, 0, gate};
     MLN_TRY(launch_gemv_tri(ctx, g1));
@@ -135,6 +147,7 @@
     if (gate) a32.cap = &f->sv.st->cap;
     MLN_TRY(launch_objective(ctx, a32));
   }
+  if (fuse) MLN_TRY(fit_enqueue_pending_rows(f, f->dr_done, f->dr_count - f->dr_done, gate));
   if (ev) MLN_HIP(ctx, hipEventRecord(ev[1], ctx->stream));
   if (gate || !use32 || !f->L32) {
     a.gate_want = MLN_GATE_F64;
@@ -150,6 +163,25 @@
       as.f_keep[0] = as.f_keep[1] = nullptr; as.f_slot = nullptr;
       as.gate_want = MLN_GATE_SUB;
       as.gate2 = &f->sv.st->sub_level; as.gate2_want = (int)lv;
+      if (fuse) {
+        int g_obj = DEFER_G_OBJ, slice = DEFER_SLICE;
+        if (const char* e = mln_experiment("MELLON_AMD_DEFER_G_OBJ")) g_obj = std::max(1, std::atoi(e));
+        if (const char* e = mln_experiment("MELLON_AMD_DEFER_SLICE")) slice = std::max(1, std::atoi(e));
+        g_obj = std::min(g_obj, as.n_wg);
+        SubGenArgs g{};
+        g.leaf0 = f->cov.leaves[0];
+        g.x = f->dr_x; g.n = f->n; g.y = f->dr_ypad; g.m = m; g.d = f->d; g.xx = f->dr_xx; g.yy = f->dr_yy; g.out = f->L; g.ldo = ld;
+        g.map = f->dr_map;
+        g.map.blocks = f->dr_blocks + f->dr_done;
+        g.map.count = std::min<int64_t>(slice, f->dr_count - f->dr_done);
+        g.map.skip_flag = f->dr_flag;
+        g.g_obj = g_obj;
+        g.done_flag = f->dr_flag;
+        MLN_TRY(launch_objective_sub_gen(ctx, as, g));
+        f->dr_done += g.map.count;
+        fuse = false;
+        continue;
+      }
       MLN_TRY(launch_objective(ctx, as));
     }
   }
@@ -354,6 +386,7 @@
     MLN_TRY(dev_bcast0(ctx, (double*)f->sv.st, (int64_t)(sizeof(SolverState) / sizeof(double))));
     MLN_HIP(ctx, hipMemcpyAsync(f->h_state, f->sv.st, sizeof(SolverState), hipMemcpyDeviceToHost, ctx->stream));
     MLN_HIP(ctx, hipStreamSynchronize(ctx->stream));
+    if (f->h_state->gate != MLN_GATE_SUB) MLN_TRY(fit_finish_rows(f));
     if (f->h_state->gate == MLN_GATE_DONE) break;
     if (subs_live && f->h_state->n_eval_sub > 0 && f->h_state->gate != MLN_GATE_SUB) subs_live = nullptr;
     if (f->h_state->gate == MLN_GATE_PAUSE) {
diff --git a/mellon_amd/csrc/cov_kernels.hip b/mellon_amd/csrc/cov_kernels.hip
--- a/mellon_amd/csrc/cov_kernels.hip
+++ b/mellon_amd/csrc/cov_kernels.hip
@@ -947,6 +947,28 @@
   return MLN_OK;
 }
 
+bool kernel_matrix_rows_eligible(const DevCov& cov, int64_t n, int64_t m, int d, int64_t ldo) {
+  bool contiguous = cov.n_toks == 1 && cov.leaves[0].ndims == d;
+  if (contiguous)
+    for (int k = 0; k < d; ++k) contiguous = contiguous && cov.dims[cov.leaves[0].dims_off + k] == k;
+  const int kind = cov.leaves[0].kind;
+  return contiguous && mln_experiment("MELLON_AMD_KM_NO_ROWS") == nullptr && ldo <= m + 64 && d <= 64 && n >= 4096 && m >= 256 &&
+         (kind == MLN_K_MATERN32 || kind == MLN_K_MATERN52 || kind == MLN_K_EXPQUAD || kind == MLN_K_EXPONENTIAL);
+}
+int64_t kernel_matrix_rows_pad() { return ROWS_PAD; }
+int kernel_matrix_rows_operands(mln_ctx* ctx, const DevCov& cov, const double* x, int64_t n, const double* y, int64_t m, int d,
+                                double* xx, double* yy, double* ypad) {
+  MLN_TRY(sqnorms(ctx, cov, x, n, d, xx));
+  MLN_TRY(sqnorms(ctx, cov, y, m, d, yy));
+  MLN_TRY(pad_rows(ctx, y, m, d, ypad));
+  MLN_HIP(ctx, hipMemsetAsync(yy + m, 0, sizeof(double) * (size_t)ROWS_PAD, ctx->stream));
+  return MLN_OK;
+}
+int launch_kernel_matrix_blocks(mln_ctx* ctx, const DevCov& cov, const double* x, int64_t n, const double* ypad, int64_t m, int d,
+                                const double* xx, const double* yy, double* out, int64_t ldo, const KmRowMap& map) {
+  return launch_kernel_matrix_rows_q(ctx, cov, x, n, ypad, m, d, xx, yy, out, ldo, 0.0, nullptr, 0, &map);
+}
+
 int launch_predict_mean1(mln_ctx* ctx, const DevCov& cov, const double* x, int64_t n, const double* y,
                          int64_t m, int d, const double* w, double mu, double* out) {
   if (n == 0) return MLN_OK;
diff --git a/mellon_amd/csrc/cov_rows.h b/mellon_amd/csrc/cov_rows.h
--- a/mellon_amd/csrc/cov_rows.h
+++ b/mellon_amd/csrc/cov_rows.h
@@ -8,6 +8,25 @@
 constexpr int NNS = 65;
 }
 
+struct KmRowMap {
+  const int* blocks;
+  int64_t count;
+  int64_t ord0;
+  int64_t rs, bpc;
+  const int* skip_flag;
+  const int* gate;
+  int gate_want;
+};
+inline KmRowMap km_row_map_all(int64_t n) {
+  const int64_t nb = (n + 127) / 128;
+  return KmRowMap{nullptr, nb, 0, 1, nb > 0 ? nb : 1, nullptr, nullptr, 0};
+}
+inline KmRowMap km_row_map_class(int64_t n, int64_t rs, int64_t cls) {
+  const int64_t bpc = ((n + rs - 1) / rs + 127) / 128;
+  const int64_t rows = n > cls ? (n - cls + rs - 1) / rs : 0;
+  return KmRowMap{nullptr, (rows + 127) / 128, cls * (bpc > 0 ? bpc : 1), rs, bpc > 0 ? bpc : 1, nullptr, nullptr, 0};
+}
+
 int launch_kernel_matrix_rows(mln_ctx* ctx, const DevCov& cov, const double* x, int64_t n, const double* y, int64_t m,
                               int d, const double* xx, const double* yy, double* out, int64_t ldo, double add_diag,
                               float* out32);
diff --git a/mellon_amd/csrc/cov_rows.hip b/mellon_amd/csrc/cov_rows.hip
--- a/mellon_amd/csrc/cov_rows.hip
+++ b/mellon_amd/csrc/cov_rows.hip
@@ -3,7 +3,8 @@
 
 #define MLN_ROWS_DECL(NAME)                                                                                     \
   int NAME(mln_ctx* ctx, const DevCov& cov, const double* x, int64_t n, const double* y, int64_t m, int d,      \
-           const double* xx, const double* yy, double* out, int64_t ldo, double add_diag, float* out32, int q32);
+           const double* xx, const double* yy, double* out, int64_t ldo, double add_diag, float* out32, int q32,  \
+           const KmRowMap* map);
 MLN_ROWS_DECL(launch_kernel_matrix_rows_matern32)
 MLN_ROWS_DECL(launch_kernel_matrix_rows_matern52)
 MLN_ROWS_DECL(launch_kernel_matrix_rows_expquad)
@@ -13,17 +14,17 @@
 int launch_kernel_matrix_rows(mln_ctx* ctx, const DevCov& cov, const double* x, int64_t n, const double* y, int64_t m,
                               int d, const double* xx, const double* yy, double* out, int64_t ldo, double add_diag,
                               float* out32) {
-  return launch_kernel_matrix_rows_q(ctx, cov, x, n, y, m, d, xx, yy, out, ldo, add_diag, out32, 0);
+  return launch_kernel_matrix_rows_q(ctx, cov, x, n, y, m, d, xx, yy, out, ldo, add_diag, out32, 0, nullptr);
 }
 
 int launch_kernel_matrix_rows_q(mln_ctx* ctx, const DevCov& cov, const double* x, int64_t n, const double* y, int64_t m,
                                 int d, const double* xx, const double* yy, double* out, int64_t ldo, double add_diag,
-                                float* out32, int q32) {
+                                float* out32, int q32, const KmRowMap* map) {
   switch (cov.leaves[0].kind) {
-    case MLN_K_MATERN32: return launch_kernel_matrix_rows_matern32(ctx, cov, x, n, y, m, d, xx, yy, out, ldo, add_diag, out32, q32);
-    case MLN_K_MATERN52: return launch_kernel_matrix_rows_matern52(ctx, cov, x, n, y, m, d, xx, yy, out, ldo, add_diag, out32, q32);
-    case MLN_K_EXPQUAD: return launch_kernel_matrix_rows_expquad(ctx, cov, x, n, y, m, d, xx, yy, out, ldo, add_diag, out32, q32);
-    case MLN_K_EXPONENTIAL: return launch_kernel_matrix_rows_exponential(ctx, cov, x, n, y, m, d, xx, yy, out, ldo, add_diag, out32, q32);
+    case MLN_K_MATERN32: return launch_kernel_matrix_rows_matern32(ctx, cov, x, n, y, m, d, xx, yy, out, ldo, add_diag, out32, q32, map);
+    case MLN_K_MATERN52: return launch_kernel_matrix_rows_matern52(ctx, cov, x, n, y, m, d, xx, yy, out, ldo, add_diag, out32, q32, map);
+    case MLN_K_EXPQUAD: return launch_kernel_matrix_rows_expquad(ctx, cov, x, n, y, m, d, xx, yy, out, ldo, add_diag, out32, q32, map);
+    case MLN_K_EXPONENTIAL: return launch_kernel_matrix_rows_exponential(ctx, cov, x, n, y, m, d, xx, yy, out, ldo, add_diag, out32, q32, map);
     default:
       mln_set_error(ctx, "persistent-row kernel matrix: unsupported leaf kind");
       return MLN_ERR_UNSUPPORTED;
diff --git a/mellon_amd/csrc/cov_rows_impl.h b/mellon_amd/csrc/cov_rows_impl.h
--- a/mellon_amd/csrc/cov_rows_impl.h
+++ b/mellon_amd/csrc/cov_rows_impl.h
@@ -22,24 +22,25 @@
 }
 
 template <int KIND, bool HAS32, int KSTEPS>
-__global__ __launch_bounds__(512) void k_kernel_matrix_rows(DevCov cov, const double* __restrict__ x, int64_t n,
-                                                            const double* __restrict__ y, int64_t m, int d,
-                                                            const double* __restrict__ xx,
-                                                            const double* __restrict__ yy,
-                                                            double* __restrict__ out, int64_t ldo, double add_diag,
-                                                            float* __restrict__ out32, int q32) {
+__device__ __forceinline__ void kernel_matrix_rows_block(const DevLeaf& leaf0, const double* __restrict__ x, int64_t n,
+                                                         const double* __restrict__ y, int64_t m, int d,
+                                                         const double* __restrict__ xx,
+                                                         const double* __restrict__ yy,
+                                                         double* __restrict__ out, int64_t ldo, double add_diag,
+                                                         float* __restrict__ out32, int q32, const int64_t base,
+                                                         const int64_t rs) {
   constexpr int YB = TN * NNS + 512;
   __shared__ double ys[2][YB];
   __shared__ double yn[3][512];
   constexpr int NST = (TN * 4 * KSTEPS + 511) / 512;
   constexpr int EPI_VALU = (HAS32 ? 32 : 29) * 16 + 8;
-  const double c2 = covepi::sq_scale<KIND>(cov.leaves[0]), m2 = -2.0 * c2;
+  const double c2 = covepi::sq_scale<KIND>(leaf0), m2 = -2.0 * c2;
   const int tid = threadIdx.x;
   const int lane = tid & 63, wave = tid >> 6, li = lane & 15, lk = lane >> 4;
-  const int64_t row0 = (int64_t)blockIdx.x * 128 + wave * 16;
+  const int64_t row0 = base + rs * (wave * 16);
   double a[16];
   {
-    const int64_t ar = (row0 + li < n) ? row0 + li : n - 1;
+    const int64_t ar = (row0 + rs * li < n) ? row0 + rs * li : n - 1;
 #pragma unroll
     for (int ks = 0; ks < 16; ++ks) {
       const int k = 4 * ks + lk;
@@ -49,15 +50,16 @@
   double xr[4];
 #pragma unroll
   for (int r = 0; r < 4; ++r) {
-    const int64_t row = row0 + lk + 4 * r;
+    const int64_t row = row0 + rs * (lk + 4 * r);
     xr[r] = (row < n) ? c2 * (xx[row] + 1e-12) : 0.0;
   }
-  double* const out_wg = out + (int64_t)blockIdx.x * 128 * ldo;
-  float* const out32_wg = HAS32 ? out32 + (int64_t)blockIdx.x * 128 * ldo : nullptr;
+  double* const out_wg = out + base * ldo;
+  float* const out32_wg = HAS32 ? out32 + base * ldo : nullptr;
+  const unsigned row_pitch = (unsigned)rs * (unsigned)ldo;
   unsigned lrowb[4], lrowb32[4];
 #pragma unroll
   for (int r = 0; r < 4; ++r) {
-    lrowb[r] = ((unsigned)(wave * 16 + lk + 4 * r) * (unsigned)ldo + (unsigned)li) * 8u;
+    lrowb[r] = ((unsigned)(wave * 16 + lk + 4 * r) * row_pitch + (unsigned)li) * 8u;
     lrowb32[r] = lrowb[r] >> 1;
   }
   for (int e = tid; e < 2 * YB; e += 512) (&ys[0][0])[e] = 0.0;
@@ -96,7 +98,7 @@
         acc[t] = __builtin_amdgcn_mfma_f64_16x16x4f64(a[ks], yb[16 * t * NNS + 4 * ks], acc[t], 0, 0, 0);
   };
   const int64_t ntiles = (ldo + TN - 1) / TN;
-  const bool interior_rows = (int64_t)blockIdx.x * 128 + 128 <= n;
+  const bool interior_rows = base + rs * 127 < n;
   stage_load(0); stage_store(0, 0);
   if (ntiles > 1) { stage_load(1); stage_store(1, 1); }
   __syncthreads();
@@ -134,7 +136,7 @@
         const double yc = yn[ncur][16 * tt + li];
 #pragma unroll
         for (int r = 0; r < 4; ++r) {
-          const int64_t row = row0 + lk + 4 * r;
+          const int64_t row = row0 + rs * (lk + 4 * r);
           if (row < n && c < ldo) {
             const double v = (c < m) ? leaf_value_k<KIND>(m2, xr[r], yc, cur[tt][r]) + ((row == c) ? add_diag : 0.0) : 0.0;
             out[row * ldo + c] = v;
@@ -163,19 +165,45 @@
   }
 }
 
+__device__ __forceinline__ int64_t km_block_base(const KmRowMap& map, int64_t ord) {
+  const int64_t cls = ord / map.bpc, b = ord - cls * map.bpc;
+  return cls + map.rs * 128 * b;
+}
+
+template <int KIND, bool HAS32, int KSTEPS>
+__global__ __launch_bounds__(512) void k_kernel_matrix_rows(DevCov cov, const double* __restrict__ x, int64_t n,
+                                                            const double* __restrict__ y, int64_t m, int d,
+                                                            const double* __restrict__ xx,
+                                                            const double* __restrict__ yy,
+                                                            double* __restrict__ out, int64_t ldo, double add_diag,
+                                                            float* __restrict__ out32, int q32, KmRowMap map) {
+  if (map.skip_flag && *map.skip_flag) return;
+  if (map.gate && (*map.gate & 3) != map.gate_want) return;
+  const int64_t ord = map.blocks ? map.blocks[blockIdx.x] : map.ord0 + blockIdx.x;
+  kernel_matrix_rows_block<KIND, HAS32, KSTEPS>(cov.leaves[0], x, n, y, m, d, xx, yy, out, ldo, add_diag, out32, q32,
+                                                km_block_base(map, ord), map.rs);
+}
+
 }
 
 
 template <int KIND>
 static int launch_rows_kind(mln_ctx* ctx, const DevCov& cov, const double* x, int64_t n, const double* y, int64_t m, int d,
                             const double* xx, const double* yy, double* out, int64_t ldo, double add_diag, float* out32,
-                            int q32) {
-  const dim3 grid((unsigned)((n + 127) / 128)), block(512);
+                            int q32, const KmRowMap* map_in) {
+  KmRowMap map = km_row_map_all(n);
+  if (map_in) map = *map_in;
+  if (map.count <= 0) return MLN_OK;
+  if (map.rs < 1 || map.bpc < 1 || (double)map.rs * (double)ldo * 128.0 * 8.0 >= 4294967296.0) {
+    mln_set_error(ctx, "persistent-row kernel matrix: row map out of range");
+    return MLN_ERR_ARG;
+  }
+  const dim3 grid((unsigned)map.count), block(512);
 #define MLN_KM_ROWS2(KS)                                                                                              \
   if (out32) hipLaunchKernelGGL((k_kernel_matrix_rows<KIND, true, KS>), grid, block, 0, ctx->stream, cov, x, n, y, m, d, \
-                                xx, yy, out, ldo, add_diag, out32, q32);                                             \
+                                xx, yy, out, ldo, add_diag, out32, q32, map);                                        \
   else hipLaunchKernelGGL((k_kernel_matrix_rows<KIND, false, KS>), grid, block, 0, ctx->stream, cov, x, n, y, m, d, xx,  \
-                          yy, out, ldo, add_diag, out32, q32);
+                          yy, out, ldo, add_diag, out32, q32, map);
   if (d <= 32) { MLN_KM_ROWS2(8) }
   else if (d <= 52) { MLN_KM_ROWS2(13) }
   else { MLN_KM_ROWS2(16) }
@@ -186,6 +214,7 @@
 
 #define MLN_DEFINE_ROWS_KIND(NAME, KIND)                                                                                 \
   int NAME(mln_ctx* ctx, const DevCov& cov, const double* x, int64_t n, const double* y, int64_t m, int d,               \
-           const double* xx, const double* yy, double* out, int64_t ldo, double add_diag, float* out32, int q32) {       \
-    return launch_rows_kind<KIND>(ctx, cov, x, n, y, m, d, xx, yy, out, ldo, add_diag, out32, q32);                      \
-  }
+           const double* xx, const double* yy, double* out, int64_t ldo, double add_diag, float* out32, int q32,         \
+           const KmRowMap* map) {                                                                                        \
+    return launch_rows_kind<KIND>(ctx, cov, x, n, y, m, d, xx, yy, out, ldo, add_diag, out32, q32, map);                 \
+  }
diff --git a/mellon_amd/csrc/cov_rows_q.h b/mellon_amd/csrc/cov_rows_q.h
--- a/mellon_amd/csrc/cov_rows_q.h
+++ b/mellon_amd/csrc/cov_rows_q.h
@@ -1,5 +1,6 @@
 #pragma once
 #include "mln_core.h"
+struct KmRowMap;
 int launch_kernel_matrix_rows_q(mln_ctx* ctx, const DevCov& cov, const double* x, int64_t n, const double* y, int64_t m,
                                 int d, const double* xx, const double* yy, double* out, int64_t ldo, double add_diag,
-                                float* out32, int q32);
+                                float* out32, int q32, const KmRowMap* map = nullptr);
diff --git a/mellon_amd/csrc/dimensionality.hip b/mellon_amd/csrc/dimensionality.hip
--- a/mellon_amd/csrc/dimensionality.hip
+++ b/mellon_amd/csrc/dimensionality.hip
@@ -578,6 +578,7 @@
   MLN_TRY(dim_one_pass_ok(f));
   MLN_HIP(ctx, hipSetDevice(ctx->device));
   MLN_TRY(fit_ensure_lp(f));
+  MLN_TRY(fit_finish_rows(f));
   const int64_t m = f->m, ld = f->ldl;
   std::vector<double> zh((size_t)(2 * m));
   MLN_HIP(ctx, hipMemcpyAsync(zh.data(), z, sizeof(double) * 2 * m, hipMemcpyDefault, ctx->stream));
diff --git a/mellon_amd/csrc/mln_internal.h b/mellon_amd/csrc/mln_internal.h
--- a/mellon_amd/csrc/mln_internal.h
+++ b/mellon_amd/csrc/mln_internal.h
@@ -9,6 +9,13 @@
 int launch_kernel_matrix(mln_ctx* ctx, const DevCov& cov, const double* x, int64_t n, const double* y,
                          int64_t m, int d, double* out, int64_t ldo, double add_diag, float* out32 = nullptr,
                          int q32 = 0);
+struct KmRowMap;
+bool kernel_matrix_rows_eligible(const DevCov& cov, int64_t n, int64_t m, int d, int64_t ldo);
+int64_t kernel_matrix_rows_pad();
+int kernel_matrix_rows_operands(mln_ctx* ctx, const DevCov& cov, const double* x, int64_t n, const double* y, int64_t m, int d,
+                                double* xx, double* yy, double* ypad);
+int launch_kernel_matrix_blocks(mln_ctx* ctx, const DevCov& cov, const double* x, int64_t n, const double* ypad, int64_t m, int d,
+                                const double* xx, const double* yy, double* out, int64_t ldo, const KmRowMap& map);
 __device__ __forceinline__ float mln_surrogate_bits(double v, int q32) {
   const unsigned fx = (unsigned)fmin(fma(v, 4294967296.0, 0.5), 4294967295.0);
   return q32 ? __uint_as_float(fx) : (float)v;
diff --git a/mellon_amd/csrc/objective.h b/mellon_amd/csrc/objective.h
--- a/mellon_amd/csrc/objective.h
+++ b/mellon_amd/csrc/objective.h
@@ -1,5 +1,6 @@
 #pragma once
 #include "mln_core.h"
+#include "cov_rows.h"
 
 struct ObjArgs {
   const double* L; int64_t ldl; int64_t n; int64_t m;
@@ -28,6 +29,16 @@
   int f_accum;
 };
 enum { MLN_GATE_F64 = 0, MLN_GATE_F32 = 1, MLN_GATE_DONE = 2, MLN_GATE_SUB = 3, MLN_GATE_F32C = 5, MLN_GATE_PAUSE = 6 };
+struct SubGenArgs {
+  DevLeaf leaf0;
+  const double* x; int64_t n; const double* y; int64_t m; int d;
+  const double* xx; const double* yy; double* out; int64_t ldo;
+  KmRowMap map;
+  int g_obj;
+  int* done_flag;
+};
+bool objective_sub_gen_ok(int64_t ldl, int kind, int d);
+int launch_objective_sub_gen(mln_ctx* ctx, const ObjArgs& a, const SubGenArgs& g);
 int objective_max_m();
 int objective_max_m_one_pass();
 bool objective_can_keep_f(int64_t n, int n_wg);
diff --git a/mellon_amd/csrc/objective.hip b/mellon_amd/csrc/objective.hip
--- a/mellon_amd/csrc/objective.hip
+++ b/mellon_amd/csrc/objective.hip
@@ -3,6 +3,7 @@
 #include "mln_internal.h"
 #include "objective.h"
 #include "mln_options.h"
+#include "cov_rows_impl.h"
 
 namespace {
 
@@ -197,16 +198,14 @@
 }
 
 template <int CPT, int R, int MODE, bool KEEP = false, bool VEC = false>
-__global__ __launch_bounds__(WG) void k_objective(ObjArgs a) {
-  if (a.gate && (*a.gate & 3) != a.gate_want) return;
-  if (a.gate2 && *a.gate2 != a.gate2_want) return;
+__device__ __forceinline__ void objective_range(const ObjArgs& a, const int wg) {
   __shared__ double red[2][8][R];
   const int tid = threadIdx.x;
   const int64_t ld2 = a.ldl / 2;
   const d2* __restrict__ L2 = reinterpret_cast<const d2*>(a.L);
   const int64_t nsteps = (a.n + R - 1) / R;
   const int64_t per = (nsteps + a.n_wg - 1) / a.n_wg;
-  const int64_t s_beg = (int64_t)blockIdx.x * per;
+  const int64_t s_beg = (int64_t)wg * per;
   int64_t s_end = s_beg + per;
   if (s_end > nsteps) s_end = nsteps;
 
@@ -252,7 +251,7 @@
     for (int64_t i = r_beg + tid; i < r_end; i += WG) fo[i] = fstage[i - r_beg];
   }
   if (MODE != MODE_FONLY) {
-    double* pg = a.part_grad + (int64_t)blockIdx.x * a.m_pad;
+    double* pg = a.part_grad + (int64_t)wg * a.m_pad;
     const int64_t store_lim = a.seg_cols > 0 ? ((a.seg_cols + 1) & ~(int64_t)1) : a.m_pad;
     const double osc = a.out_scale != 0.0 ? a.out_scale : 1.0;
 #pragma unroll
@@ -261,7 +260,7 @@
       if (col < store_lim) *reinterpret_cast<d2*>(pg + col) = (d2){g[c].x * osc, g[c].y * osc};
     }
     if (MODE == MODE_OBJ_HESS) {
-      double* ph = a.part_hess + (int64_t)blockIdx.x * a.m_pad;
+      double* ph = a.part_hess + (int64_t)wg * a.m_pad;
 #pragma unroll
       for (int c = 0; c < CPT; ++c) {
         const int64_t col = 2 * ((int64_t)c * WG + tid);
@@ -272,7 +271,33 @@
 #pragma unroll
       for (int off = 32; off > 0; off >>= 1) loss += __shfl_xor(loss, off, 64);
     }
-    if (tid == 0 && a.part_loss) a.part_loss[blockIdx.x] = loss * osc;
+    if (tid == 0 && a.part_loss) a.part_loss[wg] = loss * osc;
+  }
+}
+
+template <int CPT, int R, int MODE, bool KEEP = false, bool VEC = false>
+__global__ __launch_bounds__(WG) void k_objective(ObjArgs a) {
+  if (a.gate && (*a.gate & 3) != a.gate_want) return;
+  if (a.gate2 && *a.gate2 != a.gate2_want) return;
+  objective_range<CPT, R, MODE, KEEP, VEC>(a, (int)blockIdx.x);
+}
+
+template <int KIND, int KSTEPS, int CPT, int R>
+__global__ __launch_bounds__(WG) void k_objective_sub_gen(ObjArgs a, SubGenArgs gen) {
+  if ((int)blockIdx.x >= gen.g_obj) {
+    if (gen.map.skip_flag && *gen.map.skip_flag) return;
+    const int64_t ord = gen.map.blocks[blockIdx.x - gen.g_obj];
+    kernel_matrix_rows_block<KIND, false, KSTEPS>(gen.leaf0, gen.x, gen.n, gen.y, gen.m, gen.d, gen.xx, gen.yy, gen.out, gen.ldo,
+                                                  0.0, nullptr, 0, km_block_base(gen.map, ord), gen.map.rs);
+    return;
+  }
+  const int gate = *a.gate;
+  if (blockIdx.x == 0 && threadIdx.x == 0 && (gate & 3) == MLN_GATE_F64) *gen.done_flag = 1;
+  if ((gate & 3) != a.gate_want) return;
+  if (a.gate2 && *a.gate2 != a.gate2_want) return;
+  for (int wg = (int)blockIdx.x; wg < a.n_wg; wg += gen.g_obj) {
+    if (wg != (int)blockIdx.x) __syncthreads();
+    objective_range<CPT, R, MODE_OBJ, false, false>(a, wg);
   }
 }
 
@@ -796,3 +821,40 @@
 }
 
 int launch_reduce_obj(mln_ctx* ctx, const ObjArgs& a, double* out) { return launch_reduce_obj2(ctx, a, out, out + 1); }
+
+bool objective_sub_gen_ok(int64_t ldl, int kind, int d) {
+  const int cpt = (int)((ldl / 2 + WG - 1) / WG);
+  return ldl % 2 == 0 && cpt == 5 && d >= 1 && d <= 64 &&
+         (kind == MLN_K_MATERN32 || kind == MLN_K_MATERN52 || kind == MLN_K_EXPQUAD || kind == MLN_K_EXPONENTIAL);
+}
+
+namespace {
+template <int KIND, int KSTEPS>
+int launch_sub_gen_cpt(mln_ctx* ctx, const ObjArgs& a, const SubGenArgs& g) {
+  const dim3 grid((unsigned)(g.g_obj + g.map.count)), block(WG);
+  hipLaunchKernelGGL((k_objective_sub_gen<KIND, KSTEPS, 5, 2>), grid, block, 0, ctx->stream, a, g);
+  MLN_HIP(ctx, hipGetLastError());
+  return MLN_OK;
+}
+template <int KIND>
+int launch_sub_gen_kind(mln_ctx* ctx, const ObjArgs& a, const SubGenArgs& g) {
+  if (g.d <= 32) return launch_sub_gen_cpt<KIND, 8>(ctx, a, g);
+  if (g.d <= 52) return launch_sub_gen_cpt<KIND, 13>(ctx, a, g);
+  return launch_sub_gen_cpt<KIND, 16>(ctx, a, g);
+}
+}
+
+int launch_objective_sub_gen(mln_ctx* ctx, const ObjArgs& a, const SubGenArgs& g) {
+  if (!objective_sub_gen_ok(a.ldl, g.leaf0.kind, g.d) || !a.gate || !g.map.blocks || !g.done_flag || g.g_obj < 1 || g.map.count < 0 ||
+      a.weights || a.f_out || a.part_hess || a.L32 || a.f_slot || a.seg_cols ||
+      (double)g.map.rs * (double)g.ldo * 128.0 * 8.0 >= 4294967296.0) {
+    mln_set_error(ctx, "objective: no role-split kernel for this evaluation");
+    return MLN_ERR_UNSUPPORTED;
+  }
+  switch (g.leaf0.kind) {
+    case MLN_K_MATERN32: return launch_sub_gen_kind<MLN_K_MATERN32>(ctx, a, g);
+    case MLN_K_MATERN52: return launch_sub_gen_kind<MLN_K_MATERN52>(ctx, a, g);
+    case MLN_K_EXPQUAD: return launch_sub_gen_kind<MLN_K_EXPQUAD>(ctx, a, g);
+    default: return launch_sub_gen_kind<MLN_K_EXPONENTIAL>(ctx, a, g);
+  }
+}
diff --git a/mellon_amd/csrc/objective_batch.hip b/mellon_amd/csrc/objective_batch.hip
--- a/mellon_amd/csrc/objective_batch.hip
+++ b/mellon_amd/csrc/objective_batch.hip
@@ -234,6 +234,7 @@
 int launch_batch(mln_fit* f, const double* W, double* A1, double* part_loss, int64_t n_tiles, double* part, int n_ranges,
                  int64_t rows_per_range) {
   mln_ctx* ctx = f->ctx;
+  MLN_TRY(fit_finish_rows(f));
   hipLaunchKernelGGL((k_batch_forward<NT>), dim3((unsigned)n_tiles), dim3(256), 0, ctx->stream, f->L, f->ldl, f->n, f->ldl, W,
                      f->V, f->Vdr, f->mu, A1, part_loss);
   MLN_HIP(ctx, hipGetLastError());
```

Result: slower. 7.128 million (-3.0%).
